# flash4242/Promptable-Counterfactual-GAN

Measured on AMD Instinct MI355X. Metric: images/sec (G+D step) MNIST-28 cDCGAN bs512 @1/2/4/8 MI355X; % MFMA roofline, higher is better.
Workload: dtype f32

## Files before the change

### include/pcgan_hip.h

```cpp
#ifndef PCGAN_HIP_H
#define PCGAN_HIP_H

#include <stddef.h>
#include <stdint.h>

#ifdef __cplusplus
extern "C" {
#endif

typedef void* pcg_stream_t;

typedef enum pcg_status {
  PCG_OK = 0,
  PCG_ERR_INVALID = -1,
  PCG_ERR_WORKSPACE = -2,
  PCG_ERR_LAUNCH = -3,
  PCG_ERR_UNSUPPORTED = -4
} pcg_status;

typedef enum pcg_act {
  PCG_ACT_NONE = 0,
  PCG_ACT_RELU = 1,
  PCG_ACT_LRELU = 2,
  PCG_ACT_TANH = 3,
// ... 443 lines not shown
} pcg_patch_mask_bits_args;
int pcg_patch_mask_bits(const pcg_patch_mask_bits_args* args, pcg_stream_t stream);

typedef struct pcg_mnist_cf_entry_args {
  const float* x;
  const float* table;
  const float* mask;
  const int64_t* target;
  float* out;
  int32_t B, T, HW, K, mask_mode, q0, nq;
} pcg_mnist_cf_entry_args;
int pcg_mnist_cf_entry(const pcg_mnist_cf_entry_args* args, pcg_stream_t stream);

typedef struct pcg_mnist_cf_tail_args {
  const float* c;
  const float* x;
  const float* mask;
  float* x_cf;
  float* raw; float* masked;
  float* sums;
  float scale;
  int32_t B, T, HW, mask_mode, q0, nq;
} pcg_mnist_cf_tail_args;
int pcg_mnist_cf_tail(const pcg_mnist_cf_tail_args* args, pcg_stream_t stream);

#define PCG_MNIST_CF_GROUP_SUMS 8
typedef struct pcg_mnist_cf_score_args {
  const float* logits_cf;
  const float* logits_orig;
  const int64_t* target;
  const int64_t* y_true;
  const float* tail_sums;
  int64_t* pred; float* conf; float* p_target; float* p_true; float* p_orig_true; float* flip;
  float* group_sums;
  int32_t B, T, K, ld, group_rows, q0, nq;
} pcg_mnist_cf_score_args;
int pcg_mnist_cf_score(const pcg_mnist_cf_score_args* args, pcg_stream_t stream);

int pcg_house_losses(const float* d_real, const float* d_fake, const float* d_fake_g, int64_t n, const float* g_cls, const float* am,
                     const float* pen, float lambda_cls, float w_reg, float lambda_mask, float w_reg_log, float* out5, pcg_stream_t stream);

typedef struct pcg_house_res_fwd_args {
  const float* cont; int32_t ncont;
  const float* samples; const int32_t* seg_dev; int32_t T;
  const float* norm; const float* x; const float* mask;
  const int32_t* col_src;
  int32_t D, B;
  float* res; float* masked; float* x_cf; float* partial512; int32_t* ticket; float* pen_out; float* am_out;
} pcg_house_res_fwd_args;
typedef struct pcg_house_res_bwd_args {
  const float* res; const float* masked; const float* mask; const float* gx_a; const float* gx_b;
  float w_pen, w_am;
  int32_t ncont; const int32_t* cont_idx_dev; const int32_t* seg_dev; int32_t S, T;
  const int32_t* cat_idx_dev; const float* norm;
  int32_t D, B;
  float* dcont; float* dsamples;
} pcg_house_res_bwd_args;
typedef struct pcg_house_loss_args {
  const float* d_real; const float* d_fake; const float* d_fake_g; int32_t n;
  const float* g_cls;
  const float* am; const float* pen;
  float lambda_cls, w_reg, lambda_mask, w_reg_log;
  const float* ce_row_loss;
  int32_t n_ce;
  float* out6;
} pcg_house_loss_args;
typedef struct pcg_house_diag_args {
  const float* logits_cf; const float* logits_orig;
  const int64_t* src_rows;
  const int64_t* target_y; const float* masked;
  int32_t B, nc, D;
  float eps;
  float* out4;
  double* acc;
} pcg_house_diag_args;
int pcg_house_residual_fwd(const pcg_house_res_fwd_args* args, const pcg_sn_fwd_batch* rider , pcg_stream_t stream);
int pcg_house_residual_bwd(const pcg_house_res_bwd_args* args, const pcg_house_loss_args* losses ,
                           const pcg_house_diag_args* diag , pcg_stream_t stream);
int pcg_house_diag(const pcg_house_diag_args* args, pcg_stream_t stream);
int pcg_house_draws(int64_t* target_y, int32_t B, int32_t num_classes, const int64_t* y, uint64_t offset_target, float* mask, int32_t D,
                    const int32_t* zero_cols, int32_t n_zero_cols, uint64_t offset_mask, float* noise, int32_t T, uint64_t offset_noise,
                    uint64_t seed, float* onehot_target, float* onehot_y, pcg_stream_t stream);
int pcg_house_draws_counter(int64_t* target_y, int32_t B, int32_t num_classes, const int64_t* y, float* mask, int32_t D,
                            const int32_t* zero_cols, int32_t n_zero_cols, float* noise, int32_t T, uint64_t seed, float* onehot_target,
                            float* onehot_y, uint64_t* counter, pcg_stream_t stream);
int pcg_house_batch_draws_counter(int64_t* target_y, int32_t B, int32_t num_classes, const float* X, const int64_t* Y,
                                  const int64_t* perm, int64_t n_perm, int64_t n_rows, float* x_out, int64_t* y_out,
                                  int64_t* src_out , float* mask, int32_t D, const int32_t* zero_cols, int32_t n_zero_cols,
                                  float* noise, int32_t T, uint64_t seed, float* onehot_target , float* onehot_y ,
                                  uint64_t* counter, pcg_stream_t stream);

int pcg_house_clf_batch(const float* X, const int64_t* Y, const int64_t* perm, int64_t n_perm, int64_t n_rows, float* x_out, int64_t* y_out,
                        int32_t B, int32_t D, float* m0, int32_t w0, float keep0, float* m1, int32_t w1, float keep1, float* m2, int32_t w2,
                        float keep2, uint64_t seed, uint64_t offset, int64_t cursor, pcg_stream_t stream);
int pcg_house_clf_batch_counter(const float* X, const int64_t* Y, const int64_t* perm, int64_t n_perm, int64_t n_rows, float* x_out,
                                int64_t* y_out, int32_t B, int32_t D, float* m0, int32_t w0, float keep0, float* m1, int32_t w1, float keep1,
                                float* m2, int32_t w2, float keep2, uint64_t seed, uint64_t* counter, pcg_stream_t stream);
int pcg_ce_weighted_tally(const float* logits, const int64_t* target, const float* class_weight, int32_t B, int32_t K, int32_t seg,
                          double* tally , float* dlogits , float* dbias ,
                          float* seg_loss , pcg_stream_t stream);

int pcg_mnist_clf_batch(const float* X, const int64_t* Y, const int64_t* perm, int64_t n_perm, int64_t n_rows, float* x_out, int64_t* y_out,
                        int32_t B, int32_t D, float* m0, int32_t w0, float keep0, float* m1, int32_t w1, float keep1, uint64_t seed,
                        uint64_t offset, int64_t cursor, pcg_stream_t stream);
int pcg_mnist_clf_batch_counter(const float* X, const int64_t* Y, const int64_t* perm, int64_t n_perm, int64_t n_rows, float* x_out,
                                int64_t* y_out, int32_t B, int32_t D, float* m0, int32_t w0, float keep0, float* m1, int32_t w1, float keep1,
                                uint64_t seed, uint64_t* counter, pcg_stream_t stream);
int pcg_drop2d_flatten_fwd(const float* a, const float* mask , float scale, int32_t R, int32_t HW, int32_t C, float* out,
                           pcg_stream_t stream);
int pcg_drop2d_flatten_bwd(const float* dflat, const float* mask, float scale, const float* y, int act, float slope, int32_t R, int32_t HW,
                           int32_t C, float* out, pcg_stream_t stream);
int pcg_mnist_clf_head(const float* h, const float* m1, float scale, const float* W2, const float* b2, const int64_t* y, int32_t R, int32_t I,
                       int32_t K, float* logits, float* loss, double* tally , float* dW2, float* db2, float* dh, float* db1,
                       pcg_stream_t stream);

int pcg_dp_barrier(pcg_stream_t stream);
int32_t pcg_dp_rccl_version(void);

#define PCG_DP_UNIQUE_ID_BYTES 128
int pcg_dp_unique_id(void* id_out );
int pcg_dp_init(const void* id , int32_t rank, int32_t world);
int32_t pcg_dp_world(void);
int32_t pcg_dp_rank(void);
pcg_stream_t pcg_dp_side_stream(void);
int pcg_dp_allreduce(float* buf, int64_t n, pcg_stream_t stream);
int pcg_dp_allreduce_begin(float* buf, int64_t n, int32_t slot, pcg_stream_t producer_stream);
int pcg_dp_record(int32_t slot);
int pcg_dp_allreduce_wait(int32_t slot, pcg_stream_t consumer_stream);
int pcg_dp_allreduce_sum_f64(double* buf, int64_t n, pcg_stream_t stream);
int pcg_dp_broadcast(void* buf, int64_t nbytes, int32_t root, pcg_stream_t stream);
int pcg_dp_sync_batchnorm(int32_t enable);
int pcg_dp_shutdown(void);

int pcg_tune_set(const char* name, int32_t value);

int pcg_conv_plan_describe(const pcg_conv_geom* g, int32_t op, int32_t assume_scratch, char* out, size_t out_bytes);
enum { PCG_PLAN_GEMM_ACT = 0, PCG_PLAN_GEMM = 1, PCG_PLAN_LINEAR_WGRAD = 2, PCG_PLAN_LINEAR_WGRAD_GROUPED = 3, PCG_PLAN_MEAN = 4,
       PCG_PLAN_ABS_MEAN = 5, PCG_PLAN_CROSS_ENTROPY = 6, PCG_PLAN_EMBED_CONCAT_BWD = 7, PCG_PLAN_ACT = 8, PCG_PLAN_ELEMENTWISE = 9,
       PCG_PLAN_BN_COLREDUCE = 10, PCG_PLAN_BN_APPLY = 11, PCG_PLAN_BN_FINALIZE = 12, PCG_PLAN_INSTNORM = 13, PCG_PLAN_SPECTRAL_NORM = 14,
       PCG_PLAN_ADAM = 15 };
enum { PCG_PLAN_EW_TABULAR = 0, PCG_PLAN_EW_CF_OPS = 1, PCG_PLAN_EW_POINTWISE = 2, PCG_PLAN_EW_GATHER_CHANNEL = 3 };
int pcg_launch_plan_describe(int32_t op, const int64_t* args, int32_t n_args, char* out, size_t out_bytes);
size_t pcg_conv_scratch_parts_bytes(void);
size_t pcg_conv_scratch_arrivals_bytes(void);
int pcg_conv_set_scratch(pcg_stream_t stream, void* parts, size_t parts_bytes, void* arrivals, size_t arrivals_bytes);
int pcg_conv_reset_scratch(pcg_stream_t stream);
size_t pcg_conv_pixtab_bytes(const pcg_conv_geom* g);
int pcg_conv_pixtab_register(const pcg_conv_geom* g, void* host_out, size_t bytes, const void* device_table);
size_t pcg_conv_cliptab_bytes(const pcg_conv_geom* g);
int pcg_conv_cliptab_register(const pcg_conv_geom* g, void* host_out, size_t bytes, const void* device_table);
double pcg_conv_sched_model(const int32_t* ktiles, int32_t n);
int pcg_conv_pad_clip_query(const pcg_conv_geom* g, int32_t op, int32_t groups, int32_t assume_scratch, int32_t* taken, int32_t* order,
                            int32_t* tile_rows, double* predicted);
int pcg_debug_stamp_buffer(void* buf, int64_t bytes);

typedef struct pcg_moons_cf_desc {
  int32_t hidden, clf_hidden, B, N;
  int32_t nG, nD, nC, nG_adam, nD_adam;
  int32_t g_off[14], d_off[8], c_off[6];
  double lr_G, lr_D, beta1, beta2, adam_eps;
  float bn_eps, bn_momentum, sn_eps, slope;
  float lambda_cls, lambda_l1, lambda_l2, lambda_mask;
} pcg_moons_cf_desc;

typedef struct pcg_moons_cf_train_args {
  const float* X; const int64_t* Y;
  const int64_t* rows;
  const int64_t* target_y;
  const float* mask;
  float* g_flat; float* d_flat; const float* c_flat;
  float* g_exp_avg; float* g_exp_avg_sq; int64_t* g_step;
  float* d_exp_avg; float* d_exp_avg_sq; int64_t* d_step;
  float* bn_mean[3]; float* bn_var[3]; int64_t* bn_nbt[3];
  float* sn_u[4]; float* sn_v[4];
  float* logs;
  float* scratch; size_t scratch_bytes;
} pcg_moons_cf_train_args;

size_t pcg_moons_cf_scratch_bytes(const pcg_moons_cf_desc* desc, int32_t forward);
int pcg_moons_cf_train_steps(const pcg_moons_cf_desc* desc, const pcg_moons_cf_train_args* args, int32_t n_steps, pcg_stream_t stream);

typedef struct pcg_moons_cf_fwd_args {
  int32_t which, train, B;
  const float* x; const float* onehot; const float* mask;
  float* params;
  float* bn_mean[3]; float* bn_var[3]; int64_t* bn_nbt[3];
  float* sn_u[4]; float* sn_v[4];
  float* out0; float* out1;
  float* scratch; size_t scratch_bytes;
} pcg_moons_cf_fwd_args;
int pcg_moons_cf_forward(const pcg_moons_cf_desc* desc, const pcg_moons_cf_fwd_args* args, pcg_stream_t stream);

typedef struct pcg_moons_cf_eval_args {
  int64_t N; int32_t M, T, group;
  const float* x; const int64_t* y;
  const float* masks;
  const int64_t* target; const float* row_mask;
  const float* g_flat; const float* c_flat;
  const float* bn_mean[3]; const float* bn_var[3];
  float* raw; float* masked; float* x_cf;
  float* logits_cf; float* logits_x;
  int64_t* pred_cf; int64_t* pred_x;
  float* gain;
  float* sums;
} pcg_moons_cf_eval_args;
int pcg_moons_cf_eval(const pcg_moons_cf_desc* desc, const pcg_moons_cf_eval_args* args, pcg_stream_t stream);

typedef struct {
  const float* gamma;
  const float* beta;
  float* running_mean;
  float* running_var;
  int64_t* num_batches_tracked;
  float* save_mean;
  float* save_invstd;
  float* xhat;
  float eps;
  float momentum;
  int32_t training;
} pcg_dense_bn;
typedef struct {
  const float* xhat;
  const float* gamma;
  const float* invstd;
  float* dgamma;
  float* dbeta;
  int32_t accumulate;
} pcg_dense_bn_bwd;
int pcg_dense_rows_fwd(const float* x, const float* W, const float* bias , int32_t R, int32_t I, int32_t O,
                       const pcg_dense_bn* bn , int act, float slope, float* y, pcg_stream_t stream);
int pcg_dense_rows_dgrad(const float* dz, const float* W, int32_t R, int32_t O, int32_t I, int below_act, float below_slope,
                         const float* y_below , const pcg_dense_bn_bwd* bn , float* dx,
                         pcg_stream_t stream);
int pcg_dense_rows_wgrad(const float* dz, const float* x, int32_t R, int32_t O, int32_t I, float* dW, float* db ,
                         int accumulate, pcg_stream_t stream);
int pcg_dense_rows_fwd_post(const float* x, const float* W, const float* bias , int32_t R, int32_t I, int32_t O, int act,
                            float slope, const float* gamma, const float* beta, float* running_mean ,
                            float* running_var , int64_t* num_batches_tracked , float eps, float momentum,
                            const float* mask , float scale, float* a, float* save_mean, float* save_invstd, float* y,
                            pcg_stream_t stream);
int pcg_dense_rows_dgrad_post(const float* dz, const float* W, int32_t R, int32_t O, int32_t I, const float* mask , float scale,
                              const float* a, const float* mean, const float* invstd, const float* gamma, int act, float slope,
                              float* dgamma, float* dbeta, float* db , int accumulate, float* dx, pcg_stream_t stream);

typedef struct pcg_moons_gan_desc {
  int32_t hidden, z_dim, label_dim, B, N;
  int32_t nG, nD, nG_adam, nD_adam;
  int32_t g_off[4], d_off[4];
  double lr_G, lr_D, beta1, beta2, adam_eps;
} pcg_moons_gan_desc;

typedef struct pcg_moons_gan_train_args {
  const float* X; const int64_t* Y;
  const int64_t* rows;
  const float* z;
  const int64_t* labels;
  float* g_flat; float* d_flat;
  float* g_exp_avg; float* g_exp_avg_sq; int64_t* g_step;
  float* d_exp_avg; float* d_exp_avg_sq; int64_t* d_step;
  float* logs;
  float* scratch; size_t scratch_bytes;
} pcg_moons_gan_train_args;

size_t pcg_moons_gan_scratch_bytes(const pcg_moons_gan_desc* desc);
int pcg_moons_gan_train_steps(const pcg_moons_gan_desc* desc, const pcg_moons_gan_train_args* args, int32_t n_steps, pcg_stream_t stream);

typedef struct pcg_moons_gan_fwd_args {
  int32_t which; int64_t R;
  const float* x; const float* onehot; const float* params;
  float* out;
} pcg_moons_gan_fwd_args;
int pcg_moons_gan_forward(const pcg_moons_gan_desc* desc, const pcg_moons_gan_fwd_args* args, pcg_stream_t stream);

typedef struct pcg_moons_clf_fit_desc {
  int32_t hidden, N, nC, nC_adam;
  int32_t c_off[6];
  double lr, beta1, beta2, adam_eps;
} pcg_moons_clf_fit_desc;
typedef struct pcg_moons_clf_fit_args {
  const float* X; const int64_t* Y;
  float* c_flat; float* exp_avg; float* exp_avg_sq; int64_t* step;
  float* losses;
  int32_t* correct;
  float* scratch; size_t scratch_bytes;
} pcg_moons_clf_fit_args;
size_t pcg_moons_clf_fit_scratch_bytes(const pcg_moons_clf_fit_desc* desc);
int pcg_moons_clf_fit(const pcg_moons_clf_fit_desc* desc, const pcg_moons_clf_fit_args* args, int32_t n_steps, pcg_stream_t stream);

int32_t pcg_calib_mfma_blocks(int32_t rounds);
size_t pcg_calib_mfma_workspace_bytes(int32_t rounds);
int pcg_calib_mfma(int32_t iters, int32_t rounds, void* workspace, size_t workspace_bytes, double* flop_out ,
                   uint64_t** stamps_out , pcg_stream_t stream);
int pcg_calib_copy(const void* src, void* dst, int64_t nbytes, pcg_stream_t stream);

int pcg_relu_maxpool2_fwd(const float* z, float* p, uint8_t* idx, int32_t B, int32_t H, int32_t W, int32_t C, pcg_stream_t stream);
int pcg_relu_maxpool2_bwd(const float* dp, const float* p, const uint8_t* idx, float* dz, int32_t B, int32_t H, int32_t W, int32_t C,
                          pcg_stream_t stream);

#define PCG_DELTA_GAN_BUILD 0
#define PCG_DELTA_GAN_REGATHER 1
#define PCG_LOGIT_HEAD_D 0
#define PCG_LOGIT_HEAD_G 1
#define PCG_DELTA_GAN_CHUNK 1024

typedef struct pcg_delta_gan_entry_args {
  const float* x;
// ... 142 lines not shown
```

### promptable-counterfactual-gan_amd/_lib.py

```python
import ctypes
import os

import torch

_HERE = os.path.dirname(os.path.abspath(__file__))
LIB_PATH = os.environ.get("PCG_LIB") or os.path.join(_HERE, "libpcgan_hip.so")

PCG_OK = 0
ACT_NONE, ACT_RELU, ACT_LRELU, ACT_TANH, ACT_SIGMOID = 0, 1, 2, 3, 4
(PLAN_GEMM_ACT, PLAN_GEMM, PLAN_LINEAR_WGRAD, PLAN_LINEAR_WGRAD_GROUPED, PLAN_MEAN, PLAN_ABS_MEAN, PLAN_CROSS_ENTROPY,
 PLAN_EMBED_CONCAT_BWD, PLAN_ACT, PLAN_ELEMENTWISE, PLAN_BN_COLREDUCE, PLAN_BN_APPLY, PLAN_BN_FINALIZE, PLAN_INSTNORM,
 PLAN_SPECTRAL_NORM, PLAN_ADAM) = range(16)
PLAN_EW_TABULAR, PLAN_EW_CF_OPS, PLAN_EW_POINTWISE, PLAN_EW_GATHER_CHANNEL = range(4)


class PcgError(RuntimeError):
    pass


class ConvGeom(ctypes.Structure):

    _fields_ = [(n, ctypes.c_int32) for n in ("B", "IH", "IW", "Cin", "OH", "OW", "Cout", "KH", "KW", "stride", "pad")]

    def key(self):
# ... 123 lines not shown
    _fields_ = [(n, _P) for n in ("xhat", "gamma", "invstd", "dgamma", "dbeta")] + [("accumulate", _I)]


_PP, _PI, _F = ctypes.POINTER(ctypes.c_void_p), ctypes.POINTER(ctypes.c_int32), ctypes.c_float


class SnFwdBatch(ctypes.Structure):
    _fields_ = ([("n", _I), ("reps", _I), ("power_iteration", _I), ("eps", _F), ("w_orig", _PP), ("out_features", _PI), ("in_features", _PI)] +
                [(n, _PP) for n in ("u", "v", "w_bar", "sigma", "u_used", "v_used")])


class SnBwdBatch(ctypes.Structure):
    _fields_ = [("n", _I), ("passes", _I), ("dw_bar", _PP), ("w_bar", _PP), ("out_features", _PI), ("in_features", _PI), ("u", _PP), ("v", _PP),
                ("sigma", _PP), ("dw_orig", _PP), ("accumulate", _PI), ("db_dst", _PP), ("db_src", _PP)]


class HouseCriticFwdArgs(ctypes.Structure):
    _fields_ = ([(n, _I) for n in ("n_pass", "B", "D", "NC")] + [("slope", _F)] +
                [(n, _PP) for n in ("x", "onehot", "w_bar", "bias", "a0", "a1", "a2", "a3", "out")])


class HouseCriticBwdArgs(ctypes.Structure):
    _fields_ = ([(n, _I) for n in ("n_pass", "B", "D")] + [("slope", _F)] +
                [(n, _PP) for n in ("dout", "w_bar", "a1", "a2", "a3", "d3", "d2", "d1", "dx")])


class HouseClsFwdArgs(ctypes.Structure):
    _fields_ = ([("x", _P), ("B", _I), ("w_kmajor", _PP), ("bias", _PP)] + [(n, _P) for n in ("a1", "a2", "a3", "a4", "logits", "ce_target")] +
                [("ce_grad_scale", _F), ("ce_dlogits", _P), ("ce_row_loss", _P)])


class HouseClsBwdArgs(ctypes.Structure):
    _fields_ = [("dlogits", _P), ("B", _I), ("w_stored", _PP)] + [(n, _P) for n in ("a1", "a2", "a3", "a4", "dx")]


class HouseResFwdArgs(ctypes.Structure):
    _fields_ = ([("cont", _P), ("ncont", _I), ("samples", _P), ("seg_dev", _P), ("T", _I), ("norm", _P), ("x", _P), ("mask", _P), ("col_src", _PI),
                 ("D", _I), ("B", _I)] + [(n, _P) for n in ("res", "masked", "x_cf", "partial512", "ticket", "pen_out", "am_out")])


class HouseResBwdArgs(ctypes.Structure):
    _fields_ = ([(n, _P) for n in ("res", "masked", "mask", "gx_a", "gx_b")] + [("w_pen", _F), ("w_am", _F), ("ncont", _I), ("cont_idx_dev", _P),
                ("seg_dev", _P), ("S", _I), ("T", _I), ("cat_idx_dev", _P), ("norm", _P), ("D", _I), ("B", _I), ("dcont", _P), ("dsamples", _P)])


class HouseLossArgs(ctypes.Structure):
    _fields_ = ([("d_real", _P), ("d_fake", _P), ("d_fake_g", _P), ("n", _I), ("g_cls", _P), ("am", _P), ("pen", _P)] +
                [(n, _F) for n in ("lambda_cls", "w_reg", "lambda_mask", "w_reg_log")] + [("ce_row_loss", _P), ("n_ce", _I), ("out6", _P)])


class HouseDiagArgs(ctypes.Structure):
    _fields_ = ([(n, _P) for n in ("logits_cf", "logits_orig", "src_rows", "target_y", "masked")] + [("B", _I), ("nc", _I), ("D", _I), ("eps", _F),
                ("out4", _P), ("acc", _P)])


class DeltaGanEntryArgs(ctypes.Structure):
    _fields_ = ([(n, _P) for n in ("x", "y", "target", "y_host", "target_host", "table_g", "table_d", "g_in", "d_in", "labels_2b", "head_w",
                                   "head_w_packed")] + [(n, _I) for n in ("B", "HW", "K", "mode", "head_C", "head_P")])


class DeltaGanTailFwdArgs(ctypes.Structure):
    _fields_ = ([(n, _P) for n in ("x", "delta", "x_cf", "d_in", "loss_reg", "workspace")] + [("workspace_bytes", ctypes.c_size_t)] +
                [(n, _I) for n in ("B", "HW", "grid")])


class LogitHeadFwdArgs(ctypes.Structure):
    _fields_ = [(n, _P) for n in ("a", "w", "bias", "logits", "loss", "dlogit", "db", "workspace")] + [(n, _I) for n in ("R", "F", "mode")]


class LogitHeadBwdArgs(ctypes.Structure):
    _fields_ = [(n, _P) for n in ("a", "w", "dlogit", "da", "dw")] + [("slope", _F)] + [(n, _I) for n in ("R", "F", "dw_C", "dw_P")]


class DeltaGanTailBwdArgs(ctypes.Structure):
    _fields_ = ([(n, _P) for n in ("dD", "dC", "delta", "d_delta")] + [("lambda_cls", _F), ("reg_scale", _F)] +
                [(n, _I) for n in ("B", "HW", "dD_stride")])


class DeltaCfEntryArgs(ctypes.Structure):
    _fields_ = [(n, _P) for n in ("x", "table", "target", "target_host", "out")] + [(n, _I) for n in ("B", "T", "HW", "K", "q0", "nq")]


class DeltaCfTailArgs(ctypes.Structure):
    _fields_ = [(n, _P) for n in ("delta", "x", "x_cf", "sums")] + [(n, _I) for n in ("B", "T", "HW", "q0", "nq")]


class DeltaGanTargetDrawArgs(ctypes.Structure):
    _fields_ = [("target", _P), ("counter", _P), ("seed", ctypes.c_uint64), ("offset", ctypes.c_uint64), ("B", _I), ("K", _I)]


class ProbHeadFwdArgs(ctypes.Structure):
    _fields_ = ([(n, _P) for n in ("a", "w", "bias", "logits", "prob", "loss", "dlogit", "db", "workspace")] +
                [("workspace_bytes", ctypes.c_size_t), ("eps", _F)] + [(n, _I) for n in ("R", "F", "mode", "slabs")])


class LogEpsLossArgs(ctypes.Structure):
    _fields_ = [(n, _P) for n in ("p", "grad_out", "loss", "dp")] + [("eps", _F), ("R", _I), ("mode", _I)]


DELTA_GAN_BUILD, DELTA_GAN_REGATHER = 0, 1
LOGIT_HEAD_D, LOGIT_HEAD_G = 0, 1
DELTA_GAN_CHUNK = 1024
PROB_HEAD_D, PROB_HEAD_G = 0, 1
PROB_HEAD_MAX_SLABS = 16
CLASS_PICK_FIRST, CLASS_PICK_BEST = 0, 1
CLASS_PICK_KMAX = 64
CF_PANELS_GRID, CF_PANELS_PANELS = 0, 1

STRUCTS = {"pcg_conv_geom": ConvGeom, "pcg_in_xform": InXform, "pcg_wgrad_item": WgradItem, "pcg_sn_fwd_batch": SnFwdBatch,
           "pcg_sn_bwd_batch": SnBwdBatch, "pcg_house_g_desc": HouseGDesc, "pcg_house_g_fwd_args": HouseGFwdArgs,
           "pcg_house_g_bwd_args": HouseGBwdArgs, "pcg_house_critic_fwd_args": HouseCriticFwdArgs,
           "pcg_house_critic_bwd_args": HouseCriticBwdArgs, "pcg_house_cls_fwd_args": HouseClsFwdArgs, "pcg_house_cls_bwd_args": HouseClsBwdArgs,
           "pcg_house_res_fwd_args": HouseResFwdArgs, "pcg_house_res_bwd_args": HouseResBwdArgs, "pcg_house_loss_args": HouseLossArgs,
           "pcg_house_diag_args": HouseDiagArgs, "pcg_moons_cf_desc": MoonsCfDesc, "pcg_moons_cf_train_args": MoonsCfTrainArgs,
           "pcg_moons_cf_fwd_args": MoonsCfFwdArgs, "pcg_moons_cf_eval_args": MoonsCfEvalArgs,
           "pcg_house_cf_eval_args": HouseCfEvalArgs, "pcg_patch_mask_bits_args": PatchMaskBitsArgs,
           "pcg_mnist_cf_entry_args": MnistCfEntryArgs, "pcg_mnist_cf_tail_args": MnistCfTailArgs,
           "pcg_mnist_cf_score_args": MnistCfScoreArgs, "pcg_dense_bn": DenseBn,
           "pcg_dense_bn_bwd": DenseBnBwd, "pcg_moons_gan_desc": MoonsGanDesc, "pcg_moons_gan_train_args": MoonsGanTrainArgs,
           "pcg_moons_gan_fwd_args": MoonsGanFwdArgs, "pcg_moons_clf_fit_desc": MoonsClfFitDesc,
           "pcg_moons_clf_fit_args": MoonsClfFitArgs, "pcg_delta_gan_entry_args": DeltaGanEntryArgs,
           "pcg_delta_gan_tail_fwd_args": DeltaGanTailFwdArgs, "pcg_logit_head_fwd_args": LogitHeadFwdArgs,
           "pcg_logit_head_bwd_args": LogitHeadBwdArgs, "pcg_delta_gan_tail_bwd_args": DeltaGanTailBwdArgs,
           "pcg_delta_cf_entry_args": DeltaCfEntryArgs, "pcg_delta_cf_tail_args": DeltaCfTailArgs,
           "pcg_delta_gan_target_draw_args": DeltaGanTargetDrawArgs, "pcg_prob_head_fwd_args": ProbHeadFwdArgs,
           "pcg_log_eps_loss_args": LogEpsLossArgs}

_c = ctypes
_vp, _f, _i, _i64, _sz = _c.c_void_p, _c.c_float, _c.c_int, _c.c_int64, _c.c_size_t
_d = _c.c_double
_i32 = _c.c_int32
_gp = _c.POINTER(ConvGeom)
_xp = _c.POINTER(InXform)

PROTOTYPES = {
    "pcg_abi_version": (_i, []),
    "pcg_abi_struct_bytes": (_sz, [_c.c_char_p]),
    "pcg_last_error": (_c.c_char_p, []),
    "pcg_target_arch": (_c.c_char_p, []),
    "pcg_tune_set": (_i, [_c.c_char_p, _i32]),
    "pcg_debug_stamp_buffer": (_i, [_vp, _i64]),
    "pcg_conv_plan_describe": (_i, [_c.POINTER(ConvGeom), _i32, _i32, _c.c_char_p, _sz]),
    "pcg_launch_plan_describe": (_i, [_i32, _c.POINTER(_i64), _i32, _c.c_char_p, _sz]),
    "pcg_conv_scratch_parts_bytes": (_sz, []),
    "pcg_conv_scratch_arrivals_bytes": (_sz, []),
    "pcg_conv_set_scratch": (_i, [_vp, _vp, _sz, _vp, _sz]),
    "pcg_conv_reset_scratch": (_i, [_vp]),
    "pcg_conv_pixtab_bytes": (_sz, [_gp]),
    "pcg_conv_pixtab_register": (_i, [_gp, _vp, _sz, _vp]),
    "pcg_conv_cliptab_bytes": (_sz, [_gp]),
    "pcg_conv_cliptab_register": (_i, [_gp, _vp, _sz, _vp]),
    "pcg_conv_sched_model": (_d, [_vp, _i32]),
    "pcg_conv_pad_clip_query": (_i, [_gp, _i32, _i32, _i32, _vp, _vp, _vp, _vp]),
    "pcg_conv2d_fwd_bn_g": (_i, [_gp, _vp, _vp, _vp, _vp, _f, _f, _vp, _vp, _vp, _vp, _vp, _i32, _vp, _sz, _vp]),
    "pcg_bn_apply_act_g": (_i, [_vp, _i64, _i32, _vp, _vp, _vp, _vp, _i, _f, _vp, _i32, _vp]),
    "pcg_conv2d_dgrad_bn_phases": (_i32, [_gp]),
    "pcg_conv2d_dgrad_bnbwd_g": (_i, [_gp, _vp, _vp, _vp, _vp, _vp, _vp, _vp, _i, _f, _vp, _vp, _sz, _i32, _vp]),
    "pcg_bn_bwd_partial_g_workspace_bytes": (_sz, [_i32, _i32]),
    "pcg_bn_bwd_partial_g": (_i, [_vp, _vp, _i64, _i32, _vp, _vp, _vp, _vp, _i32, _i32, _vp, _vp, _vp, _i, _i32, _vp, _sz, _vp]),
    "pcg_bn_act_bwd_g_workspace_bytes": (_sz, [_i64, _i32, _i32]),
    "pcg_bn_act_bwd_premask_g": (_i, [_vp, _vp, _i64, _i32, _vp, _vp, _vp, _vp, _i, _f, _vp, _vp, _vp, _i, _i32, _vp, _sz, _vp]),
    "pcg_bce_pair": (_i, [_vp, _i64, _f, _f, _vp, _vp, _vp, _vp, _vp, _vp]),
    "pcg_conv2d_fwd_bnbwd_thin_ok": (_i32, [_gp]),
    "pcg_conv2d_fwd_bnbwd_thin_workspace_bytes": (_sz, [_gp]),
    "pcg_conv2d_fwd_bnbwd_thin": (_i, [_gp, _vp, _vp, _vp, _vp, _vp, _vp, _vp, _i, _f, _vp, _vp, _vp, _i, _vp, _sz, _vp]),
    "pcg_conv2d_bnin_full_ok": (_i32, [_gp, _i32]),
    "pcg_conv2d_fwd_bnin_full": (_i, [_gp, _vp, _vp, _vp, _vp, _vp, _i, _f, _i32, _vp, _vp, _i, _f, _vp, _vp]),
    "pcg_conv2d_wgrad_bnin_full": (_i, [_gp, _vp, _vp, _vp, _vp, _vp, _i, _f, _i32, _vp, _vp, _i, _vp, _sz, _vp]),
    "pcg_conv_precision_set": (_i, [_i32]),
    "pcg_conv_precision_get": (_i32, []),
    "pcg_slab_defer_begin": (_i, [_vp]),
    "pcg_slab_defer_flush": (_i, [_vp]),
    "pcg_slab_defer_pending": (_i32, []),
    "pcg_conv2d_dgrad_bnbwd_full_ok": (_i32, [_gp, _i32]),
    "pcg_conv2d_dgrad_bnbwd_full_workspace_bytes": (_sz, [_gp, _i32]),
    "pcg_conv2d_dgrad_bnbwd_full": (_i, [_gp, _vp, _vp, _vp, _vp, _vp, _vp, _vp, _i, _f, _vp, _vp, _vp, _i, _i32, _vp, _sz, _vp]),
    "pcg_calib_mfma_blocks": (_i32, [_i32]),
    "pcg_calib_mfma_workspace_bytes": (_sz, [_i32]),
    "pcg_calib_mfma": (_i, [_i32, _i32, _vp, _sz, _c.POINTER(_d), _c.POINTER(_c.c_uint64), _vp]),
    "pcg_calib_copy": (_i, [_vp, _vp, _i64, _vp]),
    "pcg_conv2d_fwd_workspace_bytes": (_sz, [_gp]),
    "pcg_conv2d_dgrad_workspace_bytes": (_sz, [_gp]),
    "pcg_conv2d_fwd": (_i, [_gp, _vp, _vp, _vp, _vp, _vp, _sz, _vp]),
    "pcg_conv2d_dgrad": (_i, [_gp, _vp, _vp, _vp, _vp, _vp, _sz, _vp]),
    "pcg_conv2d_fwd_act": (_i, [_gp, _vp, _vp, _vp, _i, _f, _vp, _vp, _sz, _vp]),
    "pcg_conv2d_dgrad_act": (_i, [_gp, _vp, _vp, _vp, _i, _f, _vp, _vp, _sz, _vp]),
    "pcg_conv2d_fwd_bn_workspace_bytes": (_sz, [_gp]),
    "pcg_conv2d_dgrad_bn_workspace_bytes": (_sz, [_gp]),
    "pcg_conv2d_fwd_bn": (_i, [_gp, _vp, _vp, _vp, _vp, _f, _f, _vp, _vp, _vp, _vp, _vp, _vp, _sz, _vp]),
    "pcg_conv2d_dgrad_bn": (_i, [_gp, _vp, _vp, _vp, _vp, _f, _f, _vp, _vp, _vp, _vp, _vp, _vp, _sz, _vp]),
    "pcg_conv2d_dgrad_mask": (_i, [_gp, _vp, _vp, _vp, _i, _f, _vp, _vp, _sz, _vp]),
    "pcg_conv2d_dgrad_mask_thin_ok": (_i32, [_gp]),
    "pcg_conv2d_xf_thin_ok": (_i32, [_gp]),
    "pcg_conv2d_fwd_add_mask": (_i, [_gp, _vp, _vp, _vp, _vp, _i, _f, _vp, _vp]),
    "pcg_conv2d_dgrad_add_mask": (_i, [_gp, _vp, _vp, _vp, _vp, _i, _f, _vp, _vp]),
    "pcg_conv2d_fwd_mask": (_i, [_gp, _vp, _vp, _vp, _i, _f, _vp, _vp, _sz, _vp]),
    "pcg_conv2d_dgrad_bnbwd": (_i, [_gp, _vp, _vp, _vp, _vp, _vp, _vp, _vp, _i, _f, _vp, _vp, _sz, _vp]),
    "pcg_conv2d_fwd_bnbwd": (_i, [_gp, _vp, _vp, _vp, _vp, _vp, _vp, _vp, _i, _f, _vp, _vp, _sz, _vp]),
    "pcg_conv2d_dgrad_add": (_i, [_gp, _vp, _vp, _vp, _vp, _vp, _sz, _vp]),
    "pcg_conv2d_fwd_bn_partial_rows": (_c.c_int32, [_gp]),
    "pcg_conv2d_dgrad_bn_partial_rows": (_c.c_int32, [_gp]),
    "pcg_bn_bwd_partial_workspace_bytes": (_sz, [_c.c_int32]),
    "pcg_bn_bwd_partial": (_i, [_vp, _vp, _i64, _c.c_int32, _vp, _vp, _vp, _vp, _c.c_int32, _vp, _vp, _vp, _i, _vp, _sz, _vp]),
    "pcg_conv2d_fwd_bn_xf": (_i, [_gp, _vp, _xp, _vp, _vp, _vp, _f, _f, _vp, _vp, _vp, _vp, _vp, _vp, _vp, _vp, _vp, _sz, _vp]),
    "pcg_conv2d_dgrad_bn_xf": (_i, [_gp, _vp, _xp, _vp, _vp, _vp, _f, _f, _vp, _vp, _vp, _vp, _vp, _vp, _vp, _vp, _vp, _sz, _vp]),
    "pcg_conv2d_fwd_xf": (_i, [_gp, _vp, _xp, _vp, _vp, _i, _f, _vp, _vp, _sz, _vp]),
    "pcg_conv2d_dgrad_xf": (_i, [_gp, _vp, _xp, _vp, _vp, _i, _f, _vp, _vp, _sz, _vp]),
    "pcg_conv2d_wgrad_xf": (_i, [_gp, _vp, _xp, _vp, _xp, _vp, _i, _vp, _sz, _vp]),
    "pcg_bn_train_stats_coef": (_i, [_vp, _i64, _c.c_int32, _f, _f, _vp, _vp, _vp, _vp, _vp, _vp, _vp, _vp, _vp, _sz, _vp]),
    "pcg_bn_db_workspace_bytes": (_sz, [_i64, _c.c_int32]),
    "pcg_bn_act_bwd_db": (_i, [_vp, _vp, _vp, _i64, _c.c_int32, _vp, _vp, _vp, _vp, _i, _f, _f, _vp, _vp, _vp, _i, _vp, _i, _vp, _sz, _vp]),
    "pcg_bn_bwd_partial_db_workspace_bytes": (_sz, [_c.c_int32]),
    "pcg_bn_bwd_partial_db": (_i, [_vp, _vp, _i64, _c.c_int32, _vp, _vp, _vp, _vp, _c.c_int32, _f, _vp, _vp, _vp, _i, _vp, _i, _vp, _sz, _vp]),
    "pcg_conv2d_dgrad_add_bnsum": (_i, [_gp, _vp, _vp, _vp, _vp, _vp, _vp, _f, _vp, _vp, _sz, _vp]),
    "pcg_conv2d_fwd_add": (_i, [_gp, _vp, _vp, _vp, _vp, _vp, _sz, _vp]),
    "pcg_conv2d_fwd_add_bnsum": (_i, [_gp, _vp, _vp, _vp, _vp, _vp, _vp, _f, _vp, _vp, _sz, _vp]),
    "pcg_conv_weight_adjoint": (_i, [_vp, _vp, _i32, _i32, _i32, _i32, _vp]),
    "pcg_conv_weight_adjoint_many": (_i, [_vp, _vp, _i32, _i32, _i32, _i32, _i32, _vp]),
    "pcg_house_losses": (_i, [_vp, _vp, _vp, _i64, _vp, _vp, _vp, _f, _f, _f, _f, _vp, _vp]),
    "pcg_dp_unique_id": (_i, [_vp]),
    "pcg_dp_init": (_i, [_vp, _i32, _i32]),
    "pcg_dp_world": (_i32, []),
    "pcg_dp_rank": (_i32, []),
    "pcg_dp_side_stream": (_vp, []),
    "pcg_dp_allreduce": (_i, [_vp, _i64, _vp]),
    "pcg_dp_allreduce_begin": (_i, [_vp, _i64, _i32, _vp]),
    "pcg_dp_record": (_i, [_i32]),
    "pcg_dp_allreduce_wait": (_i, [_i32, _vp]),
    "pcg_dp_allreduce_sum_f64": (_i, [_vp, _i64, _vp]),
    "pcg_dp_broadcast": (_i, [_vp, _i64, _i32, _vp]),
    "pcg_dp_sync_batchnorm": (_i, [_i32]),
    "pcg_dp_barrier": (_i, [_vp]),
    "pcg_dp_rccl_version": (_i32, []),
    "pcg_dp_shutdown": (_i, []),
    "pcg_conv2d_wgrad_workspace_bytes": (_sz, [_gp]),
    "pcg_conv2d_wgrad": (_i, [_gp, _vp, _vp, _vp, _i, _vp, _sz, _vp]),
    "pcg_colsum_workspace_bytes": (_sz, [_i64, _c.c_int32]),
    "pcg_colsum": (_i, [_vp, _i64, _c.c_int32, _vp, _i, _vp, _sz, _vp]),
    "pcg_bn_workspace_bytes": (_sz, [_i64, _c.c_int32]),
    "pcg_bn_train_stats": (_i, [_vp, _i64, _c.c_int32, _f, _f, _vp, _vp, _vp, _vp, _vp, _vp, _sz, _vp]),
    "pcg_bn_apply_act": (_i, [_vp, _i64, _c.c_int32, _vp, _vp, _f, _vp, _vp, _i, _f, _vp, _f, _vp, _vp]),
    "pcg_bn_act_bwd": (_i, [_vp, _vp, _vp, _i64, _c.c_int32, _vp, _vp, _vp, _i, _f, _f, _vp, _vp, _vp, _i, _vp, _sz, _vp]),
    "pcg_bn_act_bwd_premask": (_i, [_vp, _vp, _i64, _c.c_int32, _vp, _vp, _vp, _vp, _i, _f, _f, _vp, _vp, _vp, _i, _vp, _sz, _vp]),
    "pcg_embed_concat_fwd": (_i, [_vp, _vp, _vp, _vp, _vp, _c.c_int32, _c.c_int32, _c.c_int32, _c.c_int32, _vp]),
    "pcg_embed_concat_bwd": (_i, [_vp, _vp, _vp, _vp, _c.c_int32, _c.c_int32, _c.c_int32, _c.c_int32, _i, _vp]),
    "pcg_embed_table_grad": (_i, [_vp, _vp, _vp, _i32, _i32, _i32, _i32, _i32, _i, _vp]),
    "pcg_gather_channel": (_i, [_vp, _vp, _i32, _i32, _i32, _vp]),
    "pcg_axpby": (_i, [_vp, _f, _vp, _f, _vp, _i64, _vp]),
    "pcg_scale_mask_fwd": (_i, [_vp, _vp, _f, _vp, _vp, _i64, _vp]),
    "pcg_scale_mask_bwd": (_i, [_vp, _vp, _vp, _f, _vp, _i64, _vp]),
    "pcg_clamp_add_fwd": (_i, [_vp, _vp, _f, _f, _vp, _i64, _vp]),
    "pcg_clamp_add_bwd": (_i, [_vp, _vp, _vp, _f, _f, _vp, _i64, _vp]),
    "pcg_abs_mean_workspace_bytes": (_sz, []),
    "pcg_abs_mean_fwd": (_i, [_vp, _vp, _i, _i64, _vp, _vp, _sz, _vp]),
    "pcg_abs_mean_bwd": (_i, [_vp, _vp, _i, _i64, _vp, _f, _vp, _i, _vp]),
    "pcg_avgpool_fwd": (_i, [_vp, _vp, _c.c_int32, _c.c_int32, _c.c_int32, _vp]),
    "pcg_avgpool_bwd": (_i, [_vp, _vp, _c.c_int32, _c.c_int32, _c.c_int32, _vp]),
    "pcg_cross_entropy_fwd_bwd": (_i, [_vp, _vp, _c.c_int32, _c.c_int32, _f, _vp, _vp, _vp, _vp]),
    "pcg_act_fwd": (_i, [_vp, _i64, _i, _f, _vp, _vp]),
    "pcg_act_bwd": (_i, [_vp, _vp, _i64, _i, _f, _vp, _vp]),
    "pcg_bce_fwd_bwd": (_i, [_vp, _vp, _f, _i64, _f, _vp, _vp, _vp, _vp]),
    "pcg_bce_logits_fwd_bwd": (_i, [_vp, _f, _i64, _f, _vp, _vp, _vp, _vp]),
    "pcg_adam_step": (_i, [_vp, _vp, _vp, _vp, _i64, _d, _d, _d, _d, _d, _i, _i64, _vp]),
    "pcg_adam_step_capturable": (_i, [_vp, _vp, _vp, _vp, _i64, _d, _d, _d, _d, _d, _i, _vp, _vp, _vp]),
    "pcg_patch_mask": (_i, [_vp, _c.c_int32, _c.c_int32, _c.c_int32, _c.c_int32, _c.c_int32, _c.c_uint64, _c.c_uint64, _vp]),
    "pcg_randint": (_i, [_vp, _i64, _c.c_int32, _c.c_int32, _vp, _c.c_uint64, _c.c_uint64, _vp]),
    "pcg_randn": (_i, [_vp, _i64, _f, _f, _c.c_uint64, _c.c_uint64, _vp]),
    "pcg_fill": (_i, [_vp, _i64, _f, _vp]),
    "pcg_add_bias_rows": (_i, [_vp, _i64, _i32, _vp, _vp]),
    "pcg_sumsq": (_i, [_vp, _i64, _vp, _i, _vp]),
    "pcg_norm_sum": (_i, [_vp, _vp, _i32, _vp, _vp]),
    "pcg_instnorm_fwd": (_i, [_vp, _i32, _i32, _i32, _vp, _vp, _f, _i, _f, _vp, _vp, _vp, _vp]),
    "pcg_instnorm_bwd": (_i, [_vp, _vp, _i32, _i32, _i32, _vp, _vp, _vp, _vp, _vp, _vp, _vp]),
    "pcg_instnorm_bwd_bwd": (_i, [_vp, _vp, _vp, _i32, _i32, _i32, _vp, _vp, _vp, _vp, _vp, _vp, _vp]),
    "pcg_instnorm_bwd_fused": (_i, [_vp, _vp, _f, _vp, _i32, _i32, _i32, _vp, _vp, _vp, _vp, _vp, _vp, _vp, _vp, _vp, _vp]),
    "pcg_instnorm_bwd_bwd_act": (_i, [_vp, _vp, _vp, _i32, _i32, _i32, _vp, _vp, _vp, _vp, _f, _vp, _vp, _vp, _vp]),
    "pcg_rowsum3": (_i, [_i32, _vp, _vp, _i, _vp, _vp, _i, _vp, _vp, _i, _i32, _i32, _vp]),
    "pcg_nhwc_to_nchw_flat": (_i, [_vp, _vp, _i32, _i32, _i32, _i, _vp]),
    "pcg_interpolate": (_i, [_vp, _vp, _vp, _vp, _i32, _i32, _vp]),
    "pcg_interpolate_stack": (_i, [_vp, _vp, _vp, _vp, _i32, _i32, _vp]),
    "pcg_gradient_penalty_fwd": (_i, [_vp, _i32, _i32, _f, _vp, _vp, _vp]),
    "pcg_gradient_penalty_bwd": (_i, [_vp, _vp, _vp, _i32, _i32, _f, _vp, _vp]),
    "pcg_rand_uniform": (_i, [_vp, _i64, _c.c_uint64, _c.c_uint64, _vp]),
    "pcg_cross_entropy_weighted_fwd_bwd": (_i, [_vp, _vp, _vp, _i32, _i32, _f, _vp, _vp, _vp, _vp]),
    "pcg_dropout_apply": (_i, [_vp, _vp, _i64, _i32, _i32, _f, _vp, _vp]),
    "pcg_rand_bernoulli": (_i, [_vp, _i64, _f, _c.c_uint64, _c.c_uint64, _vp]),
    "pcg_resize8_normalize": (_i, [_vp, _i32, _i32, _i32, _i32, _i32, _vp, _vp, _i32, _vp, _vp, _i32, _f, _f, _vp, _vp]),
    "pcg_house_g_fwd": (_i, [_c.POINTER(HouseGDesc), _c.POINTER(HouseGFwdArgs), _vp]),
    "pcg_house_g_bwd": (_i, [_c.POINTER(HouseGDesc), _c.POINTER(HouseGBwdArgs), _vp]),
    "pcg_weighted_sum_fwd": (_i, [_i32, _vp, _vp, _vp, _vp]),
    "pcg_weighted_sum_bwd": (_i, [_i32, _vp, _vp, _vp, _vp]),
    "pcg_cf_metrics": (_i, [_vp, _vp, _vp, _vp, _i32, _i32, _vp, _vp]),
    "pcg_gemm": (_i, [_i, _i, _i32, _i32, _i32, _vp, _i32, _vp, _i32, _vp, _i32, _vp, _i, _vp]),
    "pcg_linear_wgrad_workspace_bytes": (_sz, [_i32, _i32, _i32]),
    "pcg_linear_wgrad_ticket_count": (_i32, []),
    "pcg_linear_wgrad": (_i, [_vp, _i32, _vp, _i32, _i32, _i32, _i32, _vp, _vp, _i, _i, _vp, _sz, _vp, _vp]),
    "pcg_spectral_norm_fwd_batched": (_i, [_c.POINTER(SnFwdBatch), _vp]),
    "pcg_spectral_norm_bwd_batched": (_i, [_c.POINTER(SnBwdBatch), _vp]),
    "pcg_house_critic_fwd": (_i, [_c.POINTER(HouseCriticFwdArgs), _vp]),
    "pcg_house_critic_bwd": (_i, [_c.POINTER(HouseCriticBwdArgs), _vp]),
    "pcg_house_classifier_fwd": (_i, [_c.POINTER(HouseClsFwdArgs), _c.POINTER(SnBwdBatch), _vp]),
    "pcg_house_classifier_bwd": (_i, [_c.POINTER(HouseClsBwdArgs), _c.POINTER(SnFwdBatch), _vp]),
    "pcg_house_cf_eval": (_i, [_c.POINTER(HouseGDesc), _c.POINTER(HouseCfEvalArgs), _vp]),
    "pcg_patch_mask_bits": (_i, [_c.POINTER(PatchMaskBitsArgs), _vp]),
    "pcg_mnist_cf_entry": (_i, [_c.POINTER(MnistCfEntryArgs), _vp]),
    "pcg_mnist_cf_tail": (_i, [_c.POINTER(MnistCfTailArgs), _vp]),
# ... 107 lines not shown
```

### promptable-counterfactual-gan_amd/csrc/conv_igemm.hip

```cpp
#include <string.h>
#include <array>
#include <map>
#include <mutex>
#include "conv_loaders.h"
#include "conv_pixtab.h"
#include "conv_cliptab.h"
#include "thin_conv.h"

namespace pcg {
namespace {

__device__ __forceinline__ int wave_id() { return __builtin_amdgcn_readfirstlane((int)(threadIdx.x >> 6)); }

__device__ __forceinline__ void prio_entry(const ConvP& p) { if (p.edge_prio & 1) __builtin_amdgcn_s_setprio(3); }
__device__ __forceinline__ void prio_epilogue(const ConvP& p) { if (p.edge_prio & 2) __builtin_amdgcn_s_setprio(3); }

__device__ __forceinline__ int epi_group_off(const ConvP& p, int m_block) {
  return p.epi.group_rows > 0 ? __builtin_amdgcn_readfirstlane(m_block / p.epi.group_rows) * p.N : 0;
}

template <class Cfg, bool XF, bool CLIP = false>
__global__ void __launch_bounds__(IG_THREADS, Cfg::MINW) conv_fwd_kernel(ConvP p) {
  extern __shared__ __attribute__((aligned(16))) float smem[];
  prio_entry(p);
  if constexpr (CLIP) {
    uint32_t nt, idx;
    clip_block_tile(blockIdx.x, (uint32_t)p.tilesN, gridDim.x / (uint32_t)p.tilesN, p.clip_order, false, 0u, nt, idx);
    nt = __builtin_amdgcn_readfirstlane(nt); idx = __builtin_amdgcn_readfirstlane(idx);
    const ClipTile t = clip_tile(p, 0, idx, Cfg::BM);
    const int n_block = (int)nt * Cfg::BN;
    const int ktiles = t.nh * t.nw * ((p.Cin + IG_BK - 1) / IG_BK);
    if (wave_id() >= 4) {
      const int tid = threadIdx.x - IG_LOADERS;
      FwdALoader<Cfg::BM, XF, true> la(p, t, tid);
      FwdBLoader<Cfg::BN, true> lb(p, n_block, tid);
      lb.it.clip(t.h0, t.nh, t.w0, t.nw);
      igemm_produce<Cfg>(la, lb, ktiles, smem, tid, ClockStamp{p.stamps, p.stamp_slots});
      return;
    }
    f32x16 acc[Cfg::TM][Cfg::TN];
    ClockStamp cs{p.stamps, p.stamp_slots};
    cs.phase(0);
    igemm_consume<Cfg, true, true>(ktiles, acc, smem, cs);
    prio_epilogue(p);
    const size_t npix = (size_t)p.OH * p.OW;
    igemm_store_tile<Cfg>(acc, smem, n_block, p.N, p.bias, [&](int row) -> float* {
      const int b = t.img0 + row;
      return b < p.B ? p.out + ((size_t)b * npix + t.pos) * p.N + n_block : nullptr;
    }, p.stat_partial ? p.stat_partial + (size_t)t.stat_tile * Cfg::WAVES_M * 2 * p.N : nullptr, p.act, p.slope, &p.epi,
       p.epi.group_rows > 0 ? t.group * p.N : 0);
    cs.phase(3);
    return;
  }
  const uint32_t tile = xcd_remap(blockIdx.x, gridDim.x);
  const int mt = tile / p.tilesN, nt = tile % p.tilesN;
  const int m_block = mt * Cfg::BM, n_block = nt * Cfg::BN;
  const int kt_begin = blockIdx.y * p.ktiles_per_split;
  int ktiles = p.ktiles - kt_begin;
  if (ktiles > p.ktiles_per_split) ktiles = p.ktiles_per_split;

  if (wave_id() >= 4) {
    const int tid = threadIdx.x - IG_LOADERS;
    FwdALoader<Cfg::BM, XF> la(p, m_block, tid);
    FwdBLoader<Cfg::BN> lb(p, n_block, tid);
    if (kt_begin) { la.seek(kt_begin); lb.seek(kt_begin); }
    igemm_produce<Cfg>(la, lb, ktiles, smem, tid, ClockStamp{p.stamps, p.stamp_slots});
    return;
  }
  f32x16 acc[Cfg::TM][Cfg::TN];
  ClockStamp cs{p.stamps, p.stamp_slots};
  cs.phase(0);
  igemm_consume<Cfg, true, true>(ktiles, acc, smem, cs);
  prio_epilogue(p);
  float* out = p.out + (size_t)blockIdx.y * (size_t)p.M * (size_t)p.N;
#ifdef PCG_ABL_NO_EPILOGUE
  if (acc[0][0][0] == 12345.678f) out[0] = acc[0][0][1];
  return;
#endif
  igemm_store_tile<Cfg>(acc, smem, n_block, p.N, blockIdx.y == 0 ? p.bias : nullptr, [&](int row) -> float* {
    const int m = m_block + row;
    return m < p.M ? out + (size_t)m * p.N + n_block : nullptr;
  }, p.stat_partial ? p.stat_partial + (size_t)mt * Cfg::WAVES_M * 2 * p.N : nullptr, p.act, p.slope, &p.epi, epi_group_off(p, m_block));
  cs.phase(3);
}

template <class Cfg, bool XF, bool CLIP = false>
__global__ void __launch_bounds__(IG_THREADS, Cfg::MINW) conv_dgrad_kernel(ConvP p, DgradPhases phases) {
  extern __shared__ __attribute__((aligned(16))) float smem[];
  __shared__ int rowpix[Cfg::BM];
  prio_entry(p);
  if constexpr (CLIP) {
    const uint32_t nil = phases.interleave ? (uint32_t)phases.interleave : 1u, per = nil * (uint32_t)p.tilesN;
    uint32_t within, idx;
    clip_block_tile(blockIdx.x, per, gridDim.x / per, p.clip_order, !phases.interleave, blockIdx.y, within, idx);
    idx = __builtin_amdgcn_readfirstlane(idx);
    const uint32_t py = __builtin_amdgcn_readfirstlane(phases.interleave ? within % nil : blockIdx.y), nt = __builtin_amdgcn_readfirstlane(within / nil);
    const PhaseInfo& f = phases.p[py];
    const ClipTile t = clip_tile(p, 1 + 2 * f.ph + f.pw, idx, Cfg::BM);
    const int n_block = (int)nt * Cfg::BN;
    const int ktiles = t.nh * t.nw * ((p.Cout + IG_BK - 1) / IG_BK);
    if (wave_id() >= 4) {
      const int tid = threadIdx.x - IG_LOADERS;
      uint32_t aa, cc;
      f.dPHw.divmod((uint32_t)t.pos, aa, cc);
      const int pix0 = ((int)aa * p.stride + f.ph) * p.IW + (int)cc * p.stride + f.pw;
      for (int r = tid; r < Cfg::BM; r += IG_LOADERS) rowpix[r] = t.img0 + r < p.B ? (t.img0 + r) * p.IH * p.IW + pix0 : -1;
      DgradALoader<Cfg::BM, XF, true> la(p, f, t, tid);
      DgradBLoader<Cfg::BN, true> lb(p, f, n_block, tid);
      lb.it.clip(t.h0, t.nh, t.w0, t.nw);
      igemm_produce<Cfg>(la, lb, ktiles, smem, tid, ClockStamp{p.stamps, p.stamp_slots});
      return;
    }
    f32x16 acc[Cfg::TM][Cfg::TN];
    ClockStamp cs{p.stamps, p.stamp_slots};
    cs.phase(0);
    igemm_consume<Cfg, true, false>(ktiles, acc, smem, cs);
    prio_epilogue(p);
    igemm_store_tile<Cfg>(acc, smem, n_block, p.N, p.bias, [&](int row) -> float* {
      const int pix = rowpix[row];
      return pix >= 0 ? p.out + (size_t)pix * p.Cin + n_block : nullptr;
    }, p.stat_partial ? p.stat_partial + (size_t)(f.prow0 + t.stat_tile * Cfg::WAVES_M) * 2 * p.N : nullptr, p.act, p.slope, &p.epi,
       p.epi.group_rows > 0 ? t.group * p.N : 0);
    cs.phase(3);
    return;
  }
  uint32_t bx = blockIdx.x, py = blockIdx.y;
  if (phases.interleave) {
    const uint32_t l = xcd_remap(blockIdx.x, gridDim.x);
    py = l % (uint32_t)phases.interleave; bx = l / (uint32_t)phases.interleave;
  }
  const PhaseInfo& f = phases.p[py];
  const int tilesM = (f.Mp + Cfg::BM - 1) / Cfg::BM;
  const uint32_t ntiles = (uint32_t)tilesM * p.tilesN;
  if (bx >= ntiles) return;
  const uint32_t tile = phases.interleave ? bx : xcd_remap(bx, ntiles);
  const int mt = tile / p.tilesN, nt = tile % p.tilesN;
  const int m_block = mt * Cfg::BM, n_block = nt * Cfg::BN;
  const int ktiles = f.nth * f.ntw * ((p.Cout + IG_BK - 1) / IG_BK);

  if (wave_id() >= 4) {
    const int tid = threadIdx.x - IG_LOADERS;
    for (int r = tid; r < Cfg::BM; r += IG_LOADERS) {
      const int m = m_block + r;
      int pix = -1;
      if (m < f.Mp) {
        uint32_t t, cc, b, aa;
        f.dPHw.divmod((uint32_t)m, t, cc);
        f.dPHh.divmod(t, b, aa);
        pix = ((int)b * p.IH + (int)aa * p.stride + f.ph) * p.IW + (int)cc * p.stride + f.pw;
      }
      rowpix[r] = pix;
    }
    DgradALoader<Cfg::BM, XF> la(p, f, m_block, tid);
    DgradBLoader<Cfg::BN> lb(p, f, n_block, tid);
    igemm_produce<Cfg>(la, lb, ktiles, smem, tid, ClockStamp{p.stamps, p.stamp_slots});
    return;
  }
  f32x16 acc[Cfg::TM][Cfg::TN];
  ClockStamp cs{p.stamps, p.stamp_slots};
  cs.phase(0);
  igemm_consume<Cfg, true, false>(ktiles, acc, smem, cs);
  prio_epilogue(p);
  igemm_store_tile<Cfg>(acc, smem, n_block, p.N, p.bias, [&](int row) -> float* {
    const int pix = rowpix[row];
    return pix >= 0 ? p.out + (size_t)pix * p.Cin + n_block : nullptr;
  }, p.stat_partial ? p.stat_partial + (size_t)(f.prow0 + mt * Cfg::WAVES_M) * 2 * p.N : nullptr, p.act, p.slope, &p.epi, epi_group_off(p, m_block));
  cs.phase(3);
}

struct SkPlan {
  int dp_tiles, sk_tiles, sk_blocks, ktiles;
  float* parts;
  int* arrivals;
};
struct SkSeg { int tile, kt_begin, nkt, nparts, first_block; };

__device__ __forceinline__ int sk_start(int g, const SkPlan& sk) {
  return __builtin_amdgcn_readfirstlane((int)((uint32_t)g * (uint32_t)(sk.sk_tiles * sk.ktiles) / (uint32_t)sk.sk_blocks));
}
__device__ __forceinline__ int sk_owner(int x, const SkPlan& sk) {
  return __builtin_amdgcn_readfirstlane((int)((((uint32_t)x + 1u) * (uint32_t)sk.sk_blocks - 1u) / (uint32_t)(sk.sk_tiles * sk.ktiles)));
}
__device__ __forceinline__ int sk_segments(const SkPlan& sk, SkSeg& s0, SkSeg& s1) {
  const int b = blockIdx.x;
  if (b < sk.dp_tiles) { s0 = SkSeg{(int)xcd_remap((uint32_t)b, (uint32_t)sk.dp_tiles), 0, sk.ktiles, 1, 0}; return 1; }
  const int g = (int)xcd_remap((uint32_t)(b - sk.dp_tiles), (uint32_t)sk.sk_blocks), KT = sk.ktiles;
  const int it0 = sk_start(g, sk), it1 = sk_start(g + 1, sk);
  const int j0 = __builtin_amdgcn_readfirstlane(it0 / KT), e0 = it1 < (j0 + 1) * KT ? it1 : (j0 + 1) * KT;
  auto fill = [&](SkSeg& sg, int j, int from, int to) {
    const int f = sk_owner(j * KT, sk), l = sk_owner((j + 1) * KT - 1, sk);
    sg = SkSeg{sk.dp_tiles + j, from - j * KT, to - from, l - f + 1, f};
  };
  fill(s0, j0, it0, e0);
  if (it1 <= e0) return 1;
  fill(s1, j0 + 1, e0, it1);
  return 2;
}
#if defined(__HIP_DEVICE_COMPILE__) && !defined(__gfx950__)
#error "stream-K partial-tile exchange (sc1 stores + relaxed agent-scope counters) is written for gfx950 only"
#endif
__device__ __forceinline__ void sk_store4(rsrc_t r, uint32_t off, float a, float b, float c, float d) {
  const u32x4 v = {__float_as_uint(a), __float_as_uint(b), __float_as_uint(c), __float_as_uint(d)};
  __builtin_amdgcn_raw_buffer_store_b128(v, r, off, 0, 16);
}
__device__ __forceinline__ float4 sk_load4(rsrc_t r, uint32_t off) {
  const u32x4 v = __builtin_amdgcn_raw_buffer_load_b128(r, off, 0, 16);
  return make_float4(__uint_as_float(v.x), __uint_as_float(v.y), __uint_as_float(v.z), __uint_as_float(v.w));
}
template <class Cfg, class FirstOf>
__device__ __forceinline__ bool sk_combine_core(float* parts, int* arrivals, int nblocks, int g, int j, int nparts, int first_block,
                                                FirstOf first_of, f32x16 (&acc)[Cfg::TM][Cfg::TN]) {
  if (nparts == 1) return true;
  constexpr uint32_t TILE_BYTES = Cfg::BM * Cfg::BN * 4;
  auto slot_of = [&](int blk) { return (uint32_t)(2 * blk + (first_of(blk) ? 0 : 1)); };
  const rsrc_t rs = make_rsrc(parts, (uint32_t)(2 * nblocks) * TILE_BYTES);
  const uint32_t toff = threadIdx.x * 16u;
  const uint32_t mine = slot_of(g) * TILE_BYTES + toff;
#pragma unroll
  for (int i = 0; i < Cfg::TM; ++i)
#pragma unroll
    for (int jj = 0; jj < Cfg::TN; ++jj)
#pragma unroll
      for (int q = 0; q < 4; ++q)
        sk_store4(rs, mine + (uint32_t)(((i * Cfg::TN + jj) * 4 + q) * IG_LOADERS * 16),
                  acc[i][jj][4 * q], acc[i][jj][4 * q + 1], acc[i][jj][4 * q + 2], acc[i][jj][4 * q + 3]);
  asm volatile("s_waitcnt vmcnt(0)" ::: "memory");
  int* cnt = arrivals + j * 4 + (int)(threadIdx.x >> 6);
  int old = 0;
  if ((threadIdx.x & 63) == 0) old = __hip_atomic_fetch_add(cnt, 1, __ATOMIC_RELAXED, __HIP_MEMORY_SCOPE_AGENT);
  old = __builtin_amdgcn_readfirstlane(old);
  if (old != nparts - 1) return false;
  if ((threadIdx.x & 63) == 0) __hip_atomic_store(cnt, 0, __ATOMIC_RELAXED, __HIP_MEMORY_SCOPE_AGENT);
#pragma unroll
  for (int i = 0; i < Cfg::TM; ++i)
#pragma unroll
    for (int jj = 0; jj < Cfg::TN; ++jj)
#pragma unroll
      for (int r = 0; r < 16; ++r) acc[i][jj][r] = 0.f;
  for (int k = 0; k < nparts; ++k) {
    const uint32_t src = slot_of(first_block + k) * TILE_BYTES + toff;
#pragma unroll
    for (int i = 0; i < Cfg::TM; ++i)
#pragma unroll
      for (int jj = 0; jj < Cfg::TN; ++jj)
#pragma unroll
        for (int q = 0; q < 4; ++q) {
          const float4 v = sk_load4(rs, src + (uint32_t)(((i * Cfg::TN + jj) * 4 + q) * IG_LOADERS * 16));
          acc[i][jj][4 * q] += v.x; acc[i][jj][4 * q + 1] += v.y; acc[i][jj][4 * q + 2] += v.z; acc[i][jj][4 * q + 3] += v.w;
        }
  }
  return true;
}
template <class Cfg>
__device__ __forceinline__ bool sk_combine(const SkPlan& sk, const SkSeg& sg, f32x16 (&acc)[Cfg::TM][Cfg::TN]) {
  const int g = (int)xcd_remap((uint32_t)((int)blockIdx.x - sk.dp_tiles), (uint32_t)sk.sk_blocks), j = sg.tile - sk.dp_tiles, KT = sk.ktiles;
  return sk_combine_core<Cfg>(sk.parts, sk.arrivals, sk.sk_blocks, g, j, sg.nparts, sg.first_block,
                              [&](int blk) { return sk_start(blk, sk) >= j * KT; }, acc);
}

template <class Cfg, bool XF>
__device__ __forceinline__ void fwd_sk_segment(const ConvP& p, const SkPlan& sk, const SkSeg& sg, float* smem) {
  const int mt = __builtin_amdgcn_readfirstlane(sg.tile / p.tilesN), nt = sg.tile - mt * p.tilesN;
  const int m_block = mt * Cfg::BM, n_block = nt * Cfg::BN;
  if (wave_id() >= 4) {
    const int tid = threadIdx.x - IG_LOADERS;
    FwdALoader<Cfg::BM, XF> la(p, m_block, tid);
    FwdBLoader<Cfg::BN> lb(p, n_block, tid);
    if (sg.kt_begin) { la.seek(sg.kt_begin); lb.seek(sg.kt_begin); }
    igemm_produce<Cfg>(la, lb, sg.nkt, smem, tid, ClockStamp{nullptr, 0});
    return;
  }
  f32x16 acc[Cfg::TM][Cfg::TN];
  igemm_consume<Cfg, true, true>(sg.nkt, acc, smem);
  if (sk_combine<Cfg>(sk, sg, acc))
    igemm_store_tile<Cfg>(acc, smem, n_block, p.N, p.bias, [&](int row) -> float* {
      const int m = m_block + row;
      return m < p.M ? p.out + (size_t)m * p.N + n_block : nullptr;
    }, p.stat_partial ? p.stat_partial + (size_t)mt * Cfg::WAVES_M * 2 * p.N : nullptr, p.act, p.slope, &p.epi, epi_group_off(p, m_block));
}
template <class Cfg, bool XF>
__global__ void __launch_bounds__(IG_THREADS, Cfg::MINW) conv_fwd_sk_kernel(ConvP p, SkPlan sk) {
  extern __shared__ __attribute__((aligned(16))) float smem[];
  SkSeg s0, s1{};
  const int nseg = sk_segments(sk, s0, s1);
  fwd_sk_segment<Cfg, XF>(p, sk, s0, smem);
  if (nseg == 1) return;
  lds_barrier();
  fwd_sk_segment<Cfg, XF>(p, sk, s1, smem);
}

template <class Cfg, bool XF>
__device__ __forceinline__ void dgrad_sk_segment(const ConvP& p, const DgradPhases& phases, const SkPlan& sk, const SkSeg& sg, int tiles_per_phase,
                                                 float* smem, int* rowpix) {
  const int py = __builtin_amdgcn_readfirstlane(sg.tile / tiles_per_phase), tile = sg.tile - py * tiles_per_phase;
  const PhaseInfo& f = phases.p[py];
  const int mt = __builtin_amdgcn_readfirstlane(tile / p.tilesN), nt = tile - mt * p.tilesN;
  const int m_block = mt * Cfg::BM, n_block = nt * Cfg::BN;
  if (wave_id() >= 4) {
    const int tid = threadIdx.x - IG_LOADERS;
    for (int r = tid; r < Cfg::BM; r += IG_LOADERS) {
      const int m = m_block + r;
      int pix = -1;
      if (m < f.Mp) {
        uint32_t t, cc, b, aa;
        f.dPHw.divmod((uint32_t)m, t, cc);
        f.dPHh.divmod(t, b, aa);
        pix = ((int)b * p.IH + (int)aa * p.stride + f.ph) * p.IW + (int)cc * p.stride + f.pw;
      }
      rowpix[r] = pix;
    }
    DgradALoader<Cfg::BM, XF> la(p, f, m_block, tid);
    DgradBLoader<Cfg::BN> lb(p, f, n_block, tid);
    if (sg.kt_begin) { la.seek(sg.kt_begin); lb.seek(sg.kt_begin); }
    igemm_produce<Cfg>(la, lb, sg.nkt, smem, tid, ClockStamp{nullptr, 0});
    return;
  }
  f32x16 acc[Cfg::TM][Cfg::TN];
  igemm_consume<Cfg, true, false>(sg.nkt, acc, smem);
  if (sk_combine<Cfg>(sk, sg, acc))
    igemm_store_tile<Cfg>(acc, smem, n_block, p.N, p.bias, [&](int row) -> float* {
      const int pix = rowpix[row];
      return pix >= 0 ? p.out + (size_t)pix * p.Cin + n_block : nullptr;
    }, p.stat_partial ? p.stat_partial + (size_t)(f.prow0 + mt * Cfg::WAVES_M) * 2 * p.N : nullptr, p.act, p.slope, &p.epi, epi_group_off(p, m_block));
}
template <class Cfg, bool XF>
__global__ void __launch_bounds__(IG_THREADS, Cfg::MINW) conv_dgrad_sk_kernel(ConvP p, DgradPhases phases, SkPlan sk, int tiles_per_phase) {
  extern __shared__ __attribute__((aligned(16))) float smem[];
  __shared__ int rowpix[Cfg::BM];
  SkSeg s0, s1{};
  const int nseg = sk_segments(sk, s0, s1);
  dgrad_sk_segment<Cfg, XF>(p, phases, sk, s0, tiles_per_phase, smem, rowpix);
  if (nseg == 1) return;
  lds_barrier();
  dgrad_sk_segment<Cfg, XF>(p, phases, sk, s1, tiles_per_phase, smem, rowpix);
}

template <class Cfg, bool XFA, bool XFB, bool TAB = false>
__global__ void __launch_bounds__(IG_THREADS, 4) conv_wgrad_kernel(ConvP p, int ktiles_total, int ktiles_per_split, int tiles,
                                                                   int slice_major) {
  extern __shared__ __attribute__((aligned(16))) float smem[];
  prio_entry(p);
  uint32_t tile, split;
  if (slice_major) {
    const uint32_t l = xcd_remap(blockIdx.x, gridDim.x);
    split = l / (uint32_t)tiles; tile = l - split * (uint32_t)tiles;
  } else {
    tile = xcd_remap(blockIdx.x, gridDim.x); split = blockIdx.y;
  }
  const int mt = tile / p.tilesN, nt = tile % p.tilesN;
  const int m_block = mt * Cfg::BM, n_block = nt * Cfg::BN;
  const int kt_begin = split * ktiles_per_split;
  int ktiles = ktiles_total - kt_begin;
  if (ktiles > ktiles_per_split) ktiles = ktiles_per_split;

  if (wave_id() >= 4) {
    const int tid = threadIdx.x - IG_LOADERS;
    WgradALoader<Cfg::BM, XFA> la(p, m_block, kt_begin, tid);
    WgradBLoader<Cfg::BN, XFB, TAB> lb(p, n_block, kt_begin, tid);
    igemm_produce<Cfg>(la, lb, ktiles, smem, tid, ClockStamp{p.stamps, p.stamp_slots});
    return;
  }
  f32x16 acc[Cfg::TM][Cfg::TN];
  igemm_consume<Cfg, false, false>(ktiles, acc, smem, ClockStamp{p.stamps, p.stamp_slots});
  prio_epilogue(p);
  float* slab = p.out + (size_t)split * (size_t)p.M * (size_t)p.N;
  igemm_store_tile<Cfg>(acc, smem, n_block, p.N, nullptr, [&](int row) -> float* {
    const int m = m_block + row;
    return m < p.M ? slab + (size_t)m * p.N + n_block : nullptr;
  });
}


struct SkNPlan {
  int nph, blocks, total;
  int tile0[5], it0[5], kt[4];
  float* parts; int* arrivals;
};
__device__ __forceinline__ int skn_start(int g, const SkNPlan& sk) {
  return __builtin_amdgcn_readfirstlane((int)((uint32_t)g * (uint32_t)sk.total / (uint32_t)sk.blocks));
}
__device__ __forceinline__ int skn_owner(int x, const SkNPlan& sk) {
  return __builtin_amdgcn_readfirstlane((int)((((uint32_t)x + 1u) * (uint32_t)sk.blocks - 1u) / (uint32_t)sk.total));
}
struct SkNSeg { int py, tin, t_begin, e, kt_begin, nkt, fb, nparts, mt, nt; };
__device__ __forceinline__ SkNSeg skn_segment(int it, int it1, const SkNPlan& sk, int tilesN) {
  SkNSeg s;
  s.py = 0;
  if (sk.nph > 1 && it >= sk.it0[1]) s.py = 1;
  if (sk.nph > 2 && it >= sk.it0[2]) s.py = 2;
  if (sk.nph > 3 && it >= sk.it0[3]) s.py = 3;
  const int KT = sk.kt[s.py], local = it - sk.it0[s.py];
  s.tin = __builtin_amdgcn_readfirstlane(local / KT);
  s.t_begin = sk.it0[s.py] + s.tin * KT;
  const int t_end = s.t_begin + KT;
  s.e = it1 < t_end ? it1 : t_end;
  s.kt_begin = it - s.t_begin; s.nkt = s.e - it;
  s.fb = skn_owner(s.t_begin, sk); s.nparts = skn_owner(t_end - 1, sk) - s.fb + 1;
  s.mt = __builtin_amdgcn_readfirstlane(s.tin / tilesN); s.nt = s.tin - s.mt * tilesN;
  return s;
}
template <class Cfg, bool XF>
__global__ void __launch_bounds__(IG_THREADS, Cfg::MINW) conv_dgrad_skn_kernel(ConvP p, DgradPhases phases, SkNPlan sk) {
  extern __shared__ __attribute__((aligned(16))) float smem[];
  __shared__ int rowpix[Cfg::BM];
  const int g = (int)xcd_remap(blockIdx.x, (uint32_t)sk.blocks);
  const int it1 = skn_start(g + 1, sk);
  if (wave_id() >= 4) {
    const int tid = threadIdx.x - IG_LOADERS;
#pragma unroll 1
    for (int it = skn_start(g, sk); it < it1;) {
      const SkNSeg sg = skn_segment(it, it1, sk, p.tilesN);
      const PhaseInfo& f = phases.p[sg.py];
      const int m_block = sg.mt * Cfg::BM, n_block = sg.nt * Cfg::BN;
      for (int r = tid; r < Cfg::BM; r += IG_LOADERS) {
        const int m = m_block + r;
        int pix = -1;
        if (m < f.Mp) {
          uint32_t t, cc, b, aa;
          f.dPHw.divmod((uint32_t)m, t, cc);
          f.dPHh.divmod(t, b, aa);
          pix = ((int)b * p.IH + (int)aa * p.stride + f.ph) * p.IW + (int)cc * p.stride + f.pw;
        }
        rowpix[r] = pix;
      }
      DgradALoader<Cfg::BM, XF> la(p, f, m_block, tid);
      DgradBLoader<Cfg::BN> lb(p, f, n_block, tid);
      if (sg.kt_begin) { la.seek(sg.kt_begin); lb.seek(sg.kt_begin); }
      igemm_produce<Cfg>(la, lb, sg.nkt, smem, tid, ClockStamp{nullptr, 0});
      it = sg.e;
      if (it < it1) lds_barrier();
    }
    return;
  }
#pragma unroll 1
  for (int it = skn_start(g, sk); it < it1;) {
    const SkNSeg sg = skn_segment(it, it1, sk, p.tilesN);
    const PhaseInfo& f = phases.p[sg.py];
    const int m_block = sg.mt * Cfg::BM, n_block = sg.nt * Cfg::BN;
    {
      f32x16 acc[Cfg::TM][Cfg::TN];
      igemm_consume<Cfg, true, false>(sg.nkt, acc, smem);
      const int t_begin = sg.t_begin;
      if (sk_combine_core<Cfg>(sk.parts, sk.arrivals, sk.blocks, g, sk.tile0[sg.py] + sg.tin, sg.nparts, sg.fb,
                               [&](int blk) { return skn_start(blk, sk) >= t_begin; }, acc))
        igemm_store_tile<Cfg>(acc, smem, n_block, p.N, p.bias, [&](int row) -> float* {
          const int pix = rowpix[row];
          return pix >= 0 ? p.out + (size_t)pix * p.Cin + n_block : nullptr;
        }, p.stat_partial ? p.stat_partial + (size_t)(f.prow0 + sg.mt * Cfg::WAVES_M) * 2 * p.N : nullptr, p.act, p.slope, &p.epi, epi_group_off(p, m_block));
    }
    it = sg.e;
    if (it < it1) lds_barrier();
  }
}

template <class Cfg, bool XFA, bool XFB, bool TAB>
__device__ __forceinline__ void wgrad_sk_segment(const ConvP& p, const SkPlan& sk, const SkSeg& sg, float* smem) {
  const int mt = __builtin_amdgcn_readfirstlane(sg.tile / p.tilesN), nt = sg.tile - mt * p.tilesN;
  const int m_block = mt * Cfg::BM, n_block = nt * Cfg::BN;
  if (wave_id() >= 4) {
    const int tid = threadIdx.x - IG_LOADERS;
    WgradALoader<Cfg::BM, XFA> la(p, m_block, sg.kt_begin, tid);
    WgradBLoader<Cfg::BN, XFB, TAB> lb(p, n_block, sg.kt_begin, tid);
    igemm_produce<Cfg>(la, lb, sg.nkt, smem, tid, ClockStamp{nullptr, 0});
    return;
  }
  f32x16 acc[Cfg::TM][Cfg::TN];
  igemm_consume<Cfg, false, false>(sg.nkt, acc, smem);
  if (sk_combine<Cfg>(sk, sg, acc))
    igemm_store_tile<Cfg>(acc, smem, n_block, p.N, nullptr, [&](int row) -> float* {
      const int m = m_block + row;
      return m < p.M ? p.out + (size_t)m * p.N + n_block : nullptr;
    }, nullptr, PCG_ACT_NONE, 0.f, &p.epi);
}
template <class Cfg, bool XFA, bool XFB, bool TAB = false>
__global__ void __launch_bounds__(IG_THREADS, 4) conv_wgrad_sk_kernel(ConvP p, SkPlan sk) {
  extern __shared__ __attribute__((aligned(16))) float smem[];
  SkSeg s0, s1{};
  const int nseg = sk_segments(sk, s0, s1);
  wgrad_sk_segment<Cfg, XFA, XFB, TAB>(p, sk, s0, smem);
  if (nseg == 1) return;
  lds_barrier();
  wgrad_sk_segment<Cfg, XFA, XFB, TAB>(p, sk, s1, smem);
}

using Cfg64x192 = TileCfg<64, 192, 2, 2>;
template <class Cfg, bool TAB = false>
__global__ void __launch_bounds__(IG_THREADS, 4) conv_wgrad192_kernel(ConvP p, int ktiles_total, int ktiles_per_split, int tiles,
                                                                      int slice_major) {
  static_assert(Cfg::BM == 64 && Cfg::BN == 192, "the 192-column weight-gradient tile");
  extern __shared__ __attribute__((aligned(16))) float smem[];
  prio_entry(p);
  uint32_t tile, split;
  if (slice_major) {
    const uint32_t l = xcd_remap(blockIdx.x, gridDim.x);
    split = l / (uint32_t)tiles; tile = l - split * (uint32_t)tiles;
  } else {
    tile = xcd_remap(blockIdx.x, gridDim.x); split = blockIdx.y;
  }
  const int mt = tile / p.tilesN, nt = tile % p.tilesN;
  const int m_block = mt * Cfg::BM, n_block = nt * Cfg::BN;
  const int kt_begin = split * ktiles_per_split;
  int ktiles = ktiles_total - kt_begin;
  if (ktiles > ktiles_per_split) ktiles = ktiles_per_split;
  if (wave_id() >= 4) {
    const int tid = threadIdx.x - IG_LOADERS;
    WgradALoader<Cfg::BM, false> la(p, m_block, kt_begin, tid);
    WgradBLoader192<TAB> lb(p, n_block, kt_begin, tid);
    igemm_produce<Cfg>(la, lb, ktiles, smem, tid);
    return;
  }
  f32x16 acc[Cfg::TM][Cfg::TN];
  igemm_consume<Cfg, false, false>(ktiles, acc, smem, ClockStamp{p.stamps, p.stamp_slots});
  prio_epilogue(p);
  float* slab = p.out + (size_t)split * (size_t)p.M * (size_t)p.N;
  igemm_store_tile<Cfg>(acc, smem, n_block, p.N, nullptr, [&](int row) -> float* {
    const int m = m_block + row;
    return m < p.M ? slab + (size_t)m * p.N + n_block : nullptr;
  });
}

__global__ void __launch_bounds__(256) col2im_kernel(const float4* __restrict__ dcol, float4* __restrict__ dx, const float* __restrict__ bias,
                                                     int B, int IH, int IW, int CQ, int OH, int OW, int KH, int KW, int stride, int pad,
                                                     FastDiv dCQ, FastDiv dIW, FastDiv dIH, int act, float neg) {
  const uint32_t total = (uint32_t)B * IH * IW * CQ;
  for (uint32_t idx = blockIdx.x * 256u + threadIdx.x; idx < total; idx += gridDim.x * 256u) {
    uint32_t pix, cq, t, iw, b, ih;
    dCQ.divmod(idx, pix, cq);
    dIW.divmod(pix, t, iw);
    dIH.divmod(t, b, ih);
    float4 acc = bias ? *reinterpret_cast<const float4*>(bias + 4 * cq) : make_float4(0.f, 0.f, 0.f, 0.f);
    for (int kh = 0; kh < KH; ++kh) {
      const int th = (int)ih + pad - kh;
      if (th < 0 || th % stride) continue;
      const int oh = th / stride;
      if (oh >= OH) continue;
      for (int kw = 0; kw < KW; ++kw) {
        const int tw = (int)iw + pad - kw;
        if (tw < 0 || tw % stride) continue;
        const int ow = tw / stride;
        if (ow >= OW) continue;
        const float4 v = dcol[((size_t)(((int)b * OH + oh) * OW + ow) * (KH * KW) + (kh * KW + kw)) * CQ + cq];
        acc.x += v.x; acc.y += v.y; acc.z += v.z; acc.w += v.w;
      }
    }
    if (act != PCG_ACT_NONE) {
      acc.x = act_neg_scale(acc.x, neg); acc.y = act_neg_scale(acc.y, neg); acc.z = act_neg_scale(acc.z, neg); acc.w = act_neg_scale(acc.w, neg);
    }
    dx[idx] = acc;
  }
}

using Cfg128x128 = TileCfg<128, 128, 2, 2>;
#ifndef PCG_PAD_CLIP_DEFAULT
#define PCG_PAD_CLIP_DEFAULT 1
#endif
#ifndef PCG_TILE64_SWZ
#define PCG_TILE64_SWZ 1
#endif
using Cfg128x64P = TileCfg<128, 64, 2, 2>;
#if PCG_TILE64_SWZ
using Cfg128x64 = TileCfg<128, 64, 2, 2, true, 6, 1>;
#else
using Cfg128x64 = Cfg128x64P;
#endif

template <class C>
using Bf16Twin = TileCfg<C::BM, C::BN, C::WAVES_M, C::WAVES_N, false, C::MINW, C::PF, true>;


int check_geom(const pcg_conv_geom* g) {
  PCG_REQUIRE(g != nullptr, "conv geometry is null");
  PCG_REQUIRE(g->B > 0 && g->IH > 0 && g->IW > 0 && g->Cin > 0 && g->OH > 0 && g->OW > 0 && g->Cout > 0,
              "conv geometry: non-positive extent");
  PCG_REQUIRE(g->KH > 0 && g->KW > 0 && g->stride > 0 && g->pad >= 0, "conv geometry: bad kernel/stride/pad");
  PCG_REQUIRE(g->OH == (g->IH + 2 * g->pad - g->KH) / g->stride + 1 && g->OW == (g->IW + 2 * g->pad - g->KW) / g->stride + 1,
              "conv geometry: OH/OW inconsistent with IH/IW, kernel %dx%d stride %d pad %d", g->KH, g->KW, g->stride, g->pad);
  PCG_REQUIRE((int64_t)g->B * g->IH * g->IW * g->Cin * 4 < (1ll << 31) && (int64_t)g->B * g->OH * g->OW * g->Cout * 4 < (1ll << 31) &&
                  (int64_t)g->Cout * g->KH * g->KW * g->Cin * 4 < (1ll << 31),
              "conv geometry: an operand tensor reaches 2 GiB (32-bit buffer offsets); split the batch");
  PCG_REQUIRE(g->KH * g->KW <= 32, "conv geometry: more than 32 taps (%dx%d) unsupported", g->KH, g->KW);
  return PCG_OK;
}

struct Tune { int edge_prio = -1, dgrad_swz3 = -1, wgrad_rounds = -1, korder = -1, wgrad_order = -1, dgrad_interleave = -1, fwd_splits = -1, stream_k = -1, sk_blocks = -1, dgrad_gemm = -1, t64 = -1, wgrad_pixtab = -1, pad_clip = -1, pad_clip_dgrad = -1; unsigned long long* stamps = nullptr; int stamp_slots = 0; };
Tune g_tune;

ConvP make_params(const pcg_conv_geom* g) {
  ConvP p{};
  static const int korder_env = getenv("PCG_KORDER") ? atoi(getenv("PCG_KORDER")) : 1;
  p.korder = g_tune.korder >= 0 ? g_tune.korder : korder_env;
  static const int edge_env = getenv("PCG_EDGE_PRIO") ? atoi(getenv("PCG_EDGE_PRIO")) : 2;
  p.edge_prio = g_tune.edge_prio >= 0 ? g_tune.edge_prio : edge_env;
  p.stamps = g_tune.stamps; p.stamp_slots = g_tune.stamp_slots;
  p.B = g->B; p.IH = g->IH; p.IW = g->IW; p.Cin = g->Cin; p.OH = g->OH; p.OW = g->OW; p.Cout = g->Cout;
  p.KH = g->KH; p.KW = g->KW; p.stride = g->stride; p.pad = g->pad;
  p.dOW = FastDiv((uint32_t)g->OW);
  p.dOH = FastDiv((uint32_t)g->OH);
  p.dOHW = FastDiv((uint32_t)(g->OH * g->OW));
  p.x_bytes = (uint32_t)((int64_t)g->B * g->IH * g->IW * g->Cin * 4);
  p.dy_bytes = (uint32_t)((int64_t)g->B * g->OH * g->OW * g->Cout * 4);
  p.w_bytes = (uint32_t)((int64_t)g->Cout * g->KH * g->KW * g->Cin * 4);
  return p;
}

int set_xform(const char* who, const pcg_in_xform* xf, int C, ConvP* p) {
  if (!xf || !xf->scale) return PCG_OK;
  PCG_REQUIRE(xf->shift != nullptr, "%s: input transform without shift", who);
  PCG_REQUIRE(xf->act == PCG_ACT_NONE || xf->act == PCG_ACT_RELU || xf->act == PCG_ACT_LRELU,
              "%s: input transform activation %d is not none / ReLU / LeakyReLU", who, xf->act);
  PCG_REQUIRE(C % 4 == 0 && (((uintptr_t)xf->scale | (uintptr_t)xf->shift) & 15) == 0,
              "%s: input transform needs a channel count %% 4 == 0 and 16-byte aligned scale / shift", who);
  p->in_sc = xf->scale; p->in_sh = xf->shift; p->in_neg = act_neg_of(xf->act, xf->slope); p->in_c_bytes = (uint32_t)C * 4u;
  return PCG_OK;
}

template <class Cfg, bool AK, bool BK_>
constexpr size_t smem_bytes() {
  constexpr int a = igemm_smem_floats<Cfg, AK, BK_>(), b = epilogue_smem_floats<Cfg>();
  return sizeof(float) * (size_t)(a > b ? a : b);
}

template <class K>
int set_smem(K kernel, size_t bytes) {
  hipError_t e = hipFuncSetAttribute(reinterpret_cast<const void*>(kernel), hipFuncAttributeMaxDynamicSharedMemorySize, (int)bytes);
  if (e != hipSuccess) { set_error("hipFuncSetAttribute(max dynamic LDS=%zu): %s", bytes, hipGetErrorString(e)); return PCG_ERR_LAUNCH; }
  return PCG_OK;
}

constexpr int SK_MAX_BLOCKS = 512, SK_MAX_TILES = 4096;
constexpr size_t SK_PARTS_BYTES = (size_t)2 * SK_MAX_BLOCKS * 128 * 128 * sizeof(float);
constexpr size_t SK_ARRIVALS_BYTES = (size_t)SK_MAX_TILES * 4 * sizeof(int);
struct SkScratch { int device; hipStream_t stream; float* parts; int* arrivals; };
SkScratch g_sk_scratch[64];
int g_sk_scratch_n = 0;
std::mutex g_sk_mutex;
int current_device() { int d = 0; return hipGetDevice(&d) == hipSuccess ? d : 0; }
bool sk_scratch_of(hipStream_t s, SkPlan* sk) {
  const int dev = current_device();
  std::lock_guard<std::mutex> lock(g_sk_mutex);
  for (int i = 0; i < g_sk_scratch_n; ++i)
    if (g_sk_scratch[i].stream == s && g_sk_scratch[i].device == dev) {
      if (sk) { sk->parts = g_sk_scratch[i].parts; sk->arrivals = g_sk_scratch[i].arrivals; }
      return true;
    }
  return false;
}
struct PixTabReg { int device, IH, IW, OH, OW, stride, pad, KH, KW, Cin; const uint32_t* tab; };
constexpr int PIXTAB_MAX = 256;
PixTabReg g_pixtab[PIXTAB_MAX];
int g_pixtab_n = 0;
std::mutex g_pixtab_mutex;
bool pixtab_same(const PixTabReg& r, int dev, const pcg_conv_geom* g) {
  return r.device == dev && r.IH == g->IH && r.IW == g->IW && r.OH == g->OH && r.OW == g->OW && r.stride == g->stride && r.pad == g->pad &&
         r.KH == g->KH && r.KW == g->KW && r.Cin == g->Cin;
}
const uint32_t* pixtab_of(const pcg_conv_geom* g) {
  static const int env = getenv("PCG_WGRAD_PIXTAB") ? atoi(getenv("PCG_WGRAD_PIXTAB")) : 1;
  if (!(g_tune.wgrad_pixtab >= 0 ? g_tune.wgrad_pixtab : env)) return nullptr;
  std::lock_guard<std::mutex> lock(g_pixtab_mutex);
  if (g_pixtab_n == 0) return nullptr;
  const int dev = current_device();
  for (int i = 0; i < g_pixtab_n; ++i)
    if (pixtab_same(g_pixtab[i], dev, g)) return g_pixtab[i].tab;
  return nullptr;
}
struct ClipTabReg { int device, OH, OW; const uint32_t* tab; };
constexpr int CLIPTAB_MAX = 64;
ClipTabReg g_cliptab[CLIPTAB_MAX];
int g_cliptab_n = 0;
std::mutex g_clip_mutex;
int clip_mode() {
  static const int env = getenv("PCG_PAD_CLIP") ? atoi(getenv("PCG_PAD_CLIP")) : PCG_PAD_CLIP_DEFAULT;
  return g_tune.pad_clip >= 0 ? g_tune.pad_clip : env;
}
int clip_dgrad_mode() {
  static const int env0 = getenv("PCG_PAD_CLIP_DGRAD") ? atoi(getenv("PCG_PAD_CLIP_DGRAD")) : 1;
  static const int env = env0 >= 0 && env0 <= 2 ? env0 : 1;
  return g_tune.pad_clip_dgrad >= 0 ? g_tune.pad_clip_dgrad : env;
}
const uint32_t* cliptab_of(const pcg_conv_geom* g) {
  std::lock_guard<std::mutex> lock(g_clip_mutex);
  if (g_cliptab_n == 0) return nullptr;
  const int dev = current_device();
  for (int i = 0; i < g_cliptab_n; ++i)
    if (g_cliptab[i].device == dev && g_cliptab[i].OH == g->OH && g_cliptab[i].OW == g->OW) return g_cliptab[i].tab;
  return nullptr;
}
struct ClipShape { int form, OH, OW, B, tilesN, interleave, bm0, alt64; };
struct ClipPlan { bool take; int order, bm; double ratio; };
constexpr double CLIP_UNIT64 = 254.0 / (479.0 / 2.0) / 2.0;
constexpr double CLIP_TAKE = 0.95;
constexpr double CLIP_DGRAD_COST = 0.98;
constexpr double CLIP_TAKE_DGRAD = 1.0;
constexpr int CLIP_DGRAD_MIN_TILES = 512;
double clip_predict(const ClipShape& c, int bm, int order) {
  const int npos = c.OH * c.OW, tpp = c.B / bm, tilesM = npos * tpp, nph = c.form ? 4 : 1;
  const int per = (c.form && c.interleave ? nph : 1) * c.tilesN, gx = tilesM * per, gy = c.form && !c.interleave ? nph : 1;
  std::vector<uint32_t> tab(cliptab_words(c.OH, c.OW));
  cliptab_build(c.OH, c.OW, tab.data());
  std::vector<int> len((size_t)gx * gy);
  for (int y = 0; y < gy; ++y)
    for (int b = 0; b < gx; ++b) {
      uint32_t within, idx;
      clip_block_tile((uint32_t)b, (uint32_t)per, (uint32_t)tilesM, order < 0 ? 0 : order, gy > 1, (uint32_t)y, within, idx);
      const int py = c.form ? (c.interleave ? (int)(within % (uint32_t)nph) : y) : 0;
      len[(size_t)y * gx + b] = order < 0 ? (c.form ? 4 : 16) : clip_desc_taps(tab[(size_t)(c.form ? 1 + py : 0) * npos + idx / (uint32_t)tpp]);
    }
  return clip_sched_model(len.data(), (int)len.size()) * (bm == 64 ? CLIP_UNIT64 : 1.0) * (c.form && order >= 0 ? CLIP_DGRAD_COST : 1.0);
}
ClipPlan plan_clip(const ClipShape& c) {
  static std::map<std::array<int, 9>, ClipPlan> cache;
  const int mode = clip_mode();
  const std::array<int, 9> key = {c.form, c.OH, c.OW, c.B, c.tilesN, c.interleave, c.bm0, c.alt64, mode};
  std::lock_guard<std::mutex> lock(g_clip_mutex);
  auto it = cache.find(key);
  if (it != cache.end()) return it->second;
  ClipPlan best{false, 0, c.bm0, 1.0};
  const double t0 = clip_predict(c, c.B % c.bm0 ? 64 : c.bm0, -1);
  if (mode >= 2) {
    const bool rows64 = mode >= 5 && c.alt64 && c.B % 64 == 0 && (c.OH * c.OW * (c.B / 64)) % 8 == 0;
    best = ClipPlan{true, (mode - 2) % 3, rows64 ? 64 : c.bm0, 0.0};
    best.ratio = clip_predict(c, best.bm, best.order) / t0;
  } else {
    for (int h = 0; h < 2; ++h) {
      const int bm = h ? 64 : 128;
      if (bm != c.bm0 && !(bm == 64 && c.alt64)) continue;
      if (c.B % bm || (c.OH * c.OW * (c.B / bm)) % 8) continue;
      for (int order = 0; order < 3; ++order) {
        const double r = clip_predict(c, bm, order) / t0;
        if (r < best.ratio - 1e-9) best = ClipPlan{false, order, bm, r};
      }
    }
    const int blocks = c.OH * c.OW * (c.B / best.bm) * c.tilesN * (c.form ? 4 : 1);
    best.take = c.form ? best.ratio <= CLIP_TAKE_DGRAD + 1e-9 && blocks >= CLIP_DGRAD_MIN_TILES : best.ratio <= CLIP_TAKE + 1e-9;
  }
  cache[key] = best;
  return best;
// ... 54 lines not shown
      static int once_sk = set_smem(conv_fwd_sk_kernel<Cfg, XF>, smem);
      if (once_sk != PCG_OK) return once_sk;
      hipLaunchKernelGGL((conv_fwd_sk_kernel<Cfg, XF>), dim3((unsigned)(sk.dp_tiles + sk.sk_blocks)), dim3(IG_THREADS), smem, s, p, sk);
      return launch_status("conv_fwd_sk_kernel");
    }
  }
  static int once = set_smem(conv_fwd_kernel<Cfg, XF>, smem);
  if (once != PCG_OK) return once;
  hipLaunchKernelGGL((conv_fwd_kernel<Cfg, XF>), dim3((unsigned)tilesM * p.tilesN, splits), dim3(IG_THREADS), smem, s, p);
  return launch_status("conv_fwd_kernel");
}
template <class Cfg>
int launch_fwd(const ConvP& p, int splits, hipStream_t s) {
  if (conv_bf16()) return p.in_sc ? launch_fwd_x<Bf16Twin<Cfg>, true>(p, splits, s) : launch_fwd_x<Bf16Twin<Cfg>, false>(p, splits, s);
  return p.in_sc ? launch_fwd_x<Cfg, true>(p, splits, s) : launch_fwd_x<Cfg, false>(p, splits, s);
}

template <class Cfg, bool XF>
int launch_fwd_clip_x(ConvP p, hipStream_t s) {
  p.tilesN = ceil_div(p.N, Cfg::BN);
  constexpr size_t smem = smem_bytes<Cfg, true, true>();
  static int once = set_smem(conv_fwd_kernel<Cfg, XF, true>, smem);
  if (once != PCG_OK) return once;
  hipLaunchKernelGGL((conv_fwd_kernel<Cfg, XF, true>), dim3((unsigned)(p.clip_npos * p.clip_tpp * p.tilesN)), dim3(IG_THREADS), smem, s, p);
  return launch_status("conv_fwd_kernel (clipped)");
}
template <class Cfg>
int launch_fwd_clip(const ConvP& p, hipStream_t s) { return p.in_sc ? launch_fwd_clip_x<Cfg, true>(p, s) : launch_fwd_clip_x<Cfg, false>(p, s); }

struct FwdPlan { int splits, ktiles_per_split; };
FwdPlan plan_fwd(const pcg_conv_geom* g, int have_sk = -1) {
  if (have_sk < 0) have_sk = have_sk_scratch() ? 1 : 0;
  const int M = g->B * g->OH * g->OW, N = g->Cout;
  const int tiles = ceil_div(M, 128) * ceil_div(N, N > 64 ? 128 : 64);
  const int ktiles = g->KH * g->KW * ceil_div(g->Cin, IG_BK);
  FwdPlan f{1, ktiles};
  if (g_tune.fwd_splits > 0) {
    f.ktiles_per_split = ceil_div(ktiles, g_tune.fwd_splits);
    f.splits = ceil_div(ktiles, f.ktiles_per_split);
    return f;
  }
  if (tiles > 256 && tiles < 448 && ktiles >= 32 && !have_sk) {
    int best = 1;
    double bc = 2.0;
    for (int s = 2; s <= 4; ++s) {
      const double c = (double)ceil_div(tiles * s, 256) / s + 0.1 * s;
      if (c < bc - 1e-9) { bc = c; best = s; }
    }
    f.ktiles_per_split = ceil_div(ktiles, best);
    f.splits = ceil_div(ktiles, f.ktiles_per_split);
    return f;
  }
  if (tiles > 96 || ktiles < 32) return f;
  int splits = ceil_div(tiles >= 48 ? 512 : 384, tiles);
  if (splits > ktiles / 8) splits = ktiles / 8;
  if (splits < 2) return f;
  f.ktiles_per_split = ceil_div(ktiles, splits);
  f.splits = ceil_div(ktiles, f.ktiles_per_split);
  return f;
}

bool plan_skn_shape(const DgradPhases& ph, int nphases, int BM, int tilesN, int Cout, SkNPlan* sn) {
  if (sk_mode() == 0 || nphases < 2) return false;
  sn->nph = nphases;
  bool ok = true;
  int tiles = 0, total = 0, ktmax = 0;
  for (int i = 0; i < nphases && ok; ++i) {
    const int kt = ph.p[i].nth * ph.p[i].ntw * ceil_div(Cout, IG_BK), t = ceil_div(ph.p[i].Mp, BM) * tilesN;
    ok = ph.p[i].nth > 0 && ph.p[i].ntw > 0 && ph.p[i].Mp > 0 && kt > 0;
    sn->tile0[i] = tiles; sn->it0[i] = total; sn->kt[i] = kt;
    tiles += t; total += t * kt;
    if (kt > ktmax) ktmax = kt;
  }
  sn->tile0[nphases] = tiles; sn->it0[nphases] = total;
  int blocks = total / 512 >= 16 ? 512 : 256;
  if (g_tune.sk_blocks > 0) blocks = g_tune.sk_blocks;
  ok = ok && tiles <= SK_MAX_TILES && blocks <= SK_MAX_BLOCKS && total / blocks >= 8 && (int64_t)total * blocks < (1ll << 31) &&
       ktmax <= 8 * (total / blocks) && (sk_mode() == 2 || g_tune.sk_blocks > 0 || total >= 48 * tiles);
  sn->blocks = blocks; sn->total = total;
  return ok;
}

bool dgrad_interleaved(uint32_t w_bytes, const DgradPhases& ph, int nphases) {
  static const int il_env0 = getenv("PCG_DGRAD_INTERLEAVE") ? atoi(getenv("PCG_DGRAD_INTERLEAVE")) : 1;
  const int il_env = g_tune.dgrad_interleave >= 0 ? g_tune.dgrad_interleave : il_env0;
  bool same = nphases > 1 && il_env && w_bytes <= (1u << 20);
  for (int i = 1; i < nphases; ++i) same = same && ph.p[i].Mp == ph.p[0].Mp;
  return same;
}

template <class Cfg, bool XF>
int launch_dgrad_x(ConvP p, const DgradPhases& ph, int nphases, int maxMp, hipStream_t s) {
  p.tilesN = ceil_div(p.N, Cfg::BN);
  const int tilesM = ceil_div(maxMp, Cfg::BM);
  constexpr size_t smem = smem_bytes<Cfg, true, false>();
  if constexpr (!Cfg::BF16) {
    if (p.cliptab) {
      static int once_c = set_smem(conv_dgrad_kernel<Cfg, XF, true>, smem);
      if (once_c != PCG_OK) return once_c;
      DgradPhases phc = ph;
      phc.interleave = dgrad_interleaved(p.w_bytes, ph, nphases) ? nphases : 0;
      const unsigned tiles = (unsigned)(p.clip_npos * p.clip_tpp * p.tilesN);
      hipLaunchKernelGGL((conv_dgrad_kernel<Cfg, XF, true>), phc.interleave ? dim3(tiles * nphases) : dim3(tiles, nphases), dim3(IG_THREADS), smem, s, p, phc);
      return launch_status("conv_dgrad_kernel (clipped)");
    }
  }
  if constexpr (Cfg::BM == 128 && Cfg::BN == 128) {
    bool uniform = true;
    for (int i = 0; i < nphases; ++i)
      uniform = uniform && ph.p[i].Mp == ph.p[0].Mp && ph.p[i].nth * ph.p[i].ntw == ph.p[0].nth * ph.p[0].ntw && ph.p[i].nth > 0 && ph.p[i].ntw > 0;
    if (!uniform && nphases > 1 && sk_mode() != 0) {
      SkNPlan sn{};
      SkPlan scratch{};
      if (plan_skn_shape(ph, nphases, Cfg::BM, p.tilesN, p.Cout, &sn) && sk_scratch_of(s, &scratch)) {
        sn.parts = scratch.parts; sn.arrivals = scratch.arrivals;
        static int once_sn = set_smem(conv_dgrad_skn_kernel<Cfg, XF>, smem);
        if (once_sn != PCG_OK) return once_sn;
        DgradPhases phs = ph;
        phs.interleave = 0;
        hipLaunchKernelGGL((conv_dgrad_skn_kernel<Cfg, XF>), dim3((unsigned)sn.blocks), dim3(IG_THREADS), smem, s, p, phs, sn);
        return launch_status("conv_dgrad_skn_kernel");
      }
    }
    SkPlan sk{};
    const int tpp = tilesM * p.tilesN;
    if (uniform && plan_sk(tpp * nphases, ph.p[0].nth * ph.p[0].ntw * ceil_div(p.Cout, IG_BK), s, &sk)) {
      static int once_sk = set_smem(conv_dgrad_sk_kernel<Cfg, XF>, smem);
      if (once_sk != PCG_OK) return once_sk;
      DgradPhases phs = ph;
      phs.interleave = 0;
      hipLaunchKernelGGL((conv_dgrad_sk_kernel<Cfg, XF>), dim3((unsigned)(sk.dp_tiles + sk.sk_blocks)), dim3(IG_THREADS), smem, s, p, phs, sk, tpp);
      return launch_status("conv_dgrad_sk_kernel");
    }
  }
  static int once = set_smem(conv_dgrad_kernel<Cfg, XF>, smem);
  if (once != PCG_OK) return once;
  DgradPhases phl = ph;
  const bool same = dgrad_interleaved(p.w_bytes, ph, nphases);
  phl.interleave = same ? nphases : 0;
  if (same)
    hipLaunchKernelGGL((conv_dgrad_kernel<Cfg, XF>), dim3((unsigned)tilesM * p.tilesN * nphases), dim3(IG_THREADS), smem, s, p, phl);
  else
    hipLaunchKernelGGL((conv_dgrad_kernel<Cfg, XF>), dim3((unsigned)tilesM * p.tilesN, nphases), dim3(IG_THREADS), smem, s, p, phl);
  return launch_status("conv_dgrad_kernel");
}
template <class Cfg>
int launch_dgrad(const ConvP& p, const DgradPhases& ph, int nphases, int maxMp, hipStream_t s) {
  if (conv_bf16())
    return p.in_sc ? launch_dgrad_x<Bf16Twin<Cfg>, true>(p, ph, nphases, maxMp, s) : launch_dgrad_x<Bf16Twin<Cfg>, false>(p, ph, nphases, maxMp, s);
  return p.in_sc ? launch_dgrad_x<Cfg, true>(p, ph, nphases, maxMp, s) : launch_dgrad_x<Cfg, false>(p, ph, nphases, maxMp, s);
}

struct WgradPlan { int splits, ktiles_total, ktiles_per_split, tiles; bool narrow, wide192; };

WgradPlan plan_wgrad(const pcg_conv_geom* g) {
  WgradPlan w{};
  const int M = g->Cout, N = g->KH * g->KW * g->Cin;
  w.narrow = (M <= 64);
  static const int t192_env = getenv("PCG_WGRAD_192") ? atoi(getenv("PCG_WGRAD_192")) : 1;
  w.wide192 = w.narrow && t192_env && N % 192 == 0 && (N % 128) != 0;
  const int BM = w.narrow ? 64 : 128;
  w.tiles = ceil_div(M, BM) * (w.wide192 ? N / 192 : ceil_div(N, 128));
  const int64_t K = (int64_t)g->B * g->OH * g->OW;
  w.ktiles_total = (int)ceil_div64(K, IG_BK);
  const int slots = 512 * (g_tune.wgrad_rounds > 0 ? g_tune.wgrad_rounds : 1);
  int splits = w.tiles <= slots ? slots / w.tiles : 1;
  const int max_splits = w.ktiles_total / 8 > 0 ? w.ktiles_total / 8 : 1;
  if (splits > max_splits) splits = max_splits;
  if (splits < 1) splits = 1;
  auto cost = [&](int s, int* s_eff) {
    const int kps = ceil_div(w.ktiles_total, s), se = ceil_div(w.ktiles_total, kps);
    const int n = ceil_div(w.tiles * se, 256);
    *s_eff = se;
    return (double)n * kps * (w.wide192 ? 1.5 : w.narrow ? 1.0 : 1.95) * (n == 1 ? 1.2 : 1.0) + (double)se * M * N * 8.0 / 4.0e6;
  };
  int se = 0;
  const double c0 = cost(splits, &se);
  double cb = c0;
  int sb = splits;
  for (int s = 1; s <= max_splits && s <= 64; ++s) {
    const double c = cost(s, &se);
    if (se == s && c < cb * 0.98) { cb = c; sb = s; }
  }
  if (cb < 0.95 * c0) splits = sb;
  w.ktiles_per_split = ceil_div(w.ktiles_total, splits);
  w.splits = ceil_div(w.ktiles_total, w.ktiles_per_split);
  return w;
}

}
}

using namespace pcg;

extern "C" size_t pcg_conv2d_fwd_workspace_bytes(const pcg_conv_geom* g) {
  if (check_geom(g) != PCG_OK) return 0;
  if (thin_is_cin(g) || thin_is_cout(g)) return thin_conv_fwd_workspace_bytes(g);
  const FwdPlan f = plan_fwd(g);
  return f.splits > 1 ? (size_t)f.splits * g->B * g->OH * g->OW * g->Cout * sizeof(float) : 0;
}
static bool dgrad_as_gemm(const pcg_conv_geom* g, int have_sk = -1) {
  if (have_sk < 0) have_sk = have_sk_scratch() ? 1 : 0;
  if (thin_is_cin(g) || thin_is_cout(g)) return false;
  if (g_tune.dgrad_gemm == 0) return false;
  if (g_tune.dgrad_gemm < 0 && have_sk && g->stride == 2) {
    int64_t phase_macs = 0;
    for (int a = 0; a < 2; ++a)
      for (int b = 0; b < 2; ++b) {
        const int PHh = a < g->IH ? (g->IH - a + 1) / 2 : 0, PHw = b < g->IW ? (g->IW - b + 1) / 2 : 0;
        const int kh0 = (a + g->pad) % 2, kw0 = (b + g->pad) % 2;
        const int nth = kh0 < g->KH ? (g->KH - kh0 + 1) / 2 : 0, ntw = kw0 < g->KW ? (g->KW - kw0 + 1) / 2 : 0;
        phase_macs += (int64_t)PHh * PHw * nth * ntw;
      }
    if (phase_macs * 20 <= (int64_t)g->OH * g->OW * g->KH * g->KW * 19) return false;
  }
  if (g->stride < 2 || (g->KH % g->stride == 0 && g->KW % g->stride == 0)) return false;
  if (g->Cout < 512 || g->Cin % 4 || g->Cout % 4) return false;
  const int64_t bytes = (int64_t)g->B * g->OH * g->OW * g->KH * g->KW * g->Cin * 4;
  return bytes < (1ll << 31);
}
static size_t dgrad_gemm_bytes(const pcg_conv_geom* g) { return (size_t)g->B * g->OH * g->OW * g->KH * g->KW * g->Cin * sizeof(float); }

extern "C" size_t pcg_conv_scratch_parts_bytes(void) { return pcg::SK_PARTS_BYTES; }
extern "C" size_t pcg_conv_scratch_arrivals_bytes(void) { return pcg::SK_ARRIVALS_BYTES; }
extern "C" int pcg_conv_set_scratch(pcg_stream_t stream, void* parts, size_t parts_bytes, void* arrivals, size_t arrivals_bytes) {
  using namespace pcg;
  hipStream_t s = (hipStream_t)stream;
  const int dev = current_device();
  std::lock_guard<std::mutex> lock(g_sk_mutex);
  int at = -1;
  for (int i = 0; i < g_sk_scratch_n; ++i) if (g_sk_scratch[i].stream == s && g_sk_scratch[i].device == dev) at = i;
  if (!parts) {
    if (at >= 0) g_sk_scratch[at] = g_sk_scratch[--g_sk_scratch_n];
    return PCG_OK;
  }
  PCG_REQUIRE(arrivals != nullptr && parts_bytes >= SK_PARTS_BYTES && arrivals_bytes >= SK_ARRIVALS_BYTES,
              "pcg_conv_set_scratch: parts %zu B (need %zu), arrivals %zu B (need %zu)", parts_bytes, SK_PARTS_BYTES, arrivals_bytes, SK_ARRIVALS_BYTES);
  PCG_REQUIRE((((uintptr_t)parts) & 15) == 0 && (((uintptr_t)arrivals) & 3) == 0, "pcg_conv_set_scratch: misaligned scratch");
  if (at < 0) {
    PCG_REQUIRE(g_sk_scratch_n < 64, "pcg_conv_set_scratch: more than 64 streams with scratch");
    at = g_sk_scratch_n++;
  }
  g_sk_scratch[at] = SkScratch{dev, s, (float*)parts, (int*)arrivals};
  return PCG_OK;
}
extern "C" int pcg_conv_reset_scratch(pcg_stream_t stream) {
  using namespace pcg;
  SkPlan sk{};
  if (!sk_scratch_of((hipStream_t)stream, &sk)) return PCG_OK;
  hipError_t e = hipMemsetAsync(sk.arrivals, 0, SK_ARRIVALS_BYTES, (hipStream_t)stream);
  if (e != hipSuccess) { set_error("pcg_conv_reset_scratch: %s", hipGetErrorString(e)); return PCG_ERR_LAUNCH; }
  return PCG_OK;
}

extern "C" size_t pcg_conv_pixtab_bytes(const pcg_conv_geom* g) {
  if (check_geom(g) != PCG_OK) return 0;
  return pcg::pixtab_entries(g->OH, g->OW) * 2 * sizeof(uint32_t);
}
extern "C" int pcg_conv_pixtab_register(const pcg_conv_geom* g, void* host_out, size_t bytes, const void* device_table) {
  using namespace pcg;
  if (int e = check_geom(g)) return e;
  if (host_out) {
    PCG_REQUIRE(bytes >= pcg_conv_pixtab_bytes(g) && (((uintptr_t)host_out) & 3) == 0, "pcg_conv_pixtab_register: host buffer %zu B (need %zu), 4-byte aligned",
                bytes, pcg_conv_pixtab_bytes(g));
    pixtab_build(g->IH, g->IW, g->OH, g->OW, g->stride, g->pad, g->KH, g->KW, g->Cin, static_cast<uint32_t*>(host_out));
    if (!device_table) return PCG_OK;
  }
  PCG_REQUIRE((((uintptr_t)device_table) & 7) == 0, "pcg_conv_pixtab_register: misaligned table");
  const int dev = current_device();
  std::lock_guard<std::mutex> lock(g_pixtab_mutex);
  int at = -1;
  for (int i = 0; i < g_pixtab_n; ++i) if (pixtab_same(g_pixtab[i], dev, g)) at = i;
  if (!device_table) {
    if (at >= 0) g_pixtab[at] = g_pixtab[--g_pixtab_n];
    return PCG_OK;
  }
  if (at < 0) {
    PCG_REQUIRE(g_pixtab_n < PIXTAB_MAX, "pcg_conv_pixtab_register: more than %d geometries with a table", PIXTAB_MAX);
    at = g_pixtab_n++;
  }
  g_pixtab[at] = PixTabReg{dev, g->IH, g->IW, g->OH, g->OW, g->stride, g->pad, g->KH, g->KW, g->Cin, static_cast<const uint32_t*>(device_table)};
  return PCG_OK;
}

extern "C" size_t pcg_conv_cliptab_bytes(const pcg_conv_geom* g) {
  if (check_geom(g) != PCG_OK || !pcg::clip_geom_ok(g->IH, g->IW, g->OH, g->OW, g->stride, g->pad, g->KH, g->KW)) return 0;
  return pcg::cliptab_words(g->OH, g->OW) * sizeof(uint32_t);
}
extern "C" int pcg_conv_cliptab_register(const pcg_conv_geom* g, void* host_out, size_t bytes, const void* device_table) {
  using namespace pcg;
  if (int e = check_geom(g)) return e;
  const size_t need = pcg_conv_cliptab_bytes(g);
  PCG_REQUIRE(need > 0, "pcg_conv_cliptab_register: only k4 s2 p1 geometries with IH = 2 OH and IW = 2 OW have a tile table");
  if (host_out) {
    PCG_REQUIRE(bytes >= need && (((uintptr_t)host_out) & 3) == 0, "pcg_conv_cliptab_register: host buffer %zu B (need %zu), 4-byte aligned", bytes, need);
    cliptab_build(g->OH, g->OW, static_cast<uint32_t*>(host_out));
    if (!device_table) return PCG_OK;
  }
  PCG_REQUIRE((((uintptr_t)device_table) & 3) == 0, "pcg_conv_cliptab_register: misaligned table");
  const int dev = current_device();
  std::lock_guard<std::mutex> lock(g_clip_mutex);
  int at = -1;
  for (int i = 0; i < g_cliptab_n; ++i) if (g_cliptab[i].device == dev && g_cliptab[i].OH == g->OH && g_cliptab[i].OW == g->OW) at = i;
  if (!device_table) {
    if (at >= 0) g_cliptab[at] = g_cliptab[--g_cliptab_n];
    return PCG_OK;
// ... 422 lines not shown
  return launch_status("weight_adjoint_kernel");
}

extern "C" int pcg_conv2d_dgrad_add_bnsum(const pcg_conv_geom* g, const float* dy, const float* w, const float* addend, const float* z_next,
                                          const float* mean, const float* invstd, float sum_scale, float* dx, void* partial,
                                          size_t partial_bytes, pcg_stream_t stream) {
  EpiAux e{};
  e.mode = EPI_ADDSUM;
  if (int rc = check_geom(g)) return rc;
  e.no_addend = addend == nullptr;
  if (int rc = epi_common("pcg_conv2d_dgrad_add_bnsum", g, dx, addend ? addend : dx, PCG_ACT_NONE, 0.f, &e)) return rc;
  const size_t need = pcg_conv2d_dgrad_bn_workspace_bytes(g);
  PCG_REQUIRE(need > 0, "pcg_conv2d_dgrad_add_bnsum: layer not eligible (MFMA layers, stride <= 2, channel count %% 4 == 0)");
  PCG_REQUIRE(z_next && mean && invstd && (((uintptr_t)z_next | (uintptr_t)mean | (uintptr_t)invstd) & 15) == 0,
              "pcg_conv2d_dgrad_add_bnsum: z_next / mean / invstd must be non-null and 16-byte aligned");
  if (!partial || partial_bytes < need) { set_error("pcg_conv2d_dgrad_add_bnsum: partial-sum buffer %zu B < required %zu B", partial_bytes, need); return PCG_ERR_WORKSPACE; }
  e.neg = sum_scale;
  e.delta2_bytes = (int64_t)((intptr_t)z_next - (intptr_t)dx);
  e.mean = mean; e.invstd = invstd;
  return conv2d_dgrad_impl(g, dy, w, nullptr, dx, (double*)partial, nullptr, 0, stream, PCG_ACT_NONE, 0.f, &e);
}

static int bnbwd_epi(const char* who, const pcg_conv_geom* g, const float* out, const float* z_below, const float* mean, const float* invstd,
                     const float* gamma, const float* beta, int act, float slope, size_t need, void* partial, size_t partial_bytes,
                     EpiAux* e) {
  PCG_REQUIRE(need > 0, "%s: layer not eligible (MFMA layers, stride <= 2, channel count %% 4 == 0)", who);
  PCG_REQUIRE(mean && invstd && gamma && beta, "%s: null BatchNorm parameter", who);
  PCG_REQUIRE((((uintptr_t)mean | (uintptr_t)invstd | (uintptr_t)gamma | (uintptr_t)beta) & 15) == 0, "%s: BatchNorm vectors must be 16-byte aligned", who);
  if (!partial || partial_bytes < need) { set_error("%s: partial-sum buffer %zu B < required %zu B", who, partial_bytes, need); return PCG_ERR_WORKSPACE; }
  e->mode = EPI_BNBWD;
  e->mean = mean; e->invstd = invstd; e->gamma = gamma; e->beta = beta;
  return epi_common(who, g, out, z_below, act, slope, e);
}

extern "C" int pcg_conv2d_dgrad_bnbwd(const pcg_conv_geom* g, const float* dy, const float* w, const float* z_below, const float* mean,
                                      const float* invstd, const float* gamma, const float* beta, int act, float slope, float* dx,
                                      void* partial, size_t partial_bytes, pcg_stream_t stream) {
  EpiAux e{};
  if (int rc = check_geom(g)) return rc;
  if (int rc = bnbwd_epi("pcg_conv2d_dgrad_bnbwd", g, dx, z_below, mean, invstd, gamma, beta, act, slope,
                         pcg_conv2d_dgrad_bn_workspace_bytes(g), partial, partial_bytes, &e)) return rc;
  return conv2d_dgrad_impl(g, dy, w, nullptr, dx, (double*)partial, nullptr, 0, stream, PCG_ACT_NONE, 0.f, &e);
}
extern "C" int pcg_conv2d_fwd_bnbwd(const pcg_conv_geom* g, const float* x, const float* w, const float* z_below, const float* mean,
                                    const float* invstd, const float* gamma, const float* beta, int act, float slope, float* y,
                                    void* partial, size_t partial_bytes, pcg_stream_t stream) {
  EpiAux e{};
  if (int rc = check_geom(g)) return rc;
  if (int rc = bnbwd_epi("pcg_conv2d_fwd_bnbwd", g, y, z_below, mean, invstd, gamma, beta, act, slope,
                         pcg_conv2d_fwd_bn_workspace_bytes(g), partial, partial_bytes, &e)) return rc;
  return conv2d_fwd_impl(g, x, w, nullptr, y, (double*)partial, nullptr, 0, stream, PCG_ACT_NONE, 0.f, &e);
}
extern "C" int32_t pcg_conv2d_dgrad_bn_phases(const pcg_conv_geom* g) {
  if (check_geom(g) != PCG_OK) return 0;
  DgradPhases ph{};
  int maxMp = 0;
  return build_phases(g, &ph, &maxMp);
}
extern "C" int pcg_conv2d_dgrad_bnbwd_g(const pcg_conv_geom* g, const float* dy, const float* w, const float* z_below, const float* mean,
                                        const float* invstd, const float* gamma, const float* beta, int act, float slope, float* dx,
                                        void* partial, size_t partial_bytes, int32_t groups, pcg_stream_t stream) {
  EpiAux e{};
  if (int rc = check_geom(g)) return rc;
  if (int rc = bnbwd_epi("pcg_conv2d_dgrad_bnbwd_g", g, dx, z_below, mean, invstd, gamma, beta, act, slope,
                         pcg_conv2d_dgrad_bn_workspace_bytes(g), partial, partial_bytes, &e)) return rc;
  DgradPhases ph{};
  int maxMp = 0;
  const int nph = build_phases(g, &ph, &maxMp);
  bool ok = groups >= 1 && groups <= 8 && g->B % groups == 0 && nph > 0;
  for (int i = 0; i < nph && ok; ++i) ok = ph.p[i].Mp == maxMp;
  ok = ok && (maxMp / groups) % 128 == 0 && maxMp % groups == 0;
  PCG_REQUIRE(ok, "pcg_conv2d_dgrad_bnbwd_g: needs equal sub-pixel phases whose rows split into %d groups of whole 128-row tiles", groups);
  e.group_rows = groups > 1 ? maxMp / groups : 0;
  return conv2d_dgrad_impl(g, dy, w, nullptr, dx, (double*)partial, nullptr, 0, stream, PCG_ACT_NONE, 0.f, &e);
}
namespace pcg { bool dp_sync_bn(); }
extern "C" int32_t pcg_conv2d_fwd_bnbwd_thin_ok(const pcg_conv_geom* g) {
  return check_geom(g) == PCG_OK && !pcg::dp_sync_bn() && thin_conv_fwd_bnbwd_ok(g) && g->Cout % 4 == 0 ? 1 : 0;
}
extern "C" size_t pcg_conv2d_fwd_bnbwd_thin_workspace_bytes(const pcg_conv_geom* g) {
  return pcg_conv2d_fwd_bnbwd_thin_ok(g) ? thin_conv_fwd_bnbwd_workspace_bytes(g) : 0;
}
extern "C" int pcg_conv2d_fwd_bnbwd_thin(const pcg_conv_geom* g, const float* x, const float* w, const float* z_below, const float* mean,
                                         const float* invstd, const float* gamma, const float* beta, int act, float slope, float* dz,
                                         float* dgamma, float* dbeta, int accumulate, void* workspace, size_t workspace_bytes,
                                         pcg_stream_t stream) {
  if (int e = check_geom(g)) return e;
  PCG_REQUIRE(x && w && z_below && mean && invstd && gamma && beta && dz, "pcg_conv2d_fwd_bnbwd_thin: null pointer");
  PCG_REQUIRE(act == PCG_ACT_NONE || act == PCG_ACT_RELU || act == PCG_ACT_LRELU, "pcg_conv2d_fwd_bnbwd_thin: activation %d is not none / ReLU / LeakyReLU", act);
  PCG_REQUIRE(pcg_conv2d_fwd_bnbwd_thin_ok(g), "pcg_conv2d_fwd_bnbwd_thin: geometry not eligible (pcg_conv2d_fwd_bnbwd_thin_ok)");
  PCG_REQUIRE((((uintptr_t)z_below | (uintptr_t)dz) & 15) == 0, "pcg_conv2d_fwd_bnbwd_thin: tensors must be 16-byte aligned");
  return thin_conv_fwd_bnbwd(g, x, w, z_below, mean, invstd, gamma, beta, act, slope, dz, dgamma, dbeta, accumulate, workspace, workspace_bytes,
                             (hipStream_t)stream);
}
extern "C" int32_t pcg_conv2d_dgrad_bnbwd_full_ok(const pcg_conv_geom* g, int32_t groups) {
  return check_geom(g) == PCG_OK && !pcg::dp_sync_bn() && thin_conv_dgrad_bnbwd_full_ok(g, groups) ? 1 : 0;
}
extern "C" size_t pcg_conv2d_dgrad_bnbwd_full_workspace_bytes(const pcg_conv_geom* g, int32_t groups) {
  return pcg_conv2d_dgrad_bnbwd_full_ok(g, groups) ? thin_conv_dgrad_bnbwd_full_workspace_bytes(g, groups) : 0;
}
extern "C" int pcg_conv2d_dgrad_bnbwd_full(const pcg_conv_geom* g, const float* dy, const float* w, const float* z_below, const float* mean,
                                           const float* invstd, const float* gamma, const float* beta, int act, float slope, float* dz,
                                           float* dgamma, float* dbeta, int accumulate, int32_t groups, void* workspace, size_t workspace_bytes,
                                           pcg_stream_t stream) {
  if (int e = check_geom(g)) return e;
  PCG_REQUIRE(dy && w && z_below && mean && invstd && gamma && beta && dz, "pcg_conv2d_dgrad_bnbwd_full: null pointer");
  PCG_REQUIRE(act == PCG_ACT_NONE || act == PCG_ACT_RELU || act == PCG_ACT_LRELU, "pcg_conv2d_dgrad_bnbwd_full: activation %d is not none / ReLU / LeakyReLU", act);
  PCG_REQUIRE(pcg_conv2d_dgrad_bnbwd_full_ok(g, groups), "pcg_conv2d_dgrad_bnbwd_full: geometry / batch not eligible (pcg_conv2d_dgrad_bnbwd_full_ok)");
  PCG_REQUIRE((((uintptr_t)z_below | (uintptr_t)dz | (uintptr_t)w) & 15) == 0, "pcg_conv2d_dgrad_bnbwd_full: tensors must be 16-byte aligned");
  return thin_conv_dgrad_bnbwd_full(g, dy, w, z_below, mean, invstd, gamma, beta, act, slope, dz, dgamma, dbeta, accumulate, groups, workspace,
                                    workspace_bytes, (hipStream_t)stream);
}
extern "C" int32_t pcg_conv2d_bnin_full_ok(const pcg_conv_geom* g, int32_t groups) {
  return check_geom(g) == PCG_OK && thin_conv_bnin_full_ok(g, groups) ? 1 : 0;
}
static int bnin_args(const char* who, const pcg_conv_geom* g, const float* z, const float* mean, const float* invstd, const float* gamma, const float* beta,
                     int in_act, int32_t groups) {
  if (int e = check_geom(g)) return e;
  PCG_REQUIRE(z && mean && invstd && gamma && beta, "%s: null pointer", who);
  PCG_REQUIRE(in_act == PCG_ACT_NONE || in_act == PCG_ACT_RELU || in_act == PCG_ACT_LRELU, "%s: input activation %d is not none / ReLU / LeakyReLU", who, in_act);
  PCG_REQUIRE(pcg_conv2d_bnin_full_ok(g, groups), "%s: geometry / batch not eligible (pcg_conv2d_bnin_full_ok)", who);
  return PCG_OK;
}
extern "C" int pcg_conv2d_fwd_bnin_full(const pcg_conv_geom* g, const float* z, const float* mean, const float* invstd, const float* gamma,
                                        const float* beta, int in_act, float in_slope, int32_t groups, const float* w, const float* bias, int act,
                                        float slope, float* y, pcg_stream_t stream) {
  if (int e = bnin_args("pcg_conv2d_fwd_bnin_full", g, z, mean, invstd, gamma, beta, in_act, groups)) return e;
  PCG_REQUIRE(w && y && act >= PCG_ACT_NONE && act <= PCG_ACT_SIGMOID, "pcg_conv2d_fwd_bnin_full: bad arguments");
  const ThinBnIn bi{mean, invstd, gamma, beta, in_act, in_slope, groups};
  return thin_conv_fwd(g, z, w, bias, y, nullptr, 0, (hipStream_t)stream, act, slope, &bi);
}
extern "C" int pcg_conv2d_wgrad_bnin_full(const pcg_conv_geom* g, const float* z, const float* mean, const float* invstd, const float* gamma,
                                          const float* beta, int in_act, float in_slope, int32_t groups, const float* dy, float* dw, int accumulate,
                                          void* workspace, size_t workspace_bytes, pcg_stream_t stream) {
  if (int e = bnin_args("pcg_conv2d_wgrad_bnin_full", g, z, mean, invstd, gamma, beta, in_act, groups)) return e;
  PCG_REQUIRE(dy && dw, "pcg_conv2d_wgrad_bnin_full: null pointer");
  const ThinBnIn bi{mean, invstd, gamma, beta, in_act, in_slope, groups};
  return thin_conv_wgrad(g, z, dy, dw, accumulate, workspace, workspace_bytes, (hipStream_t)stream, nullptr, &bi);
}
extern "C" int32_t pcg_conv2d_fwd_bn_partial_rows(const pcg_conv_geom* g) { return check_geom(g) == PCG_OK ? fwd_stat_rows(g) : 0; }
extern "C" int32_t pcg_conv2d_dgrad_bn_partial_rows(const pcg_conv_geom* g) { return check_geom(g) == PCG_OK ? dgrad_stat_rows(g) : 0; }

extern "C" int pcg_slab_defer_begin(pcg_stream_t stream) { return slab_defer_begin((hipStream_t)stream); }
extern "C" int pcg_slab_defer_flush(pcg_stream_t stream) { return slab_defer_flush((hipStream_t)stream); }
extern "C" int32_t pcg_slab_defer_pending(void) { return slab_defer_pending(); }

extern "C" size_t pcg_conv2d_wgrad_workspace_bytes(const pcg_conv_geom* g) {
  if (check_geom(g) != PCG_OK) return 0;
  if (thin_is_cin(g) || thin_is_cout(g)) return thin_conv_wgrad_workspace_bytes(g);
  const WgradPlan w = plan_wgrad(g);
  return (size_t)w.splits * (size_t)g->Cout * (size_t)g->KH * g->KW * g->Cin * sizeof(float);
}

template <class Cfg, bool XFA, bool XFB, bool TAB = false>
static int launch_wgrad_x(const ConvP& p, const WgradPlan& wp, int slice_major, hipStream_t s) {
  if constexpr (!TAB) {
    if (p.pixtab) return launch_wgrad_x<Cfg, XFA, XFB, true>(p, wp, slice_major, s);
  }
  constexpr size_t smem = smem_bytes<Cfg, false, false>();
  static int once = set_smem(conv_wgrad_kernel<Cfg, XFA, XFB, TAB>, smem);
  if (once != PCG_OK) return once;
  hipLaunchKernelGGL((conv_wgrad_kernel<Cfg, XFA, XFB, TAB>), slice_major ? dim3((unsigned)wp.tiles * wp.splits) : dim3((unsigned)wp.tiles, wp.splits),
                     dim3(IG_THREADS), smem, s, p, wp.ktiles_total, wp.ktiles_per_split, wp.tiles, slice_major);
  return launch_status("conv_wgrad_kernel");
}
template <class Cfg, bool XFA, bool XFB, bool TAB = false>
static int launch_wgrad_sk_x(const ConvP& p, const SkPlan& sk, hipStream_t s) {
  if constexpr (!Cfg::BF16) {
    if (conv_bf16()) return launch_wgrad_sk_x<Bf16Twin<Cfg>, XFA, XFB>(p, sk, s);
  }
  if constexpr (!TAB) {
    if (p.pixtab) return launch_wgrad_sk_x<Cfg, XFA, XFB, true>(p, sk, s);
  }
  constexpr size_t smem = smem_bytes<Cfg, false, false>();
  static int once = set_smem(conv_wgrad_sk_kernel<Cfg, XFA, XFB, TAB>, smem);
  if (once != PCG_OK) return once;
  hipLaunchKernelGGL((conv_wgrad_sk_kernel<Cfg, XFA, XFB, TAB>), dim3((unsigned)(sk.dp_tiles + sk.sk_blocks)), dim3(IG_THREADS), smem, s, p, sk);
  return launch_status("conv_wgrad_sk_kernel");
}
template <class Cfg, bool TAB = false>
static int launch_wgrad192(const ConvP& p, const WgradPlan& wp, int slice_major, hipStream_t s) {
  if constexpr (!TAB) {
    if (p.pixtab) return launch_wgrad192<Cfg, true>(p, wp, slice_major, s);
  }
  constexpr size_t smem = smem_bytes<Cfg, false, false>();
  static int once = set_smem(conv_wgrad192_kernel<Cfg, TAB>, smem);
  if (once != PCG_OK) return once;
  hipLaunchKernelGGL((conv_wgrad192_kernel<Cfg, TAB>), slice_major ? dim3((unsigned)wp.tiles * wp.splits) : dim3((unsigned)wp.tiles, wp.splits),
                     dim3(IG_THREADS), smem, s, p, wp.ktiles_total, wp.ktiles_per_split, wp.tiles, slice_major);
  return launch_status("conv_wgrad192_kernel");
}
template <class Cfg>
static int launch_wgrad(const ConvP& p, const WgradPlan& wp, int slice_major, int xf_side, hipStream_t s) {
  if constexpr (!Cfg::BF16) {
    if (conv_bf16()) return launch_wgrad<Bf16Twin<Cfg>>(p, wp, slice_major, xf_side, s);
  }
  if (xf_side == 1) return launch_wgrad_x<Cfg, false, true>(p, wp, slice_major, s);
  if (xf_side == 2) return launch_wgrad_x<Cfg, true, false>(p, wp, slice_major, s);
  return launch_wgrad_x<Cfg, false, false>(p, wp, slice_major, s);
}

extern "C" int pcg_conv2d_wgrad_xf(const pcg_conv_geom* g, const float* x, const pcg_in_xform* xf_x, const float* dy,
                                   const pcg_in_xform* xf_dy, float* dw, int accumulate, void* workspace, size_t workspace_bytes,
                                   pcg_stream_t stream) {
  if (int e = check_geom(g)) return e;
  PCG_REQUIRE(x && dy && dw, "pcg_conv2d_wgrad: null pointer");
  const bool hx = xf_x && xf_x->scale, hy = xf_dy && xf_dy->scale;
  PCG_REQUIRE(!(hx && hy), "pcg_conv2d_wgrad_xf: at most one operand can carry an input transform");
  if (thin_is_cin(g) || thin_is_cout(g)) {
    PCG_REQUIRE(!hx && (!hy || thin_conv_xf_ok(g)), "pcg_conv2d_wgrad: input transforms on the MFMA path (Cin > 3 and Cout > 3) and, on the dy side, on the thin forms of pcg_conv2d_xf_thin_ok only");
    PCG_REQUIRE(!hy || (xf_dy->act == PCG_ACT_NONE || xf_dy->act == PCG_ACT_RELU || xf_dy->act == PCG_ACT_LRELU), "pcg_conv2d_wgrad: transform activation %d", hy ? xf_dy->act : 0);
    const ThinXf tx{hy ? xf_dy->scale : nullptr, hy ? xf_dy->shift : nullptr, hy ? act_neg_of(xf_dy->act, xf_dy->slope) : 1.f};
    return thin_conv_wgrad(g, x, dy, dw, accumulate, workspace, workspace_bytes, (hipStream_t)stream, &tx);
  }
  PCG_REQUIRE(g->Cin % 4 == 0 && g->Cout % 4 == 0, "pcg_conv2d_wgrad: Cin=%d and Cout=%d must be multiples of 4", g->Cin, g->Cout);
  const WgradPlan wp = plan_wgrad(g);
  const size_t need = pcg_conv2d_wgrad_workspace_bytes(g);
  if (workspace == nullptr || workspace_bytes < need) {
    set_error("pcg_conv2d_wgrad: workspace %zu B < required %zu B", workspace_bytes, need);
    return PCG_ERR_WORKSPACE;
  }
  PCG_REQUIRE(((uintptr_t)workspace & 15) == 0 && ((uintptr_t)dw & 15) == 0, "pcg_conv2d_wgrad: workspace/dw must be 16-byte aligned");
  ConvP p = make_params(g);
  p.x = x; p.dy = dy; p.out = (float*)workspace;
  p.M = g->Cout; p.N = g->KH * g->KW * g->Cin;
  p.tilesN = ceil_div(p.N, 128);
  p.pixtab = pixtab_of(g);
  if (int e = hx ? set_xform("pcg_conv2d_wgrad_xf", xf_x, g->Cin, &p) : set_xform("pcg_conv2d_wgrad_xf", xf_dy, g->Cout, &p)) return e;
  hipStream_t s = (hipStream_t)stream;
  static const int order_env0 = getenv("PCG_WGRAD_ORDER") ? atoi(getenv("PCG_WGRAD_ORDER")) : -1;
  const int order_env = g_tune.wgrad_order >= 0 ? g_tune.wgrad_order : order_env0;
  const int slice_major = order_env >= 0 ? order_env : (wp.tiles <= 8 ? 1 : 0);
  const int side = hx ? 1 : hy ? 2 : 0;
  if (!wp.narrow && !wp.wide192 && wp.tiles > 96 && sk_mode() != 0) {
    SkPlan sk{};
    bool take = plan_sk(wp.tiles, wp.ktiles_total, s, &sk);
    if (!take && wp.splits == 1) { sk = SkPlan{wp.tiles, 0, 0, wp.ktiles_total, nullptr, nullptr}; take = true; }
    if (take) {
      p.out = dw;
      if (accumulate) { p.epi.mode = EPI_ADD; p.epi.neg = 1.f; p.epi.delta_bytes = 0; }
      return side == 1 ? launch_wgrad_sk_x<Cfg128x128, false, true>(p, sk, s)
           : side == 2 ? launch_wgrad_sk_x<Cfg128x128, true, false>(p, sk, s) : launch_wgrad_sk_x<Cfg128x128, false, false>(p, sk, s);
    }
  }
  int rc;
  if (wp.wide192 && side == 0) {
    p.tilesN = p.N / 192;
    rc = conv_bf16() ? launch_wgrad192<Bf16Twin<Cfg64x192>>(p, wp, slice_major, s) : launch_wgrad192<Cfg64x192>(p, wp, slice_major, s);
  } else {
    WgradPlan wq = wp;
    if (wp.wide192) {
      wq.wide192 = false;
      wq.tiles = ceil_div(p.M, 64) * ceil_div(p.N, 128);
    }
    rc = wq.narrow ? launch_wgrad<TileCfg<64, 128, 1, 4>>(p, wq, slice_major, side, s) : launch_wgrad<Cfg128x128>(p, wq, slice_major, side, s);
  }
  if (rc != PCG_OK) return rc;
  const size_t n = (size_t)p.M * p.N;
  return launch_slab_reduce((const float*)workspace, dw, n, n, wp.splits, accumulate, s, true);
}

extern "C" int pcg_conv2d_wgrad(const pcg_conv_geom* g, const float* x, const float* dy, float* dw, int accumulate,
                                void* workspace, size_t workspace_bytes, pcg_stream_t stream) {
  return pcg_conv2d_wgrad_xf(g, x, nullptr, dy, nullptr, dw, accumulate, workspace, workspace_bytes, stream);
}

extern "C" int pcg_conv_plan_describe(const pcg_conv_geom* g, int32_t op, int32_t assume_scratch, char* out, size_t out_bytes) {
  if (int e = check_geom(g)) return e;
  PCG_REQUIRE(out && out_bytes > 0 && op >= 0 && op <= 2, "pcg_conv_plan_describe: bad arguments");
  const int have = assume_scratch ? (sk_mode() != 0 ? 1 : 0) : (have_sk_scratch() ? 1 : 0);
  char buf[512];
  buf[0] = 0;
  auto say = [&](const char* fmt, auto... a) { snprintf(buf + strlen(buf), sizeof(buf) - strlen(buf), fmt, a...); };
  if (thin_is_cin(g) || thin_is_cout(g)) {
    say("%s", "thin (Cin or Cout <= 3): no matrix-core launch");
  } else if (op == 0) {
    const int M = g->B * g->OH * g->OW, N = g->Cout, kt = g->KH * g->KW * ceil_div(g->Cin, IG_BK);
    const FwdPlan f = plan_fwd(g, have);
    SkPlan sk{};
    if (N <= 64) say("128x64 tiles: %d", ceil_div(M, 128));
    else if (fwd_use_t64(M, N, f.splits)) say("64x128 tiles: %d", ceil_div(M, 64) * ceil_div(N, 128));
    else if (f.splits == 1 && have && plan_sk_shape(ceil_div(M, 128) * ceil_div(N, 128), kt, &sk))
      say("stream-K: %d whole tiles + %d tiles x %d k-tiles over %d ranges", sk.dp_tiles, sk.sk_tiles, kt, sk.sk_blocks);
    else if (f.splits > 1) say("128x128 tiles: %d x %d K-slices of %d k-tiles (slabs)", ceil_div(M, 128) * ceil_div(N, 128), f.splits, f.ktiles_per_split);
    else say("128x128 tiles: %d", ceil_div(M, 128) * ceil_div(N, 128));
  } else if (op == 1) {
    if (dgrad_as_gemm(g, have)) {
      const int M = g->B * g->OH * g->OW, N = g->KH * g->KW * g->Cin, kt = ceil_div(g->Cout, IG_BK), tiles = ceil_div(M, 128) * ceil_div(N, 128);
      SkPlan sk{};
      say("%s", "GEMM + col2im: ");
      if (have && plan_sk_shape(tiles, kt, &sk)) say("stream-K: %d whole tiles + %d tiles x %d k-tiles over %d ranges", sk.dp_tiles, sk.sk_tiles, kt, sk.sk_blocks);
      else say("128x128 tiles: %d", tiles);
    } else {
      DgradPhases ph{};
      int maxMp = 0;
      const int nph = build_phases(g, &ph, &maxMp);
      const int N = g->Cin, tilesN = ceil_div(N, N > 64 ? 128 : 64);
      bool uniform = true;
      for (int i = 0; i < nph; ++i)
        uniform = uniform && ph.p[i].Mp == ph.p[0].Mp && ph.p[i].nth * ph.p[i].ntw == ph.p[0].nth * ph.p[0].ntw && ph.p[i].nth > 0 && ph.p[i].ntw > 0;
      SkNPlan sn{};
      SkPlan sk{};
      say("%d phase%s: ", nph, nph == 1 ? "" : "s");
      if (N > 64 && have && !uniform && plan_skn_shape(ph, nph, 128, tilesN, g->Cout, &sn))
        say("stream-K over unequal phases: %d tiles, %d k-tile iterations over %d ranges", sn.tile0[nph], sn.total, sn.blocks);
      else if (N > 64 && have && uniform && nph > 0 &&
               plan_sk_shape(ceil_div(maxMp, 128) * tilesN * nph, ph.p[0].nth * ph.p[0].ntw * ceil_div(g->Cout, IG_BK), &sk))
        say("stream-K: %d whole tiles + %d tiles over %d ranges", sk.dp_tiles, sk.sk_tiles, sk.sk_blocks);
      else say("%s tiles: %d per phase", N > 64 ? "128x128" : "128x64", ceil_div(maxMp, 128) * tilesN);
    }
  } else {
    const WgradPlan w = plan_wgrad(g);
    SkPlan sk{};
    if (!w.narrow && !w.wide192 && w.tiles > 96 && have && plan_sk_shape(w.tiles, w.ktiles_total, &sk))
      say("stream-K: %d whole tiles + %d tiles x %d k-tiles over %d ranges, dw written by the epilogue", sk.dp_tiles, sk.sk_tiles, w.ktiles_total, sk.sk_blocks);
    else if (!w.narrow && !w.wide192 && w.tiles > 96 && w.splits == 1 && sk_mode() != 0) say("128x128 tiles: %d, dw written by the epilogue", w.tiles);
    else say("%s tiles: %d x %d K-slices of %d k-tiles (slabs + slab_reduce)", w.wide192 ? "64x192" : w.narrow ? "64x128" : "128x128", w.tiles, w.splits, w.ktiles_per_split);
  }
  snprintf(out, out_bytes, "%s", buf);
  return PCG_OK;
}

extern "C" int pcg_conv_pad_clip_query(const pcg_conv_geom* g, int32_t op, int32_t groups, int32_t assume_scratch, int32_t* taken,
                                       int32_t* order, int32_t* tile_rows, double* predicted) {
  if (int e = check_geom(g)) return e;
  PCG_REQUIRE((op == 0 || op == 1) && groups >= 1, "pcg_conv_pad_clip_query: bad arguments");
  const int have = assume_scratch && sk_mode() != 0 ? 1 : 0;
  ClipPlan cp{false, 0, 0, 1.0};
  if (mfma_layer(g) && op == 0) {
    const int M = g->B * g->OH * g->OW, N = g->Cout, kt = g->KH * g->KW * ceil_div(g->Cin, IG_BK);
    const FwdPlan f = plan_fwd(g, have);
    const bool t64 = fwd_use_t64(M, N, f.splits);
    SkPlan sk{};
    const bool plain = f.splits == 1 && !(N > 64 && !t64 && have && plan_sk_shape(ceil_div(M, 128) * ceil_div(N, 128), kt, &sk));
    cp = clip_fwd_plan(g, groups, t64, plain);
  } else if (mfma_layer(g) && g->stride <= 2 && !dgrad_as_gemm(g, have)) {
    DgradPhases ph{};
    int maxMp = 0;
    const int nph = build_phases(g, &ph, &maxMp);
    SkPlan sk{};
    const bool plain = nph == 4 && !(g->Cin > 64 && have && plan_sk_shape(ceil_div(maxMp, 128) * ceil_div(g->Cin, 128) * nph, 4 * ceil_div(g->Cout, IG_BK), &sk));
    const uint32_t w_bytes = (uint32_t)((int64_t)g->Cout * g->KH * g->KW * g->Cin * 4);
    cp = clip_dgrad_plan(g, groups, dgrad_interleaved(w_bytes, ph, nph), plain);
  }
  if (taken) *taken = cp.take && cliptab_of(g) ? 1 : 0;
  if (order) *order = cp.order;
  if (tile_rows) *tile_rows = cp.bm;
  if (predicted) *predicted = cp.ratio;
  return PCG_OK;
}

extern "C" int pcg_tune_set(const char* name, int32_t value) {
  PCG_REQUIRE(name != nullptr, "pcg_tune_set: null name");
  if (!strcmp(name, "korder")) g_tune.korder = value;
  else if (!strcmp(name, "edge_prio")) g_tune.edge_prio = value;
  else if (!strcmp(name, "dgrad_swz3")) g_tune.dgrad_swz3 = value;
  else if (!strcmp(name, "wgrad_rounds")) g_tune.wgrad_rounds = value;
  else if (!strcmp(name, "wgrad_order")) g_tune.wgrad_order = value;
  else if (!strcmp(name, "dgrad_interleave")) g_tune.dgrad_interleave = value;
  else if (!strcmp(name, "fwd_splits")) g_tune.fwd_splits = value;
  else if (!strcmp(name, "stream_k")) g_tune.stream_k = value;
  else if (!strcmp(name, "sk_blocks")) g_tune.sk_blocks = value;
  else if (!strcmp(name, "dgrad_gemm")) g_tune.dgrad_gemm = value;
  else if (!strcmp(name, "t64")) g_tune.t64 = value;
  else if (!strcmp(name, "wgrad_pixtab")) g_tune.wgrad_pixtab = value;
  else if (!strcmp(name, "pad_clip")) g_tune.pad_clip = value;
  else if (!strcmp(name, "pad_clip_dgrad")) {
    PCG_REQUIRE(value >= -1 && value <= 2, "pcg_tune_set: pad_clip_dgrad is 0, 1 or 2 (-1: built-in), not %d", (int)value);
    g_tune.pad_clip_dgrad = value;
  }
  else {
    set_error("pcg_tune_set: unknown switch '%s' (korder, edge_prio, dgrad_swz3, wgrad_rounds, wgrad_order, dgrad_interleave, fwd_splits, "
              "stream_k, sk_blocks, dgrad_gemm, t64); the loader switches wgrad_pixtab, pad_clip and pad_clip_dgrad are accepted as well", name);
    return PCG_ERR_INVALID;
  }
  return PCG_OK;
}

extern "C" int pcg_debug_stamp_buffer(void* buf, int64_t bytes) {
  g_tune.stamps = static_cast<unsigned long long*>(buf);
  g_tune.stamp_slots = buf ? (int)(bytes / 16) : 0;
#ifdef PCG_CLOCK_STAMP
  return 1;
#else
  return 0;
#endif
}
```

### promptable-counterfactual-gan_amd/csrc/igemm_core.h

```cpp
#pragma once
#include "pcg_common.h"

namespace pcg {

typedef float f32x16 __attribute__((ext_vector_type(16)));

typedef unsigned int u32x4 __attribute__((ext_vector_type(4)));
using rsrc_t = __amdgpu_buffer_rsrc_t;
constexpr uint32_t OOB_OFF = 0x80000000u;

__device__ __forceinline__ rsrc_t make_rsrc(const void* p, uint32_t bytes) {
  return __builtin_amdgcn_make_buffer_rsrc(const_cast<void*>(p), 0, bytes, 0x00020000);
}
__device__ __forceinline__ float4 buf_load4(rsrc_t r, uint32_t off) {
  const u32x4 v = __builtin_amdgcn_raw_buffer_load_b128(r, off, 0, 0);
  return make_float4(__uint_as_float(v.x), __uint_as_float(v.y), __uint_as_float(v.z), __uint_as_float(v.w));
}

constexpr int IG_LOADERS = 256;
constexpr int IG_THREADS = 512;
constexpr int IG_BK = 32;
#ifndef PCG_PREFETCH_DEPTH
#define PCG_PREFETCH_DEPTH 2
#endif
// ... 211 lines not shown
  const unsigned long long loop_t0 = __builtin_amdgcn_s_memtime();
#endif
  int kt = 0;
  for (; kt + 4 < ktiles; kt += 2) {
    cs.sec_begin();
#ifdef PCG_CLOCK_STAMP
    asm volatile("s_waitcnt vmcnt(8)" ::: "memory");
    cs.sec_end(2);
#endif
    IA::store(As + IA::FLOATS, ra[1], tid);
    IB::store(Bs + IB::FLOATS, rb[1], tid);
    cs.sec_end(0);
    la.load_next(ra[1]); lb.load_next(rb[1]);
    cs.sec_end(1);
    cs.bar_begin(); lds_barrier(); cs.bar_end();
    cs.sec_begin();
#ifdef PCG_CLOCK_STAMP
    asm volatile("s_waitcnt vmcnt(8)" ::: "memory");
    cs.sec_end(2);
#endif
    IA::store(As, ra[0], tid);
    IB::store(Bs, rb[0], tid);
    cs.sec_end(0);
    la.load_next(ra[0]); lb.load_next(rb[0]);
    cs.sec_end(1);
    cs.bar_begin(); lds_barrier(); cs.bar_end();
  }
  for (; kt + 1 < ktiles; kt += 2) {
    la.transform(ra[1]); lb.transform(rb[1]);
    IA::store(As + IA::FLOATS, ra[1], tid);
    IB::store(Bs + IB::FLOATS, rb[1], tid);
    if (kt + 3 < ktiles) { la.load_next(ra[1]); lb.load_next(rb[1]); }
    cs.bar_begin(); lds_barrier(); cs.bar_end();
    if (kt + 2 < ktiles) {
      la.transform(ra[0]); lb.transform(rb[0]);
      IA::store(As, ra[0], tid);
      IB::store(Bs, rb[0], tid);
    }
    if (kt + 4 < ktiles) { la.load_next(ra[0]); lb.load_next(rb[0]); }
    cs.bar_begin(); lds_barrier(); cs.bar_end();
  }
  if (kt < ktiles) lds_barrier();
#ifdef PCG_CLOCK_STAMP
  cs.bar_flush(1, __builtin_amdgcn_s_memtime() - loop_t0);
#endif
  } else {
  float4 ra[IA::NV], rb[IB::NV];
  if (ktiles > 0) {
    la.load_next(ra);
    lb.load_next(rb);
    la.transform(ra); lb.transform(rb);
    IA::store(As, ra, tid);
    IB::store(Bs, rb, tid);
    if (ktiles > 1) {
      la.load_next(ra);
      lb.load_next(rb);
    }
  }
  lds_barrier();
  int nxt = 1;
  for (int kt = 0; kt < ktiles; ++kt) {
#ifndef PCG_ABL_PRODUCER_IDLE
    if (kt + 1 < ktiles) {
      la.transform(ra); lb.transform(rb);
      IA::store(As + nxt * IA::FLOATS, ra, tid);
      IB::store(Bs + nxt * IB::FLOATS, rb, tid);
    }
    if (kt + 2 < ktiles) {
      la.load_next(ra);
      lb.load_next(rb);
    }
#endif
    lds_barrier();
    nxt ^= 1;
  }
  }
}

template <bool BF> struct MmaFrag { float v[4]; };
template <> struct MmaFrag<true> { bf16x8 v; };

template <class Cfg, bool AK, bool BK_>
__device__ __forceinline__ void igemm_consume(int ktiles, f32x16 (&acc)[Cfg::TM][Cfg::TN], const float* smem, ClockStamp cs = ClockStamp{nullptr, 0}) {
  using IA = LdsImage<Cfg::BM, AK, Cfg::SWZ, Cfg::BF16>;
  using IB = LdsImage<Cfg::BN, BK_, Cfg::SWZ, Cfg::BF16>;
  constexpr int KG = IG_BK / (Cfg::BF16 ? 16 : 8);
  const float* As = smem;
  const float* Bs = smem + 2 * IA::FLOATS;
  const int lane = threadIdx.x & 63, wave = threadIdx.x >> 6;
  const int wm = wave / Cfg::WAVES_N, wn = wave % Cfg::WAVES_N;
  const int li = lane & 31, lh = lane >> 5;
  const int arow = wm * Cfg::WTM, brow = wn * Cfg::WTN;
#pragma unroll
  for (int i = 0; i < Cfg::TM; ++i)
#pragma unroll
    for (int j = 0; j < Cfg::TN; ++j)
#pragma unroll
      for (int r = 0; r < 16; ++r) acc[i][j][r] = 0.f;

  MmaFrag<Cfg::BF16> a[2][Cfg::TM], b[2][Cfg::TN];
  auto fetch = [&](const float* as, const float* bs, int ks, int buf) {
#pragma unroll
    for (int i = 0; i < Cfg::TM; ++i) IA::frag(as, arow + 32 * i, ks, li, lh, a[buf][i].v);
#pragma unroll
    for (int j = 0; j < Cfg::TN; ++j) IB::frag(bs, brow + 32 * j, ks, li, lh, b[buf][j].v);
  };
  auto mma = [&](int buf) {
    if constexpr (Cfg::BF16) {
#pragma unroll
      for (int i = 0; i < Cfg::TM; ++i)
#pragma unroll
        for (int j = 0; j < Cfg::TN; ++j)
          acc[i][j] = __builtin_amdgcn_mfma_f32_32x32x16_bf16(a[buf][i].v, b[buf][j].v, acc[i][j], 0, 0, 0);
    } else {
#pragma unroll
      for (int t = 0; t < 4; ++t)
#pragma unroll
        for (int i = 0; i < Cfg::TM; ++i)
#pragma unroll
          for (int j = 0; j < Cfg::TN; ++j)
            acc[i][j] = __builtin_amdgcn_mfma_f32_32x32x2f32(a[buf][i].v[t], b[buf][j].v[t], acc[i][j], 0, 0, 0);
    }
  };

  lds_barrier();
  if (ktiles <= 0) return;
  __builtin_amdgcn_s_setprio(PCG_CONSUMER_PRIO);
  cs.begin(); cs.phase(1); cs.bar_init();
#ifdef PCG_CLOCK_STAMP
  const unsigned long long loop_t0 = __builtin_amdgcn_s_memtime();
#endif
  fetch(As, Bs, 0, 0);
  int cur = 0;
#if PCG_CONSUMER_ALTERNATE
  const int alt_phase = (int)((blockIdx.x / PCG_CONSUMER_ALTERNATE) & 1u);
#endif
  for (int kt = 0; kt < ktiles; ++kt) {
#if PCG_CONSUMER_ALTERNATE
    if ((kt + alt_phase) & 1) __builtin_amdgcn_s_setprio(2); else __builtin_amdgcn_s_setprio(1);
#endif
    const float* as = As + cur * IA::FLOATS;
    const float* bs = Bs + cur * IB::FLOATS;
#pragma unroll
    for (int ks = 0; ks < KG - 1; ++ks) {
      fetch(as, bs, ks + 1, (ks + 1) & 1);
      mma(ks & 1);
    }
    cs.bar_begin();
    lds_barrier();
    cs.bar_end();
    cur ^= 1;
    if (kt + 1 < ktiles) fetch(As + cur * IA::FLOATS, Bs + cur * IB::FLOATS, 0, KG & 1);
    mma((KG - 1) & 1);
  }
  cs.end(); cs.phase(2);
#ifdef PCG_CLOCK_STAMP
  cs.bar_flush(0, __builtin_amdgcn_s_memtime() - loop_t0);
#endif
  __builtin_amdgcn_s_setprio(0);
}

template <class Cfg>
constexpr int epilogue_smem_floats() { return 4 * Cfg::WTM * (Cfg::WTN + 4); }

enum { EPI_NONE = 0, EPI_MASK = 1, EPI_BNBWD = 2, EPI_ADD = 3, EPI_ADDSUM = 4 };
struct EpiAux {
  int mode;
  float neg;
  int64_t delta_bytes;
  int64_t delta2_bytes;
  const float* mean; const float* invstd; const float* gamma; const float* beta;
  int no_addend;
  int group_rows;
};

__device__ __forceinline__ void epi_store4(float* p, float4 v) { *reinterpret_cast<float4*>(p) = v; }

template <class Cfg, class RowBase>
__device__ __forceinline__ void igemm_store_tile(f32x16 (&acc)[Cfg::TM][Cfg::TN], float* smem, int n_block, int N,
                                                 const float* bias, RowBase row_base, double* stat_row = nullptr, int act = PCG_ACT_NONE,
                                                 float slope = 0.f, const EpiAux* epi = nullptr, int stat_goff = 0) {
  constexpr int LDW = Cfg::WTN + 4;
  constexpr int Q = Cfg::WTN / 4;
  constexpr int RPI = 64 / Q;
  static_assert(Cfg::WTM % RPI == 0, "wave tile rows must be a multiple of the rows stored per instruction");
  const int lane = threadIdx.x & 63, wave = threadIdx.x >> 6;
  const int wm = wave / Cfg::WAVES_N, wn = wave % Cfg::WAVES_N, li = lane & 31, lh = lane >> 5;
  float* reg = smem + wave * (Cfg::WTM * LDW);
#pragma unroll
  for (int i = 0; i < Cfg::TM; ++i)
#pragma unroll
    for (int j = 0; j < Cfg::TN; ++j)
#pragma unroll
      for (int r = 0; r < 16; ++r) reg[(32 * i + acc_row(r, lh)) * LDW + 32 * j + li] = acc[i][j][r];
  asm volatile("s_waitcnt lgkmcnt(0)" ::: "memory");
  const int cq = lane % Q, r0 = lane / Q;
  const int n = n_block + wn * Cfg::WTN + 4 * cq;
  const bool nok = n < N && r0 < RPI;
  float4 bv = make_float4(0.f, 0.f, 0.f, 0.f);
  if (bias && nok) bv = *reinterpret_cast<const float4*>(bias + n);
  double s1[4] = {0.0, 0.0, 0.0, 0.0}, s2[4] = {0.0, 0.0, 0.0, 0.0};
  const bool want_sums = stat_row != nullptr;
  const int emode = epi ? epi->mode : EPI_NONE;
  if (emode == EPI_NONE) {
#pragma unroll
    for (int k = 0; k < Cfg::WTM / RPI; ++k) {
      const int row = r0 + RPI * k;
      float* dst = row_base(wm * Cfg::WTM + row);
      if (dst && nok) {
        float4 v = *reinterpret_cast<const float4*>(reg + row * LDW + 4 * cq);
        v.x += bv.x; v.y += bv.y; v.z += bv.z; v.w += bv.w;
        if (act != PCG_ACT_NONE) {
          v.x = act_neg_scale(v.x, slope); v.y = act_neg_scale(v.y, slope); v.z = act_neg_scale(v.z, slope); v.w = act_neg_scale(v.w, slope);
        }
        epi_store4(dst + wn * Cfg::WTN + 4 * cq, v);
        if (want_sums) {
          const double d0 = v.x, d1 = v.y, d2 = v.z, d3 = v.w;
          s1[0] += d0; s1[1] += d1; s1[2] += d2; s1[3] += d3;
          s2[0] = fma(d0, d0, s2[0]); s2[1] = fma(d1, d1, s2[1]); s2[2] = fma(d2, d2, s2[2]); s2[3] = fma(d3, d3, s2[3]);
        }
      }
    }
  } else {
    const float neg = epi->neg;
    const int64_t delta = epi->delta_bytes;
    float4 sc = make_float4(1.f, 1.f, 1.f, 1.f), sh = make_float4(0.f, 0.f, 0.f, 0.f), mu = sh, is = sc;
    if (emode == EPI_BNBWD && nok) {
      mu = *reinterpret_cast<const float4*>(epi->mean + stat_goff + n);
      is = *reinterpret_cast<const float4*>(epi->invstd + stat_goff + n);
      const float4 ga = *reinterpret_cast<const float4*>(epi->gamma + n), be = *reinterpret_cast<const float4*>(epi->beta + n);
      bn_fold(ga.x, be.x, mu.x, is.x, sc.x, sh.x); bn_fold(ga.y, be.y, mu.y, is.y, sc.y, sh.y);
      bn_fold(ga.z, be.z, mu.z, is.z, sc.z, sh.z); bn_fold(ga.w, be.w, mu.w, is.w, sc.w, sh.w);
    }
    if (emode == EPI_ADDSUM && nok) {
      mu = *reinterpret_cast<const float4*>(epi->mean + n);
      is = *reinterpret_cast<const float4*>(epi->invstd + n);
    }
    constexpr int NK = Cfg::WTM / RPI, CH = (NK >= 8 && Cfg::MINW < 6) ? NK / 2 : NK;
#pragma unroll
    for (int k0 = 0; k0 < NK; k0 += CH) {
    float4 u[CH];
#pragma unroll
    for (int kk = 0; kk < CH; ++kk) {
      float* dst = row_base(wm * Cfg::WTM + r0 + RPI * (k0 + kk));
      u[kk] = (dst && nok && !epi->no_addend) ? *reinterpret_cast<const float4*>(reinterpret_cast<const char*>(dst + wn * Cfg::WTN + 4 * cq) + delta)
                                              : make_float4(0.f, 0.f, 0.f, 0.f);
    }
    if (emode == EPI_ADDSUM) {
      const int64_t delta2 = epi->delta2_bytes;
      const double sc2 = (double)neg;
#pragma unroll
      for (int kk = 0; kk < CH; ++kk) {
        const int row = r0 + RPI * (k0 + kk);
        float* dst = row_base(wm * Cfg::WTM + row);
        if (dst && nok) {
          float4 v = *reinterpret_cast<const float4*>(reg + row * LDW + 4 * cq);
          const float4 z = *reinterpret_cast<const float4*>(reinterpret_cast<const char*>(dst + wn * Cfg::WTN + 4 * cq) + delta2);
          v.x += u[kk].x; v.y += u[kk].y; v.z += u[kk].z; v.w += u[kk].w;
          epi_store4(dst + wn * Cfg::WTN + 4 * cq, v);
          if (want_sums) {
            const double d0 = sc2 * (double)v.x, d1 = sc2 * (double)v.y, d2 = sc2 * (double)v.z, d3 = sc2 * (double)v.w;
            s1[0] += d0; s1[1] += d1; s1[2] += d2; s1[3] += d3;
            s2[0] = fma(d0, (double)((z.x - mu.x) * is.x), s2[0]); s2[1] = fma(d1, (double)((z.y - mu.y) * is.y), s2[1]);
            s2[2] = fma(d2, (double)((z.z - mu.z) * is.z), s2[2]); s2[3] = fma(d3, (double)((z.w - mu.w) * is.w), s2[3]);
          }
        }
      }
    } else {
#pragma unroll
    for (int kk = 0; kk < CH; ++kk) {
      const int row = r0 + RPI * (k0 + kk);
      float* dst = row_base(wm * Cfg::WTM + row);
      if (dst && nok) {
        float4 v = *reinterpret_cast<const float4*>(reg + row * LDW + 4 * cq);
        if (emode == EPI_ADD) {
          v.x += u[kk].x; v.y += u[kk].y; v.z += u[kk].z; v.w += u[kk].w;
          if (epi->delta2_bytes != 0) {
            const float4 a2 = *reinterpret_cast<const float4*>(reinterpret_cast<const char*>(dst + wn * Cfg::WTN + 4 * cq) + epi->delta2_bytes);
            v.x *= a2.x > 0.f ? 1.f : neg; v.y *= a2.y > 0.f ? 1.f : neg; v.z *= a2.z > 0.f ? 1.f : neg; v.w *= a2.w > 0.f ? 1.f : neg;
          }
        } else {
          const float4 pre = make_float4(fmaf(u[kk].x, sc.x, sh.x), fmaf(u[kk].y, sc.y, sh.y), fmaf(u[kk].z, sc.z, sh.z), fmaf(u[kk].w, sc.w, sh.w));
          v.x *= pre.x > 0.f ? 1.f : neg; v.y *= pre.y > 0.f ? 1.f : neg; v.z *= pre.z > 0.f ? 1.f : neg; v.w *= pre.w > 0.f ? 1.f : neg;
        }
        epi_store4(dst + wn * Cfg::WTN + 4 * cq, v);
        if (want_sums) {
          s1[0] += (double)v.x; s1[1] += (double)v.y; s1[2] += (double)v.z; s1[3] += (double)v.w;
          s2[0] = fma((double)v.x, (double)((u[kk].x - mu.x) * is.x), s2[0]); s2[1] = fma((double)v.y, (double)((u[kk].y - mu.y) * is.y), s2[1]);
          s2[2] = fma((double)v.z, (double)((u[kk].z - mu.z) * is.z), s2[2]); s2[3] = fma((double)v.w, (double)((u[kk].w - mu.w) * is.w), s2[3]);
        }
      }
    }
    }
    __builtin_amdgcn_sched_barrier(0);
    }
  }
  if (want_sums) {
#pragma unroll
    for (int off = Q; off < 64; off <<= 1) {
#pragma unroll
      for (int e = 0; e < 4; ++e) { s1[e] += __shfl_xor(s1[e], off); s2[e] += __shfl_xor(s2[e], off); }
    }
    if (r0 == 0 && nok) {
      double* pr = stat_row + (size_t)wm * 2 * N;
#pragma unroll
      for (int e = 0; e < 4; ++e) { pr[n + e] = s1[e]; pr[N + n + e] = s2[e]; }
// ... 7 lines not shown
```

### promptable-counterfactual-gan_amd/csrc/pcg_common.h

```cpp
#pragma once
#include <hip/hip_runtime.h>
#include <stdint.h>
#include <stddef.h>
#include "../../include/pcgan_hip.h"

#ifdef PCG_SEG_TIMING
extern __device__ unsigned long long* pcg_dbg_ts;
#define PCG_T(i) do { if (threadIdx.x == 0 && pcg_dbg_ts) pcg_dbg_ts[blockIdx.x * 16 + (i)] = wall_clock64(); } while (0)
#else
#define PCG_T(i) do { } while (0)
#endif

namespace pcg {

void set_error(const char* fmt, ...);
int launch_status(const char* what);
bool conv_bf16();

#define PCG_REQUIRE(cond, ...)                 \
  do {                                         \
    if (!(cond)) {                             \
      ::pcg::set_error(__VA_ARGS__);           \
      return PCG_ERR_INVALID;                  \
    }                                          \
  } while (0)

struct FastDiv {
  uint32_t d, mul, shr;
  __host__ __device__ FastDiv() : d(1), mul(0), shr(0) {}
  explicit FastDiv(uint32_t div) : d(div), mul(0), shr(0) {
    if (div > 1) {
      uint32_t l = 0;
      while ((1u << l) < div) ++l;
      const unsigned p = 31 + l;
      const uint64_t m = ((1ull << p) + div - 1) / div;
      mul = (uint32_t)m;
      shr = p - 32;
    }
  }
  __host__ __device__ __forceinline__ uint32_t div(uint32_t n) const {
#if defined(__HIP_DEVICE_COMPILE__)
    return mul ? (__umulhi(n, mul) >> shr) : n;
#else
    return mul ? (uint32_t)(((uint64_t)n * mul) >> 32) >> shr : n;
#endif
  }
  __host__ __device__ __forceinline__ void divmod(uint32_t n, uint32_t& q, uint32_t& r) const {
    q = div(n);
    r = n - q * d;
  }
};

__device__ __forceinline__ uint32_t xcd_remap(uint32_t bid, uint32_t nblocks) {
  const uint32_t q = nblocks >> 3, r = nblocks & 7u;
  const uint32_t xcd = bid & 7u, idx = bid >> 3;
  const uint32_t base = xcd < r ? xcd * (q + 1) : r * (q + 1) + (xcd - r) * q;
  return base + idx;
}

__device__ __forceinline__ float act_apply(float v, int act, float slope) {
  switch (act) {
    case PCG_ACT_RELU: return v > 0.f ? v : 0.f;
    case PCG_ACT_LRELU: return v > 0.f ? v : v * slope;
    case PCG_ACT_TANH: return tanhf(v);
    case PCG_ACT_SIGMOID: return 1.f / (1.f + expf(-v));
    default: return v;
  }
}
__device__ __forceinline__ float act_neg_scale(float v, float neg) { return v > 0.f ? v : v * neg; }
static inline bool act_is_cheap(int act) { return act == PCG_ACT_NONE || act == PCG_ACT_RELU || act == PCG_ACT_LRELU; }
static inline float act_neg_of(int act, float slope) { return act == PCG_ACT_RELU ? 0.f : act == PCG_ACT_LRELU ? slope : 1.f; }

__device__ __forceinline__ void bn_fold(float gamma, float beta, float mean, float invstd, float& sc, float& sh) {
  sc = gamma * invstd;
  sh = fmaf(-mean, sc, beta);
}

__device__ __forceinline__ float act_grad_from_out(float y, int act, float slope) {
  switch (act) {
    case PCG_ACT_RELU: return y > 0.f ? 1.f : 0.f;
    case PCG_ACT_LRELU: return y > 0.f ? 1.f : slope;
    case PCG_ACT_TANH: return 1.f - y * y;
    case PCG_ACT_SIGMOID: return y * (1.f - y);
    default: return 1.f;
  }
}

static inline int64_t ceil_div64(int64_t a, int64_t b) { return (a + b - 1) / b; }
static inline int ceil_div(int a, int b) { return (a + b - 1) / b; }

}
```

### promptable-counterfactual-gan_amd/ops.py

```python
import ctypes
import threading

import torch

from . import _lib
from ._lib import ACT_LRELU, ACT_NONE, ACT_RELU, ACT_SIGMOID, ACT_TANH, ConvGeom, check

_ws_cache = {}

_conv_hook = None


def set_conv_hook(hook):
    global _conv_hook
    _conv_hook = hook


def _conv_label(g, op):
    if g.Cin <= 3 or g.Cout <= 3:
        return f"thin_{op}"
    if op == "wgrad":
        n = g.KH * g.KW * g.Cin
        if g.Cout <= 64:
            return "conv_wgrad192_kernel<64x192>" if (n % 192 == 0 and n % 128 != 0) else "conv_wgrad_kernel<64x128>"
        return "conv_wgrad_kernel<128x128>"
    n = g.Cout if op == "fwd" else g.Cin
    if n > 64:
        return f"conv_{op}_kernel<128x128>"
    swz = op == "fwd" or g.stride == 1
    return f"conv_{op}_kernel<128x64{'/swz3' if swz else ''}>"


def _conv_flops(g):
    return 2.0 * g.B * g.OH * g.OW * g.Cout * g.KH * g.KW * g.Cin


class _Timed:
    def __init__(self, g, op):
        _conv_scratch()
        _conv_cliptab(g)
        self.on = _conv_hook is not None
        if self.on:
            self.g, self.op = g, op
            self.t0 = torch.cuda.Event(enable_timing=True)
            self.t1 = torch.cuda.Event(enable_timing=True)

    def __enter__(self):
        if self.on:
            self.t0.record()
        return self

    def __exit__(self, *exc):
        if self.on:
            self.t1.record()
            _conv_hook(_conv_label(self.g, self.op), _conv_flops(self.g), self.t0, self.t1)
        return False


_sk_streams = {}
_sk_pool = {}
_sk_arrival_pool = _sk_pool
_SK_SPARES = 2
_sk_last = None


def _stream():
    return ctypes.c_void_p(torch.cuda.current_stream().cuda_stream)


def prepare_conv_scratch(device_index=None):
    if device_index is None:
        device_index = torch.cuda.current_device()
    if torch.cuda.is_current_stream_capturing():
        return
    lib = _lib.load()
    dev = torch.device("cuda", device_index)
    nparts, narr = lib.pcg_conv_scratch_parts_bytes(), lib.pcg_conv_scratch_arrivals_bytes()
    pool = _sk_pool.setdefault(device_index, [])
    while len(pool) < _SK_SPARES:
        pool.append((torch.empty(nparts, dtype=torch.uint8, device=dev), torch.zeros(narr, dtype=torch.uint8, device=dev)))


def _conv_scratch():
    global _sk_last
    s = torch.cuda.current_stream()
    key = (s.device_index, s.cuda_stream)
    if key == _sk_last:
        return
    if key not in _sk_streams:
        capturing = torch.cuda.is_current_stream_capturing()
        if not capturing:
            prepare_conv_scratch(s.device_index)
        pool = _sk_pool.setdefault(s.device_index, [])
        if not pool:
            raise _lib.PcgError("conv call on a new stream inside a HIP-graph capture with no spare stream-K scratch left: call "
                                "pcgan_amd.ops.prepare_conv_scratch() on this device before capturing (the scratch must not come "
                                "from the graph's private memory pool)")
        parts, arrivals = pool.pop()
        lib = _lib.load()
        if lib.pcg_conv_set_scratch(ctypes.c_void_p(s.cuda_stream), _p(parts), parts.numel(), _p(arrivals), arrivals.numel()) == 0:
            _sk_streams[key] = (parts, arrivals)
        else:
            pool.append((parts, arrivals))
            _sk_streams[key] = None
        if not capturing:
            prepare_conv_scratch(s.device_index)
    _sk_last = key


_pixtabs = {}


def _pixtab_key(g, device_index):
    return (device_index, g.IH, g.IW, g.OH, g.OW, g.stride, g.pad, g.KH, g.KW, g.Cin)


def prepare_conv_pixtab(g, device=None):
    device = torch.device("cuda", torch.cuda.current_device()) if device is None else device
    key = _pixtab_key(g, device.index)
    if key in _pixtabs or torch.cuda.is_current_stream_capturing():
        return _pixtabs.get(key)
    lib = _lib.load()
    n = lib.pcg_conv_pixtab_bytes(ctypes.byref(g))
    host = torch.empty(n, dtype=torch.uint8)
    check(lib.pcg_conv_pixtab_register(ctypes.byref(g), _p(host), n, None), "pcg_conv_pixtab_register")
    with torch.cuda.device(device):
        tab = host.to(device)
        check(lib.pcg_conv_pixtab_register(ctypes.byref(g), None, 0, _p(tab)), "pcg_conv_pixtab_register")
    _pixtabs[key] = tab
    return tab


def drop_conv_pixtab(g, device=None):
    device = torch.device("cuda", torch.cuda.current_device()) if device is None else device
    with torch.cuda.device(device):
        check(_lib.load().pcg_conv_pixtab_register(ctypes.byref(g), None, 0, None), "pcg_conv_pixtab_register")
    _pixtabs[_pixtab_key(g, device.index)] = None


_cliptabs = {}


def _conv_cliptab(g):
    if g.KH != 4 or g.stride != 2 or g.pad != 1:
        return
    key = (torch.cuda.current_device(), g.OH, g.OW)
    if key in _cliptabs or torch.cuda.is_current_stream_capturing():
        return
    lib = _lib.load()
    n = lib.pcg_conv_cliptab_bytes(ctypes.byref(g))
    tab = None
    if n:
        host = torch.empty(n, dtype=torch.uint8)
        check(lib.pcg_conv_cliptab_register(ctypes.byref(g), _p(host), n, None), "pcg_conv_cliptab_register")
        tab = host.cuda()
        check(lib.pcg_conv_cliptab_register(ctypes.byref(g), None, 0, _p(tab)), "pcg_conv_cliptab_register")
    _cliptabs[key] = tab


def conv_pad_clip_query(g, op, groups=1, assume_scratch=True):
    taken, order, rows, pred = ctypes.c_int32(0), ctypes.c_int32(0), ctypes.c_int32(0), ctypes.c_double(1.0)
    check(_lib.load().pcg_conv_pad_clip_query(ctypes.byref(g), int(op), int(groups), int(bool(assume_scratch)), ctypes.byref(taken),
                                              ctypes.byref(order), ctypes.byref(rows), ctypes.byref(pred)), "pcg_conv_pad_clip_query")
    return bool(taken.value), order.value, rows.value, pred.value


def launch_plan(op, *args):
    buf = ctypes.create_string_buffer(256)
    arr = (ctypes.c_int64 * max(len(args), 1))(*[int(a) for a in args])
    check(_lib.load().pcg_launch_plan_describe(int(op), arr, len(args), buf, 256), "pcg_launch_plan_describe")
    return buf.value.decode()


def _p(t):
    return ctypes.c_void_p(t.data_ptr()) if t is not None else ctypes.c_void_p(0)


def _chk(t, name, dtype=torch.float32):
    if not t.is_cuda:
        raise _lib.PcgError(f"{name}: expected a tensor on the GPU (libpcgan_hip has no CPU path), got {t.device}")
    if t.dtype != dtype:
        raise _lib.PcgError(f"{name}: expected {dtype}, got {t.dtype}")
    if not t.is_contiguous():
        raise _lib.PcgError(f"{name}: expected a contiguous tensor, got strides {t.stride()} for shape {tuple(t.shape)}")
    return t


_ws_retired = []


def _scratch(kind, nbytes, device):
    stream = torch.cuda.current_stream(device).cuda_stream if device.type == "cuda" else 0
    key = (device.type, device.index, stream, kind)
    buf = _ws_cache.get(key)
    if buf is None or buf.numel() < nbytes:
        if buf is not None:
            _ws_retired.append(buf)
        buf = torch.empty(max(int(nbytes), 1 << 20), dtype=torch.uint8, device=device)
        _ws_cache[key] = buf
    return buf


def workspace(nbytes, device):
    return _scratch(0, nbytes, device)


def workspace2(nbytes, device):
    return _scratch(2, nbytes, device)


_ticket_pool = {}


def _ticket_buffer(device):
    stream = torch.cuda.current_stream(device).cuda_stream if device.type == "cuda" else 0
    key = (device.type, device.index, stream, "tickets")
    tk = _ws_cache.get(key)
    if tk is None:
        n = _lib.load().pcg_linear_wgrad_ticket_count()
        pool = _ticket_pool.setdefault((device.type, device.index), [])
        capturing = device.type == "cuda" and torch.cuda.is_current_stream_capturing()
        if not pool and not capturing:
            pool.extend(torch.zeros((8, n), dtype=torch.int32, device=device).unbind(0))
        tk = pool.pop() if pool else torch.zeros(n, dtype=torch.int32, device=device)
        _ws_cache[key] = tk
    return tk


def ohwi(w):
    v = w.permute(0, 2, 3, 1)
    if not v.is_contiguous():
        raise _lib.PcgError("conv weight is not in channels_last (OHWI) memory layout; FlatModule keeps it that way")
    return v


def conv_geom(B, IH, IW, Cin, Cout, KH, KW, stride, pad):
    OH = (IH + 2 * pad - KH) // stride + 1
    OW = (IW + 2 * pad - KW) // stride + 1
    return ConvGeom(B, IH, IW, Cin, OH, OW, Cout, KH, KW, stride, pad)


class InputXform:

    def __init__(self, coef, act, slope):
        C = coef.numel() // 2
        self.coef, self.act, self.slope, self.C = coef, int(act), float(slope), C
        self.c_struct = _lib.InXform(coef.data_ptr(), coef.data_ptr() + 4 * C, int(act), float(slope))

    def ref(self):
        return ctypes.byref(self.c_struct)


def xform_ok(g, operand):
    return g.Cin > 3 and g.Cout > 3 and g.Cin % 4 == 0 and g.Cout % 4 == 0 and g.stride <= 2


class BnInput:

    def __init__(self, mean, invstd, gamma, beta, act, slope, groups=1):
        self.mean, self.invstd, self.gamma, self.beta = mean, invstd, gamma, beta
        self.act, self.slope, self.groups = int(act), float(slope), int(groups)


def bnin_full_ok(g, groups=1):
    return bool(_lib.load().pcg_conv2d_bnin_full_ok(ctypes.byref(g), int(groups)))


def xform_thin_ok(g):
    return bool(_lib.load().pcg_conv2d_xf_thin_ok(ctypes.byref(g)))


def _xref(xf):
    return xf.ref() if xf is not None else None


def conv2d_fwd(g, x, w, bias=None, out=None, act=0, slope=0.0, xf=None):
    _chk(x, "x"); _chk(w, "w")
    assert x.numel() == g.B * g.IH * g.IW * g.Cin and w.numel() == g.Cout * g.KH * g.KW * g.Cin
    y = out if out is not None else torch.empty((g.B, g.OH, g.OW, g.Cout), dtype=torch.float32, device=x.device)
    lib = _lib.load()
    need = lib.pcg_conv2d_fwd_workspace_bytes(ctypes.byref(g))
    ws = workspace(need, x.device) if need else None
    with _Timed(g, "fwd"):
        if isinstance(xf, BnInput):
            check(lib.pcg_conv2d_fwd_bnin_full(ctypes.byref(g), _p(x), _p(xf.mean), _p(xf.invstd), _p(xf.gamma), _p(xf.beta), xf.act, xf.slope,
                                               xf.groups, _p(w), _p(bias), int(act), float(slope), _p(y), _stream()), "pcg_conv2d_fwd_bnin_full")
        elif xf is not None:
            assert xf.C == g.Cin
            check(lib.pcg_conv2d_fwd_xf(ctypes.byref(g), _p(x), xf.ref(), _p(w), _p(bias), int(act), float(slope), _p(y), _p(ws),
                                        ws.numel() if need else 0, _stream()), "pcg_conv2d_fwd_xf")
        else:
            check(lib.pcg_conv2d_fwd_act(ctypes.byref(g), _p(x), _p(w), _p(bias), int(act), float(slope), _p(y), _p(ws),
                                         ws.numel() if need else 0, _stream()), "pcg_conv2d_fwd_act")
    return y


def conv2d_dgrad(g, dy, w, bias_x=None, out=None, act=0, slope=0.0, xf=None):
    _chk(dy, "dy"); _chk(w, "w")
    assert dy.numel() == g.B * g.OH * g.OW * g.Cout and w.numel() == g.Cout * g.KH * g.KW * g.Cin
    dx = out if out is not None else torch.empty((g.B, g.IH, g.IW, g.Cin), dtype=torch.float32, device=dy.device)
    lib = _lib.load()
    need = lib.pcg_conv2d_dgrad_workspace_bytes(ctypes.byref(g))
    ws = workspace(need, dy.device) if need else None
    with _Timed(g, "dgrad"):
        if xf is not None:
            assert xf.C == g.Cout
            check(lib.pcg_conv2d_dgrad_xf(ctypes.byref(g), _p(dy), xf.ref(), _p(w), _p(bias_x), int(act), float(slope), _p(dx), _p(ws),
                                          ws.numel() if need else 0, _stream()), "pcg_conv2d_dgrad_xf")
        else:
            check(lib.pcg_conv2d_dgrad_act(ctypes.byref(g), _p(dy), _p(w), _p(bias_x), int(act), float(slope), _p(dx), _p(ws),
                                           ws.numel() if need else 0, _stream()), "pcg_conv2d_dgrad_act")
    return dx


def conv_bn_train(g, a, w, bias, transposed, eps, momentum, running_mean, running_var, num_batches_tracked, xf=None, gamma=None,
                  beta=None):
    _chk(a, "a"); _chk(w, "w")
# ... 1930 lines not shown
```

Before: 53560.

## Skip padded-zero MFMA steps in stride-2 4x4 wgrad and pair tile blocks

Adds a padding-skip variant of the wgrad consume loop for 4x4 stride-2 pad-1 convolutions. It statically drops the MFMA sub-steps for kernel taps that only ever read the zero border: whole taps when OW==4, and k-groups whose output row hits the padded edge otherwise. Because this leaves some blocks with less work than others, it also adds a host-side search for an XOR block-pairing bit that balances skipped and non-skipped tiles across co-scheduled blocks. The cost is more template instantiations and extra per-k-group branch logic in the inner loop. The default mode enables it only for OW<=8.

```diff
diff --git a/include/pcgan_hip.h b/include/pcgan_hip.h
--- a/include/pcgan_hip.h
+++ b/include/pcgan_hip.h
@@ -619,6 +619,8 @@
 double pcg_conv_sched_model(const int32_t* ktiles, int32_t n);
 int pcg_conv_pad_clip_query(const pcg_conv_geom* g, int32_t op, int32_t groups, int32_t assume_scratch, int32_t* taken, int32_t* order,
                             int32_t* tile_rows, double* predicted);
+int pcg_conv_wgrad_padskip_query(const pcg_conv_geom* g, int32_t op, int32_t* applies, double* fraction);
+int pcg_conv_wgrad_padskip_plan(const pcg_conv_geom* g, int32_t assume_scratch, int32_t* mode, int32_t* pair_bit);
 int pcg_debug_stamp_buffer(void* buf, int64_t bytes);
 
 typedef struct pcg_moons_cf_desc {
diff --git a/promptable-counterfactual-gan_amd/_lib.py b/promptable-counterfactual-gan_amd/_lib.py
--- a/promptable-counterfactual-gan_amd/_lib.py
+++ b/promptable-counterfactual-gan_amd/_lib.py
@@ -299,6 +299,8 @@
     "pcg_conv_cliptab_register": (_i, [_gp, _vp, _sz, _vp]),
     "pcg_conv_sched_model": (_d, [_vp, _i32]),
     "pcg_conv_pad_clip_query": (_i, [_gp, _i32, _i32, _i32, _vp, _vp, _vp, _vp]),
+    "pcg_conv_wgrad_padskip_query": (_i, [_gp, _i32, _vp, _vp]),
+    "pcg_conv_wgrad_padskip_plan": (_i, [_gp, _i32, _vp, _vp]),
     "pcg_conv2d_fwd_bn_g": (_i, [_gp, _vp, _vp, _vp, _vp, _f, _f, _vp, _vp, _vp, _vp, _vp, _i32, _vp, _sz, _vp]),
     "pcg_bn_apply_act_g": (_i, [_vp, _i64, _i32, _vp, _vp, _vp, _vp, _i, _f, _vp, _i32, _vp]),
     "pcg_conv2d_dgrad_bn_phases": (_i32, [_gp]),
diff --git a/promptable-counterfactual-gan_amd/csrc/conv_igemm.hip b/promptable-counterfactual-gan_amd/csrc/conv_igemm.hip
--- a/promptable-counterfactual-gan_amd/csrc/conv_igemm.hip
+++ b/promptable-counterfactual-gan_amd/csrc/conv_igemm.hip
@@ -2,6 +2,7 @@
 #include <array>
 #include <map>
 #include <mutex>
+#include <vector>
 #include "conv_loaders.h"
 #include "conv_pixtab.h"
 #include "conv_cliptab.h"
@@ -181,8 +182,7 @@
 __device__ __forceinline__ int sk_owner(int x, const SkPlan& sk) {
   return __builtin_amdgcn_readfirstlane((int)((((uint32_t)x + 1u) * (uint32_t)sk.sk_blocks - 1u) / (uint32_t)(sk.sk_tiles * sk.ktiles)));
 }
-__device__ __forceinline__ int sk_segments(const SkPlan& sk, SkSeg& s0, SkSeg& s1) {
-  const int b = blockIdx.x;
+__device__ __forceinline__ int sk_segments(const SkPlan& sk, SkSeg& s0, SkSeg& s1, int b) {
   if (b < sk.dp_tiles) { s0 = SkSeg{(int)xcd_remap((uint32_t)b, (uint32_t)sk.dp_tiles), 0, sk.ktiles, 1, 0}; return 1; }
   const int g = (int)xcd_remap((uint32_t)(b - sk.dp_tiles), (uint32_t)sk.sk_blocks), KT = sk.ktiles;
   const int it0 = sk_start(g, sk), it1 = sk_start(g + 1, sk);
@@ -252,8 +252,8 @@
   return true;
 }
 template <class Cfg>
-__device__ __forceinline__ bool sk_combine(const SkPlan& sk, const SkSeg& sg, f32x16 (&acc)[Cfg::TM][Cfg::TN]) {
-  const int g = (int)xcd_remap((uint32_t)((int)blockIdx.x - sk.dp_tiles), (uint32_t)sk.sk_blocks), j = sg.tile - sk.dp_tiles, KT = sk.ktiles;
+__device__ __forceinline__ bool sk_combine(const SkPlan& sk, const SkSeg& sg, f32x16 (&acc)[Cfg::TM][Cfg::TN], int b) {
+  const int g = (int)xcd_remap((uint32_t)(b - sk.dp_tiles), (uint32_t)sk.sk_blocks), j = sg.tile - sk.dp_tiles, KT = sk.ktiles;
   return sk_combine_core<Cfg>(sk.parts, sk.arrivals, sk.sk_blocks, g, j, sg.nparts, sg.first_block,
                               [&](int blk) { return sk_start(blk, sk) >= j * KT; }, acc);
 }
@@ -272,7 +272,7 @@
   }
   f32x16 acc[Cfg::TM][Cfg::TN];
   igemm_consume<Cfg, true, true>(sg.nkt, acc, smem);
-  if (sk_combine<Cfg>(sk, sg, acc))
+  if (sk_combine<Cfg>(sk, sg, acc, (int)blockIdx.x))
     igemm_store_tile<Cfg>(acc, smem, n_block, p.N, p.bias, [&](int row) -> float* {
       const int m = m_block + row;
       return m < p.M ? p.out + (size_t)m * p.N + n_block : nullptr;
@@ -282,7 +282,7 @@
 __global__ void __launch_bounds__(IG_THREADS, Cfg::MINW) conv_fwd_sk_kernel(ConvP p, SkPlan sk) {
   extern __shared__ __attribute__((aligned(16))) float smem[];
   SkSeg s0, s1{};
-  const int nseg = sk_segments(sk, s0, s1);
+  const int nseg = sk_segments(sk, s0, s1, (int)blockIdx.x);
   fwd_sk_segment<Cfg, XF>(p, sk, s0, smem);
   if (nseg == 1) return;
   lds_barrier();
@@ -317,7 +317,7 @@
   }
   f32x16 acc[Cfg::TM][Cfg::TN];
   igemm_consume<Cfg, true, false>(sg.nkt, acc, smem);
-  if (sk_combine<Cfg>(sk, sg, acc))
+  if (sk_combine<Cfg>(sk, sg, acc, (int)blockIdx.x))
     igemm_store_tile<Cfg>(acc, smem, n_block, p.N, p.bias, [&](int row) -> float* {
       const int pix = rowpix[row];
       return pix >= 0 ? p.out + (size_t)pix * p.Cin + n_block : nullptr;
@@ -328,20 +328,45 @@
   extern __shared__ __attribute__((aligned(16))) float smem[];
   __shared__ int rowpix[Cfg::BM];
   SkSeg s0, s1{};
-  const int nseg = sk_segments(sk, s0, s1);
+  const int nseg = sk_segments(sk, s0, s1, (int)blockIdx.x);
   dgrad_sk_segment<Cfg, XF>(p, phases, sk, s0, tiles_per_phase, smem, rowpix);
   if (nseg == 1) return;
   lds_barrier();
   dgrad_sk_segment<Cfg, XF>(p, phases, sk, s1, tiles_per_phase, smem, rowpix);
 }
 
-template <class Cfg, bool XFA, bool XFB, bool TAB = false>
+template <class Cfg>
+__device__ __forceinline__ PadSkip wgrad_padskip(const ConvP& p, int n_block, int kt_begin) {
+  const int wn = __builtin_amdgcn_readfirstlane((int)(threadIdx.x >> 6)) % Cfg::WAVES_N;
+  const int tap = __builtin_amdgcn_readfirstlane((int)((uint32_t)(n_block + wn * Cfg::WTN) / (uint32_t)p.Cin));
+  const int kh = tap >> 2, kw = tap & 3;
+  PadSkip ps;
+  ps.q0 = kt_begin * IG_BK;
+  ps.lgw = 31 - __builtin_clz((unsigned)p.OW); ps.ohm = p.OH - 1;
+  const bool w4 = p.OW == 4;
+  ps.tmask = w4 && tap < 16 ? (kw == 0 ? 1 : kw == 3 ? 8 : 0) : 0;
+  ps.oh_zero = w4 ? -1 : kh == 0 ? 0 : kh == 3 ? p.OH - 1 : -1;
+  return ps;
+}
+__device__ __forceinline__ uint32_t wgrad_pair_block(uint32_t b, uint32_t nblocks, int pair_xor) {
+  return ((b >> 8) & 1u) && (b | 255u) < nblocks ? b ^ (uint32_t)pair_xor : b;
+}
+
+template <class Cfg, bool XFA, bool XFB, bool TAB = false, int PS = 0>
 __global__ void __launch_bounds__(IG_THREADS, 4) conv_wgrad_kernel(ConvP p, int ktiles_total, int ktiles_per_split, int tiles,
-                                                                   int slice_major) {
+                                                                   int slice_major, int pair_xor) {
   extern __shared__ __attribute__((aligned(16))) float smem[];
   prio_entry(p);
   uint32_t tile, split;
-  if (slice_major) {
+  if constexpr (PS) {
+    const uint32_t b = wgrad_pair_block(blockIdx.x, gridDim.x, pair_xor);
+    if (slice_major) {
+      const uint32_t l = xcd_remap(b, gridDim.x);
+      split = l / (uint32_t)tiles; tile = l - split * (uint32_t)tiles;
+    } else {
+      split = b / (uint32_t)tiles; tile = xcd_remap(b - split * (uint32_t)tiles, (uint32_t)tiles);
+    }
+  } else if (slice_major) {
     const uint32_t l = xcd_remap(blockIdx.x, gridDim.x);
     split = l / (uint32_t)tiles; tile = l - split * (uint32_t)tiles;
   } else {
@@ -361,7 +386,8 @@
     return;
   }
   f32x16 acc[Cfg::TM][Cfg::TN];
-  igemm_consume<Cfg, false, false>(ktiles, acc, smem, ClockStamp{p.stamps, p.stamp_slots});
+  if constexpr (PS) igemm_consume_padskip<Cfg, false, false, PS>(ktiles, acc, smem, ClockStamp{p.stamps, p.stamp_slots}, wgrad_padskip<Cfg>(p, n_block, kt_begin));
+  else igemm_consume<Cfg, false, false>(ktiles, acc, smem, ClockStamp{p.stamps, p.stamp_slots});
   prio_epilogue(p);
   float* slab = p.out + (size_t)split * (size_t)p.M * (size_t)p.N;
   igemm_store_tile<Cfg>(acc, smem, n_block, p.N, nullptr, [&](int row) -> float* {
@@ -453,8 +479,8 @@
   }
 }
 
-template <class Cfg, bool XFA, bool XFB, bool TAB>
-__device__ __forceinline__ void wgrad_sk_segment(const ConvP& p, const SkPlan& sk, const SkSeg& sg, float* smem) {
+template <class Cfg, bool XFA, bool XFB, bool TAB, int PS>
+__device__ __forceinline__ void wgrad_sk_segment(const ConvP& p, const SkPlan& sk, const SkSeg& sg, float* smem, int b) {
   const int mt = __builtin_amdgcn_readfirstlane(sg.tile / p.tilesN), nt = sg.tile - mt * p.tilesN;
   const int m_block = mt * Cfg::BM, n_block = nt * Cfg::BN;
   if (wave_id() >= 4) {
@@ -465,22 +491,24 @@
     return;
   }
   f32x16 acc[Cfg::TM][Cfg::TN];
-  igemm_consume<Cfg, false, false>(sg.nkt, acc, smem);
-  if (sk_combine<Cfg>(sk, sg, acc))
+  if constexpr (PS) igemm_consume_padskip<Cfg, false, false, PS>(sg.nkt, acc, smem, ClockStamp{nullptr, 0}, wgrad_padskip<Cfg>(p, n_block, sg.kt_begin));
+  else igemm_consume<Cfg, false, false>(sg.nkt, acc, smem);
+  if (sk_combine<Cfg>(sk, sg, acc, b))
     igemm_store_tile<Cfg>(acc, smem, n_block, p.N, nullptr, [&](int row) -> float* {
       const int m = m_block + row;
       return m < p.M ? p.out + (size_t)m * p.N + n_block : nullptr;
     }, nullptr, PCG_ACT_NONE, 0.f, &p.epi);
 }
-template <class Cfg, bool XFA, bool XFB, bool TAB = false>
-__global__ void __launch_bounds__(IG_THREADS, 4) conv_wgrad_sk_kernel(ConvP p, SkPlan sk) {
+template <class Cfg, bool XFA, bool XFB, bool TAB = false, int PS = 0>
+__global__ void __launch_bounds__(IG_THREADS, 4) conv_wgrad_sk_kernel(ConvP p, SkPlan sk, int pair_xor) {
   extern __shared__ __attribute__((aligned(16))) float smem[];
   SkSeg s0, s1{};
-  const int nseg = sk_segments(sk, s0, s1);
-  wgrad_sk_segment<Cfg, XFA, XFB, TAB>(p, sk, s0, smem);
+  const int b = PS ? (int)wgrad_pair_block(blockIdx.x, gridDim.x, pair_xor) : (int)blockIdx.x;
+  const int nseg = sk_segments(sk, s0, s1, b);
+  wgrad_sk_segment<Cfg, XFA, XFB, TAB, PS>(p, sk, s0, smem, b);
   if (nseg == 1) return;
   lds_barrier();
-  wgrad_sk_segment<Cfg, XFA, XFB, TAB>(p, sk, s1, smem);
+  wgrad_sk_segment<Cfg, XFA, XFB, TAB, PS>(p, sk, s1, smem, b);
 }
 
 using Cfg64x192 = TileCfg<64, 192, 2, 2>;
@@ -582,7 +610,7 @@
   return PCG_OK;
 }
 
-struct Tune { int edge_prio = -1, dgrad_swz3 = -1, wgrad_rounds = -1, korder = -1, wgrad_order = -1, dgrad_interleave = -1, fwd_splits = -1, stream_k = -1, sk_blocks = -1, dgrad_gemm = -1, t64 = -1, wgrad_pixtab = -1, pad_clip = -1, pad_clip_dgrad = -1; unsigned long long* stamps = nullptr; int stamp_slots = 0; };
+struct Tune { int edge_prio = -1, dgrad_swz3 = -1, wgrad_rounds = -1, korder = -1, wgrad_order = -1, dgrad_interleave = -1, fwd_splits = -1, stream_k = -1, sk_blocks = -1, dgrad_gemm = -1, t64 = -1, wgrad_pixtab = -1, pad_clip = -1, pad_clip_dgrad = -1, wgrad_padskip = -1; unsigned long long* stamps = nullptr; int stamp_slots = 0; };
 Tune g_tune;
 
 ConvP make_params(const pcg_conv_geom* g) {
@@ -943,6 +971,55 @@
 }
 
 struct WgradPlan { int splits, ktiles_total, ktiles_per_split, tiles; bool narrow, wide192; };
+
+bool wgrad_padskip_geom(const pcg_conv_geom* g) {
+  auto pow2 = [](int v) { return v >= 4 && (v & (v - 1)) == 0; };
+  return g->KH == 4 && g->KW == 4 && g->stride == 2 && g->pad == 1 && g->IH == 2 * g->OH && g->IW == 2 * g->OW && pow2(g->OH) && pow2(g->OW) &&
+         g->Cin % 64 == 0 && !thin_is_cin(g) && !thin_is_cout(g);
+}
+double wgrad_padskip_fraction(const pcg_conv_geom* g) { return g->OW == 4 ? 0.125 : 0.5 / g->OH; }
+constexpr int WGRAD_PADSKIP_DEFAULT = 1;
+int wgrad_padskip_mode(const pcg_conv_geom* g) {
+  static const int env0 = getenv("PCG_WGRAD_PADSKIP") ? atoi(getenv("PCG_WGRAD_PADSKIP")) : WGRAD_PADSKIP_DEFAULT;
+  static const int env = env0 >= 0 && env0 <= 3 ? env0 : WGRAD_PADSKIP_DEFAULT;
+  const int v = g_tune.wgrad_padskip >= 0 ? g_tune.wgrad_padskip : env;
+  return v == 1 ? (g->OW <= 8 ? 2 : 0) : v == 2 ? 2 : v == 3 ? 1 : 0;
+}
+struct PairForm { int sk, n0, n1, n2, n3; };
+int wgrad_pair_xor(int waves_n, int wtn, int tilesN, int Cin, int OW, const PairForm& f) {
+  struct Entry { int key[10]; int bit; };
+  static std::vector<Entry> cache;
+  static std::mutex cache_mutex;
+  const int key[10] = {waves_n, wtn, tilesN, Cin, OW, f.sk, f.n0, f.n1, f.n2, f.n3};
+  std::lock_guard<std::mutex> lock(cache_mutex);
+  for (const Entry& e : cache)
+    if (!memcmp(e.key, key, sizeof(key))) return e.bit;
+  const int blocks = f.sk ? f.n0 + f.n2 : f.n0 * f.n1;
+  auto tile_of = [&](int b) {
+    if (!f.sk) return f.n2 ? (int)(xcd_remap((uint32_t)b, (uint32_t)blocks) % (uint32_t)f.n0) : (int)xcd_remap((uint32_t)(b % f.n0), (uint32_t)f.n0);
+    if (b < f.n0) return (int)xcd_remap((uint32_t)b, (uint32_t)f.n0);
+    const uint32_t g = xcd_remap((uint32_t)(b - f.n0), (uint32_t)f.n2);
+    return f.n0 + (int)(g * (uint32_t)(f.n1 * f.n3) / (uint32_t)f.n2 / (uint32_t)f.n3);
+  };
+  auto cls = [&](int b) {
+    const int nt = tile_of(b) % tilesN;
+    int c = 0;
+    for (int wn = 0; wn < waves_n; ++wn) {
+      const int tap = (nt * 128 + wn * wtn) / Cin, kh = tap >> 2, kw = tap & 3;
+      c += tap < 16 && (OW == 4 ? (kw == 0 || kw == 3) : (kh == 0 || kh == 3)) ? 1 : 0;
+    }
+    return c;
+  };
+  int best_m = 0, best = -1;
+  for (int m = 0; m <= 128; m = m ? 2 * m : 1) {
+    int score = 0;
+    for (int b = 256; (b | 255) < blocks; b += (b & 255) == 255 ? 257 : 1)
+      score += waves_n - abs(cls(b ^ m) + cls(b - 256) - waves_n);
+    if (score > best) { best = score; best_m = m; }
+  }
+  if (cache.size() < 256) cache.push_back(Entry{{key[0], key[1], key[2], key[3], key[4], key[5], key[6], key[7], key[8], key[9]}, best_m});
+  return best_m;
+}
 
 WgradPlan plan_wgrad(const pcg_conv_geom* g) {
   WgradPlan w{};
@@ -1671,30 +1748,55 @@
   return (size_t)w.splits * (size_t)g->Cout * (size_t)g->KH * g->KW * g->Cin * sizeof(float);
 }
 
-template <class Cfg, bool XFA, bool XFB, bool TAB = false>
-static int launch_wgrad_x(const ConvP& p, const WgradPlan& wp, int slice_major, hipStream_t s) {
+static int wgrad_slice_major(const WgradPlan& wp) {
+  static const int order_env0 = getenv("PCG_WGRAD_ORDER") ? atoi(getenv("PCG_WGRAD_ORDER")) : -1;
+  const int order_env = g_tune.wgrad_order >= 0 ? g_tune.wgrad_order : order_env0;
+  return order_env >= 0 ? order_env : (wp.tiles <= 8 ? 1 : 0);
+}
+template <class Cfg, bool XFA, bool XFB, bool TAB = false, int PS = 0>
+static int launch_wgrad_x(const ConvP& p, const WgradPlan& wp, int slice_major, hipStream_t s, int padskip = 0) {
   if constexpr (!TAB) {
-    if (p.pixtab) return launch_wgrad_x<Cfg, XFA, XFB, true>(p, wp, slice_major, s);
+    if (p.pixtab) return launch_wgrad_x<Cfg, XFA, XFB, true>(p, wp, slice_major, s, padskip);
+  }
+  if constexpr (!PS && !XFA && !XFB && !Cfg::BF16) {
+    if (padskip) return p.OW == 4 ? launch_wgrad_x<Cfg, XFA, XFB, TAB, 1>(p, wp, slice_major, s, padskip)
+                                  : launch_wgrad_x<Cfg, XFA, XFB, TAB, 2>(p, wp, slice_major, s, padskip);
   }
   constexpr size_t smem = smem_bytes<Cfg, false, false>();
-  static int once = set_smem(conv_wgrad_kernel<Cfg, XFA, XFB, TAB>, smem);
+  static int once = set_smem(conv_wgrad_kernel<Cfg, XFA, XFB, TAB, PS>, smem);
   if (once != PCG_OK) return once;
-  hipLaunchKernelGGL((conv_wgrad_kernel<Cfg, XFA, XFB, TAB>), slice_major ? dim3((unsigned)wp.tiles * wp.splits) : dim3((unsigned)wp.tiles, wp.splits),
-                     dim3(IG_THREADS), smem, s, p, wp.ktiles_total, wp.ktiles_per_split, wp.tiles, slice_major);
+  if constexpr (PS) {
+    const int blocks = wp.tiles * wp.splits;
+    static_assert(Cfg::BN == 128, "wgrad_pair_xor counts 128-column tiles");
+    const int px = padskip == 2 ? wgrad_pair_xor(Cfg::WAVES_N, Cfg::WTN, p.tilesN, p.Cin, p.OW, PairForm{0, wp.tiles, wp.splits, slice_major ? 1 : 0, 0}) : 0;
+    hipLaunchKernelGGL((conv_wgrad_kernel<Cfg, XFA, XFB, TAB, PS>), dim3((unsigned)blocks), dim3(IG_THREADS), smem, s, p, wp.ktiles_total,
+                       wp.ktiles_per_split, wp.tiles, slice_major, px);
+  } else {
+    hipLaunchKernelGGL((conv_wgrad_kernel<Cfg, XFA, XFB, TAB, PS>), slice_major ? dim3((unsigned)wp.tiles * wp.splits) : dim3((unsigned)wp.tiles, wp.splits),
+                       dim3(IG_THREADS), smem, s, p, wp.ktiles_total, wp.ktiles_per_split, wp.tiles, slice_major, 0);
+  }
   return launch_status("conv_wgrad_kernel");
 }
-template <class Cfg, bool XFA, bool XFB, bool TAB = false>
-static int launch_wgrad_sk_x(const ConvP& p, const SkPlan& sk, hipStream_t s) {
+template <class Cfg, bool XFA, bool XFB, bool TAB = false, int PS = 0>
+static int launch_wgrad_sk_x(const ConvP& p, const SkPlan& sk, hipStream_t s, int padskip = 0) {
   if constexpr (!Cfg::BF16) {
     if (conv_bf16()) return launch_wgrad_sk_x<Bf16Twin<Cfg>, XFA, XFB>(p, sk, s);
   }
   if constexpr (!TAB) {
-    if (p.pixtab) return launch_wgrad_sk_x<Cfg, XFA, XFB, true>(p, sk, s);
+    if (p.pixtab) return launch_wgrad_sk_x<Cfg, XFA, XFB, true>(p, sk, s, padskip);
+  }
+  if constexpr (!PS && !XFA && !XFB && !Cfg::BF16) {
+    if (padskip) return p.OW == 4 ? launch_wgrad_sk_x<Cfg, XFA, XFB, TAB, 1>(p, sk, s, padskip) : launch_wgrad_sk_x<Cfg, XFA, XFB, TAB, 2>(p, sk, s, padskip);
   }
   constexpr size_t smem = smem_bytes<Cfg, false, false>();
-  static int once = set_smem(conv_wgrad_sk_kernel<Cfg, XFA, XFB, TAB>, smem);
+  static int once = set_smem(conv_wgrad_sk_kernel<Cfg, XFA, XFB, TAB, PS>, smem);
   if (once != PCG_OK) return once;
-  hipLaunchKernelGGL((conv_wgrad_sk_kernel<Cfg, XFA, XFB, TAB>), dim3((unsigned)(sk.dp_tiles + sk.sk_blocks)), dim3(IG_THREADS), smem, s, p, sk);
+  const int blocks = sk.dp_tiles + sk.sk_blocks;
+  int px = 0;
+  if constexpr (PS) {
+    if (padskip == 2) px = wgrad_pair_xor(Cfg::WAVES_N, Cfg::WTN, p.tilesN, p.Cin, p.OW, PairForm{1, sk.dp_tiles, sk.sk_tiles, sk.sk_blocks, sk.ktiles});
+  }
+  hipLaunchKernelGGL((conv_wgrad_sk_kernel<Cfg, XFA, XFB, TAB, PS>), dim3((unsigned)blocks), dim3(IG_THREADS), smem, s, p, sk, px);
   return launch_status("conv_wgrad_sk_kernel");
 }
 template <class Cfg, bool TAB = false>
@@ -1710,13 +1812,13 @@
   return launch_status("conv_wgrad192_kernel");
 }
 template <class Cfg>
-static int launch_wgrad(const ConvP& p, const WgradPlan& wp, int slice_major, int xf_side, hipStream_t s) {
+static int launch_wgrad(const ConvP& p, const WgradPlan& wp, int slice_major, int xf_side, hipStream_t s, int padskip) {
   if constexpr (!Cfg::BF16) {
-    if (conv_bf16()) return launch_wgrad<Bf16Twin<Cfg>>(p, wp, slice_major, xf_side, s);
+    if (conv_bf16()) return launch_wgrad<Bf16Twin<Cfg>>(p, wp, slice_major, xf_side, s, 0);
   }
   if (xf_side == 1) return launch_wgrad_x<Cfg, false, true>(p, wp, slice_major, s);
   if (xf_side == 2) return launch_wgrad_x<Cfg, true, false>(p, wp, slice_major, s);
-  return launch_wgrad_x<Cfg, false, false>(p, wp, slice_major, s);
+  return launch_wgrad_x<Cfg, false, false>(p, wp, slice_major, s, padskip);
 }
 
 extern "C" int pcg_conv2d_wgrad_xf(const pcg_conv_geom* g, const float* x, const pcg_in_xform* xf_x, const float* dy,
@@ -1747,10 +1849,9 @@
   p.pixtab = pixtab_of(g);
   if (int e = hx ? set_xform("pcg_conv2d_wgrad_xf", xf_x, g->Cin, &p) : set_xform("pcg_conv2d_wgrad_xf", xf_dy, g->Cout, &p)) return e;
   hipStream_t s = (hipStream_t)stream;
-  static const int order_env0 = getenv("PCG_WGRAD_ORDER") ? atoi(getenv("PCG_WGRAD_ORDER")) : -1;
-  const int order_env = g_tune.wgrad_order >= 0 ? g_tune.wgrad_order : order_env0;
-  const int slice_major = order_env >= 0 ? order_env : (wp.tiles <= 8 ? 1 : 0);
+  const int slice_major = wgrad_slice_major(wp);
   const int side = hx ? 1 : hy ? 2 : 0;
+  const int padskip = wgrad_padskip_geom(g) ? wgrad_padskip_mode(g) : 0;
   if (!wp.narrow && !wp.wide192 && wp.tiles > 96 && sk_mode() != 0) {
     SkPlan sk{};
     bool take = plan_sk(wp.tiles, wp.ktiles_total, s, &sk);
@@ -1759,7 +1860,7 @@
       p.out = dw;
       if (accumulate) { p.epi.mode = EPI_ADD; p.epi.neg = 1.f; p.epi.delta_bytes = 0; }
       return side == 1 ? launch_wgrad_sk_x<Cfg128x128, false, true>(p, sk, s)
-           : side == 2 ? launch_wgrad_sk_x<Cfg128x128, true, false>(p, sk, s) : launch_wgrad_sk_x<Cfg128x128, false, false>(p, sk, s);
+           : side == 2 ? launch_wgrad_sk_x<Cfg128x128, true, false>(p, sk, s) : launch_wgrad_sk_x<Cfg128x128, false, false>(p, sk, s, padskip);
     }
   }
   int rc;
@@ -1772,7 +1873,7 @@
       wq.wide192 = false;
       wq.tiles = ceil_div(p.M, 64) * ceil_div(p.N, 128);
     }
-    rc = wq.narrow ? launch_wgrad<TileCfg<64, 128, 1, 4>>(p, wq, slice_major, side, s) : launch_wgrad<Cfg128x128>(p, wq, slice_major, side, s);
+    rc = wq.narrow ? launch_wgrad<TileCfg<64, 128, 1, 4>>(p, wq, slice_major, side, s, padskip) : launch_wgrad<Cfg128x128>(p, wq, slice_major, side, s, padskip);
   }
   if (rc != PCG_OK) return rc;
   const size_t n = (size_t)p.M * p.N;
@@ -1869,6 +1970,39 @@
   return PCG_OK;
 }
 
+extern "C" int pcg_conv_wgrad_padskip_query(const pcg_conv_geom* g, int32_t op, int32_t* applies, double* fraction) {
+  if (int e = check_geom(g)) return e;
+  PCG_REQUIRE(op >= 0 && op <= 2, "pcg_conv_wgrad_padskip_query: op is 0, 1 or 2, not %d", (int)op);
+  const bool yes = op == 2 && !conv_bf16() && wgrad_padskip_geom(g);
+  if (applies) *applies = yes ? 1 : 0;
+  if (fraction) *fraction = yes ? wgrad_padskip_fraction(g) : 0.0;
+  return PCG_OK;
+}
+
+extern "C" int pcg_conv_wgrad_padskip_plan(const pcg_conv_geom* g, int32_t assume_scratch, int32_t* mode, int32_t* pair_bit) {
+  if (int e = check_geom(g)) return e;
+  int m = 0, bit = 0;
+  if (!conv_bf16() && wgrad_padskip_geom(g)) {
+    m = wgrad_padskip_mode(g);
+    if (m == 2) {
+      const WgradPlan wp = plan_wgrad(g);
+      const int tilesN = ceil_div(g->KH * g->KW * g->Cin, 128);
+      const int have = assume_scratch ? (sk_mode() != 0 ? 1 : 0) : (have_sk_scratch() ? 1 : 0);
+      SkPlan sk{};
+      bool take = false;
+      if (!wp.narrow && !wp.wide192 && wp.tiles > 96 && sk_mode() != 0) {
+        take = have && plan_sk_shape(wp.tiles, wp.ktiles_total, &sk);
+        if (!take && wp.splits == 1) { sk = SkPlan{wp.tiles, 0, 0, wp.ktiles_total, nullptr, nullptr}; take = true; }
+      }
+      if (take) bit = wgrad_pair_xor(2, 64, tilesN, g->Cin, g->OW, PairForm{1, sk.dp_tiles, sk.sk_tiles, sk.sk_blocks, sk.ktiles});
+      else bit = wgrad_pair_xor(wp.narrow ? 4 : 2, wp.narrow ? 32 : 64, tilesN, g->Cin, g->OW, PairForm{0, wp.tiles, wp.splits, wgrad_slice_major(wp), 0});
+    }
+  }
+  if (mode) *mode = m;
+  if (pair_bit) *pair_bit = bit;
+  return PCG_OK;
+}
+
 extern "C" int pcg_tune_set(const char* name, int32_t value) {
   PCG_REQUIRE(name != nullptr, "pcg_tune_set: null name");
   if (!strcmp(name, "korder")) g_tune.korder = value;
@@ -1884,13 +2018,17 @@
   else if (!strcmp(name, "t64")) g_tune.t64 = value;
   else if (!strcmp(name, "wgrad_pixtab")) g_tune.wgrad_pixtab = value;
   else if (!strcmp(name, "pad_clip")) g_tune.pad_clip = value;
+  else if (!strcmp(name, "wgrad_padskip")) {
+    PCG_REQUIRE(value >= -1 && value <= 3, "pcg_tune_set: wgrad_padskip is 0, 1, 2 or 3 (-1: built-in), not %d", (int)value);
+    g_tune.wgrad_padskip = value;
+  }
   else if (!strcmp(name, "pad_clip_dgrad")) {
     PCG_REQUIRE(value >= -1 && value <= 2, "pcg_tune_set: pad_clip_dgrad is 0, 1 or 2 (-1: built-in), not %d", (int)value);
     g_tune.pad_clip_dgrad = value;
   }
   else {
     set_error("pcg_tune_set: unknown switch '%s' (korder, edge_prio, dgrad_swz3, wgrad_rounds, wgrad_order, dgrad_interleave, fwd_splits, "
-              "stream_k, sk_blocks, dgrad_gemm, t64); the loader switches wgrad_pixtab, pad_clip and pad_clip_dgrad are accepted as well", name);
+              "stream_k, sk_blocks, dgrad_gemm, t64); the loader switches wgrad_pixtab, pad_clip, pad_clip_dgrad and wgrad_padskip are accepted as well", name);
     return PCG_ERR_INVALID;
   }
   return PCG_OK;
diff --git a/promptable-counterfactual-gan_amd/csrc/igemm_core.h b/promptable-counterfactual-gan_amd/csrc/igemm_core.h
--- a/promptable-counterfactual-gan_amd/csrc/igemm_core.h
+++ b/promptable-counterfactual-gan_amd/csrc/igemm_core.h
@@ -387,6 +387,110 @@
     cur ^= 1;
     if (kt + 1 < ktiles) fetch(As + cur * IA::FLOATS, Bs + cur * IB::FLOATS, 0, KG & 1);
     mma((KG - 1) & 1);
+  }
+  cs.end(); cs.phase(2);
+#ifdef PCG_CLOCK_STAMP
+  cs.bar_flush(0, __builtin_amdgcn_s_memtime() - loop_t0);
+#endif
+  __builtin_amdgcn_s_setprio(0);
+}
+
+struct PadSkip {
+  int tmask;
+  int q0;
+  int lgw, ohm;
+  int oh_zero;
+};
+template <int V> struct IntC { static constexpr int value = V; };
+
+template <class Cfg, bool AK, bool BK_, int PS>
+__device__ __forceinline__ void igemm_consume_padskip(int ktiles, f32x16 (&acc)[Cfg::TM][Cfg::TN], const float* smem, ClockStamp cs = ClockStamp{nullptr, 0},
+                                                      PadSkip ps = PadSkip{0, 0, 0, 0, -1}) {
+  static_assert((PS == 1 || PS == 2) && !Cfg::BF16, "the padding skip is written for the fp32 k-groups of 8");
+  using IA = LdsImage<Cfg::BM, AK, Cfg::SWZ, Cfg::BF16>;
+  using IB = LdsImage<Cfg::BN, BK_, Cfg::SWZ, Cfg::BF16>;
+  constexpr int KG = IG_BK / (Cfg::BF16 ? 16 : 8);
+  const float* As = smem;
+  const float* Bs = smem + 2 * IA::FLOATS;
+  const int lane = threadIdx.x & 63, wave = threadIdx.x >> 6;
+  const int wm = wave / Cfg::WAVES_N, wn = wave % Cfg::WAVES_N;
+  const int li = lane & 31, lh = lane >> 5;
+  const int arow = wm * Cfg::WTM, brow = wn * Cfg::WTN;
+#pragma unroll
+  for (int i = 0; i < Cfg::TM; ++i)
+#pragma unroll
+    for (int j = 0; j < Cfg::TN; ++j)
+#pragma unroll
+      for (int r = 0; r < 16; ++r) acc[i][j][r] = 0.f;
+
+  MmaFrag<Cfg::BF16> a[2][Cfg::TM], b[2][Cfg::TN];
+  auto fetch = [&](const float* as, const float* bs, int ks, int buf) {
+#pragma unroll
+    for (int i = 0; i < Cfg::TM; ++i) IA::frag(as, arow + 32 * i, ks, li, lh, a[buf][i].v);
+#pragma unroll
+    for (int j = 0; j < Cfg::TN; ++j) IB::frag(bs, brow + 32 * j, ks, li, lh, b[buf][j].v);
+  };
+  auto mma = [&](int buf, auto T0, auto T1) {
+#pragma unroll
+    for (int t = T0.value; t < T1.value; ++t)
+#pragma unroll
+      for (int i = 0; i < Cfg::TM; ++i)
+#pragma unroll
+        for (int j = 0; j < Cfg::TN; ++j)
+          acc[i][j] = __builtin_amdgcn_mfma_f32_32x32x2f32(a[buf][i].v[t], b[buf][j].v[t], acc[i][j], 0, 0, 0);
+  };
+
+  lds_barrier();
+  if (ktiles <= 0) return;
+  __builtin_amdgcn_s_setprio(PCG_CONSUMER_PRIO);
+  cs.begin(); cs.phase(1); cs.bar_init();
+#ifdef PCG_CLOCK_STAMP
+  const unsigned long long loop_t0 = __builtin_amdgcn_s_memtime();
+#endif
+  auto dead = [&](int q, auto BR) {
+    int m = 0;
+    if constexpr (BR.value != 0) {
+#pragma unroll
+      for (int ks = 0; ks < KG; ++ks) m |= (((q + 8 * ks) >> ps.lgw) & ps.ohm) == ps.oh_zero ? 1 << ks : 0;
+    }
+    return m;
+  };
+#if PCG_CONSUMER_ALTERNATE
+  const int alt_phase = (int)((blockIdx.x / PCG_CONSUMER_ALTERNATE) & 1u);
+#endif
+  auto loop = [&](auto T0, auto T1, auto BR) {
+    int qt = ps.q0;
+    int dm = dead(qt, BR);
+    if (!(dm & 1)) fetch(As, Bs, 0, 0);
+    int cur = 0;
+    for (int kt = 0; kt < ktiles; ++kt) {
+#if PCG_CONSUMER_ALTERNATE
+      if ((kt + alt_phase) & 1) __builtin_amdgcn_s_setprio(2); else __builtin_amdgcn_s_setprio(1);
+#endif
+      const float* as = As + cur * IA::FLOATS;
+      const float* bs = Bs + cur * IB::FLOATS;
+      const int dn = dead(qt + IG_BK, BR);
+#pragma unroll
+      for (int ks = 0; ks < KG - 1; ++ks) {
+        if (!((dm >> (ks + 1)) & 1)) fetch(as, bs, ks + 1, (ks + 1) & 1);
+        if (!((dm >> ks) & 1)) mma(ks & 1, T0, T1);
+      }
+      cs.bar_begin();
+      lds_barrier();
+      cs.bar_end();
+      cur ^= 1;
+      if (kt + 1 < ktiles && !(dn & 1)) fetch(As + cur * IA::FLOATS, Bs + cur * IB::FLOATS, 0, KG & 1);
+      if (!((dm >> (KG - 1)) & 1)) mma((KG - 1) & 1, T0, T1);
+      qt += IG_BK; dm = dn;
+    }
+  };
+  if constexpr (PS == 1) {
+    if (ps.tmask == 1) loop(IntC<1>{}, IntC<4>{}, IntC<0>{});
+    else if (ps.tmask == 8) loop(IntC<0>{}, IntC<3>{}, IntC<0>{});
+    else loop(IntC<0>{}, IntC<4>{}, IntC<0>{});
+  } else {
+    if (ps.oh_zero >= 0) loop(IntC<0>{}, IntC<4>{}, IntC<1>{});
+    else loop(IntC<0>{}, IntC<4>{}, IntC<0>{});
   }
   cs.end(); cs.phase(2);
 #ifdef PCG_CLOCK_STAMP
diff --git a/promptable-counterfactual-gan_amd/csrc/pcg_common.h b/promptable-counterfactual-gan_amd/csrc/pcg_common.h
--- a/promptable-counterfactual-gan_amd/csrc/pcg_common.h
+++ b/promptable-counterfactual-gan_amd/csrc/pcg_common.h
@@ -51,7 +51,7 @@
   }
 };
 
-__device__ __forceinline__ uint32_t xcd_remap(uint32_t bid, uint32_t nblocks) {
+__host__ __device__ __forceinline__ uint32_t xcd_remap(uint32_t bid, uint32_t nblocks) {
   const uint32_t q = nblocks >> 3, r = nblocks & 7u;
   const uint32_t xcd = bid & 7u, idx = bid >> 3;
   const uint32_t base = xcd < r ? xcd * (q + 1) : r * (q + 1) + (xcd - r) * q;
diff --git a/promptable-counterfactual-gan_amd/ops.py b/promptable-counterfactual-gan_amd/ops.py
--- a/promptable-counterfactual-gan_amd/ops.py
+++ b/promptable-counterfactual-gan_amd/ops.py
@@ -163,6 +163,20 @@
     check(_lib.load().pcg_conv_pad_clip_query(ctypes.byref(g), int(op), int(groups), int(bool(assume_scratch)), ctypes.byref(taken),
                                               ctypes.byref(order), ctypes.byref(rows), ctypes.byref(pred)), "pcg_conv_pad_clip_query")
     return bool(taken.value), order.value, rows.value, pred.value
+
+
+def conv_wgrad_padskip_query(g, op=2):
+    applies, frac = ctypes.c_int32(0), ctypes.c_double(0.0)
+    check(_lib.load().pcg_conv_wgrad_padskip_query(ctypes.byref(g), int(op), ctypes.byref(applies), ctypes.byref(frac)),
+          "pcg_conv_wgrad_padskip_query")
+    return bool(applies.value), frac.value
+
+
+def conv_wgrad_padskip_plan(g, assume_scratch=True):
+    mode, bit = ctypes.c_int32(-1), ctypes.c_int32(-1)
+    check(_lib.load().pcg_conv_wgrad_padskip_plan(ctypes.byref(g), int(bool(assume_scratch)), ctypes.byref(mode), ctypes.byref(bit)),
+          "pcg_conv_wgrad_padskip_plan")
+    return mode.value, bit.value
 
 
 def launch_plan(op, *args):
```

Result: faster. 54120, median of 6 (+1.0%).
